# marios2019/CSN

Hardware: AMD Instinct MI355X
Metric: CSA fwd+bwd points/sec (10k pts x 256 ch, K=3) (higher is better)
Workload: dtype bf16x3 (fp32 operands split into 2 bf16, 3 bf16 MFMA per product, fp32 accumulate); 1 GPU; BASELINE configs[2]: CSA K=3, 32 query shapes/GPU x 10000 pts x 256 ch, n_heads=1, d_k=d_v=256, 20 blocks of 500, 39 classes, fwd + masked CE + bwd, train mode (dropout 0.1 live, 2K+2 evaluations/shape), math mode bf16x3; K=3, parallelism=single GPU

## Files before the change

csn_amd/_lib.py:

```python
from __future__ import annotations

import ctypes
import hashlib
import os
import subprocess
from ctypes import c_char_p, c_double, c_float, c_int, c_longlong, c_ulonglong, c_void_p
from typing import Optional

_HERE = os.path.dirname(os.path.abspath(__file__))
_CSRC = os.path.join(_HERE, "csrc")
LIB_PATH = os.path.join(_HERE, "libcsn_hip.so")
SOURCES = ["gemm_f32.hip", "gemm_bf16x3.hip", "wx_stream.hip", "wx_lnb.hip", "loss.hip", "attn_f32.hip", "attn_bf16x3.hip", "attn_dkv.hip", "attn_dv_scores.hip", "fold.hip", "outproj_ln.hip", "retrieval.hip", "retrieval_screen.hip", "combine.hip", "compat.hip", "minkowski_csn.hip", "minkowski_seg.hip", "rows_fc.hip", "sparse_conv.hip", "sparse_conv_maps16.hip", "train_maps16.hip", "sparse_conv_cat.hip", "octant_conv.hip", "octant_conv_maps16.hip", "octant_conv_stats.hip", "rows_bn_act.hip", "point_field.hip", "kernel_map.hip", "octant_map.hip", "points.hip", "csn_capi.hip"]
HEADERS = ["csn_common.h", "csn_kernels.h", "csn_window.h", "wx_common.h", "rows_mma.h", "sconv_gemm_body.inc", "sconv_a16_body.inc", "rows_bn_act_body.inc", "octant_rows_body.inc", os.path.join("..", "..", "include", "csn_hip.h")]
ARCH = "gfx950"
BUILD_FLAGS = [f"--offload-arch={ARCH}", "-O3", "-std=c++17", "-fPIC", "-fvisibility=hidden", "-shared"]

_lib: Optional[ctypes.CDLL] = None


class CsnError(RuntimeError):
    pass


class BnTerms(ctypes.Structure):
    _fields_ = [("z", c_void_p * 3), ("ld_z", c_longlong * 3), ("mean", c_void_p * 3), ("scale", c_void_p * 3),
                ("gamma", c_void_p * 3), ("beta", c_void_p * 3), ("dz", c_void_p * 3), ("ld_dz", c_longlong * 3),
                ("dgamma", c_void_p * 3), ("dbeta", c_void_p * 3)]


class CatParts(ctypes.Structure):
    _fields_ = [("x", c_void_p * 4), ("ld_x", c_longlong * 4), ("c_in", c_int * 4)]


STAMP_PATH = LIB_PATH + ".sha256"


def _source_digest() -> str:
    h = hashlib.sha256(" ".join(BUILD_FLAGS).encode())
    for f in SOURCES + HEADERS:
        h.update(f.encode())
        with open(os.path.join(_CSRC, f), "rb") as fh:
            h.update(fh.read())
    return h.hexdigest()


def _stale() -> bool:
# ... 127 lines not shown
                                        c_float, c_ulonglong, c_void_p]),
    "csn_varlen_attn_bwd_f32": (c_int, [c_void_p, c_void_p, c_longlong, c_void_p, c_void_p, c_void_p, c_longlong, c_longlong,
                                        c_int, c_int, c_void_p, c_void_p, c_void_p, c_void_p, c_void_p, c_void_p, c_void_p,
                                        c_longlong, c_longlong, c_int, c_int, c_int, c_int, c_int, c_void_p, c_void_p, c_int,
                                        c_float, c_ulonglong, c_void_p]),
    "csn_cross_attn_flash_available": (c_int, [c_int]),
    "csn_cross_attn_bwd_flash_f32": (c_int, [c_void_p, c_void_p, c_longlong, c_void_p, c_void_p, c_void_p, c_longlong, c_longlong,
                                             c_int, c_int, c_void_p, c_void_p, c_void_p, c_void_p, c_void_p, c_longlong,
                                             c_longlong, c_int, c_int, c_int, c_int, c_int, c_int, c_float, c_ulonglong,
                                             c_void_p]),
    "csn_varlen_attn_bwd_flash_f32": (c_int, [c_void_p, c_void_p, c_longlong, c_void_p, c_void_p, c_void_p, c_longlong, c_longlong,
                                              c_int, c_int, c_void_p, c_void_p, c_void_p, c_void_p, c_void_p, c_longlong,
                                              c_longlong, c_int, c_int, c_int, c_int, c_int, c_void_p, c_void_p, c_int, c_float,
                                              c_ulonglong, c_void_p]),
    "csn_project_qkv_f32": (c_int, [c_void_p, c_longlong, c_int, c_void_p, c_int, c_int, c_void_p, c_longlong, c_int, c_void_p,
                                    c_longlong, c_int, c_int, c_int, c_float, c_int, c_void_p]),
    "csn_outproj_ln_workspace_floats": (c_longlong, [c_int, c_int, c_int, c_int]),
    "csn_masked_ce_workspace_bytes": (c_longlong, [c_int, c_int]),
    "csn_masked_ce_fwd_f32": (c_int, [c_void_p, c_longlong, c_int, c_void_p, c_longlong, c_int, c_int, c_int, c_int, c_void_p,
                                      c_void_p, c_longlong, c_void_p, c_void_p]),
    "csn_masked_ce_bwd_f32": (c_int, [c_void_p, c_longlong, c_int, c_void_p, c_longlong, c_int, c_int, c_int, c_int, c_void_p,
                                      c_void_p, c_void_p, c_void_p, c_longlong, c_int, c_void_p]),
    "csn_outproj_ln_fwd_f32": (c_int, [c_void_p, c_longlong, c_void_p, c_void_p, c_longlong, c_void_p, c_void_p,
                                       c_longlong, c_void_p, c_int, c_int, c_int, c_int, c_int, c_float, c_float,
                                       c_ulonglong, c_void_p, c_void_p, c_longlong, c_void_p]),
    "csn_outproj_ln_bwd_f32": (c_int, [c_void_p, c_void_p, c_void_p, c_longlong, c_void_p, c_longlong, c_void_p,
                                       c_void_p, c_void_p, c_void_p, c_void_p, c_void_p, c_longlong, c_int, c_int, c_int,
                                       c_int, c_int, c_int, c_float, c_ulonglong, c_int, c_longlong, c_void_p, c_int,
                                       c_void_p, c_int, c_void_p]),
    "csn_outproj_lnb_workspace_floats": (c_longlong, [c_int, c_int, c_int, c_int, c_int]),
    "csn_outproj_lnb_f32": (c_int, [c_void_p, c_void_p, c_void_p, c_longlong, c_void_p, c_void_p, c_void_p, c_void_p, c_int, c_int,
                                    c_int, c_int, c_int, c_int, c_float, c_ulonglong, c_void_p, c_int, c_void_p, c_int, c_void_p,
                                    c_void_p, c_void_p, c_longlong, c_void_p]),
    "csn_project_wgrad_f32": (c_int, [c_void_p, c_longlong, c_int, c_void_p, c_longlong, c_int, c_void_p, c_int, c_int,
                                      c_int, c_int, c_float, c_int, c_void_p, c_longlong, c_void_p]),
    "csn_retrieval_measure_f32": (c_int, [c_void_p, c_void_p, c_void_p, c_int, c_int, c_int, c_int, c_int, c_void_p,
                                          c_longlong, c_void_p]),
    "csn_rowsum_f32": (c_int, [c_void_p, c_void_p, c_longlong, c_int, c_longlong, c_void_p]),
    "csn_mix_fwd_f32": (c_int, [c_void_p, c_void_p, c_void_p, c_void_p, c_void_p, c_int, c_int, c_int, c_int, c_void_p,
                                c_void_p]),
    "csn_mix_bwd_f32": (c_int, [c_void_p, c_void_p, c_void_p, c_void_p, c_void_p, c_void_p, c_void_p, c_int, c_int, c_int,
                                c_int, c_void_p, c_void_p, c_void_p]),
    "csn_compat_fwd_f32": (c_int, [c_void_p, c_void_p, c_void_p, c_void_p, c_void_p, c_void_p, c_void_p, c_void_p, c_int, c_int,
                                   c_int, c_int, c_void_p]),
    "csn_compat_bwd_f32": (c_int, [c_void_p, c_void_p, c_void_p, c_void_p, c_void_p, c_void_p, c_void_p, c_void_p, c_longlong,
                                   c_void_p, c_void_p, c_void_p, c_void_p, c_void_p, c_int, c_int, c_int, c_int, c_void_p]),
    "csn_ragged_pool_f32": (c_int, [c_void_p, c_longlong, c_int, c_void_p, c_void_p, c_int, c_int, c_void_p, c_void_p, c_void_p,
                                    c_void_p, c_void_p]),
    "csn_ragged_pool_bwd_f32": (c_int, [c_void_p, c_void_p, c_void_p, c_void_p, c_int, c_int, c_void_p, c_longlong, c_int, c_int,
                                        c_void_p]),
    "csn_ragged_mix_fwd_f32": (c_int, [c_void_p, c_longlong, c_int, c_int, c_int, c_void_p, c_void_p, c_int, c_int, c_int, c_void_p,
                                       c_void_p, c_void_p, c_void_p, c_longlong, c_void_p]),
    "csn_ragged_mix_bwd_f32": (c_int, [c_void_p, c_longlong, c_void_p, c_longlong, c_int, c_int, c_int, c_void_p, c_void_p, c_int,
                                       c_int, c_int, c_void_p, c_void_p, c_void_p, c_void_p, c_void_p, c_void_p, c_longlong,
                                       c_void_p]),
    "csn_ragged_retrieval_f32": (c_int, [c_void_p, c_void_p, c_void_p, c_int, c_void_p, c_void_p, c_void_p, c_int, c_int, c_void_p,
                                         c_void_p, c_longlong, c_void_p]),
    "csn_retrieval_screen_workspace_floats": (c_longlong, [c_longlong, c_longlong, c_int, c_int, c_int, c_int]),
    "csn_retrieval_screen_eps": (c_float, [c_int]),
    "csn_ragged_retrieval_screen_f16": (c_int, [c_void_p, c_void_p, c_void_p, c_int, c_void_p, c_void_p, c_void_p, c_int, c_int,
                                                c_void_p, c_void_p, c_longlong, c_void_p]),
    "csn_ragged_retrieval_pairs_f32": (c_int, [c_void_p, c_void_p, c_void_p, c_int, c_void_p, c_void_p, c_void_p, c_int, c_int,
                                               c_void_p, c_longlong, c_void_p, c_void_p, c_longlong, c_void_p]),
    "csn_ragged_seg_workspace_bytes": (c_longlong, [c_int]),
    "csn_ragged_seg_fwd_f32": (c_int, [c_void_p, c_int, c_int, c_void_p, c_void_p, c_void_p, c_int, c_int, c_int, c_void_p, c_void_p,
                                       c_void_p, c_void_p, c_void_p, c_void_p, c_longlong, c_void_p]),
# ... 68 lines not shown
                                                  c_void_p, c_void_p, c_void_p, c_void_p, c_float, c_float, c_void_p, c_longlong,
                                                  c_void_p]),
    "csn_sparse_conv_stats_fwd_t16": (c_int, [c_void_p, c_int, c_longlong, c_int, c_void_p, c_int, c_int, c_int, c_int, c_void_p, c_void_p,
                                              c_longlong, c_void_p, c_void_p, c_void_p, c_void_p, c_float, c_float, c_void_p,
                                              c_longlong, c_void_p]),
    "csn_rows_bn_act_fwd_t16": (c_int, [c_void_p, c_int, c_int, c_int, c_int, c_float, c_void_p, c_int, c_longlong, c_int, c_void_p,
                                        c_int, c_longlong, c_void_p]),
    "csn_rows_bn_act_bwd_t16": (c_int, [c_void_p, c_longlong, c_void_p, c_int, c_longlong, c_void_p, c_int, c_int, c_int, c_int,
                                        c_float, c_int, c_void_p, c_longlong, c_void_p, c_longlong, c_void_p]),
    "csn_sparse_conv_bwd_t16": (c_int, [c_void_p, c_longlong, c_void_p, c_int, c_longlong, c_int, c_int, c_int, c_int, c_int, c_void_p,
                                        c_void_p, c_void_p, c_void_p, c_longlong, c_void_p, c_void_p, c_void_p, c_longlong, c_void_p]),
    "csn_voxel_mean_f32": (c_int, [c_void_p, c_longlong, c_int, c_void_p, c_void_p, c_int, c_int, c_void_p, c_longlong, c_void_p]),
    "csn_point_interp_fwd_f32": (c_int, [c_void_p, c_longlong, c_int, c_void_p, c_void_p, c_void_p, c_int, c_int, c_void_p, c_longlong,
                                         c_void_p]),
    "csn_point_interp_bwd_f32": (c_int, [c_void_p, c_longlong, c_int, c_void_p, c_void_p, c_void_p, c_void_p, c_int, c_int, c_void_p,
                                         c_longlong, c_void_p]),
    "csn_coord_keys_i64": (c_int, [c_void_p, c_int, c_int, c_void_p, c_void_p, c_void_p]),
    "csn_coord_down_i64": (c_int, [c_void_p, c_int, c_int, c_void_p, c_void_p]),
    "csn_kernel_map_i32": (c_int, [c_void_p, c_void_p, c_int, c_void_p, c_int, c_int, c_int, c_void_p, c_void_p, c_void_p]),
    "csn_octant_partition_i32": (c_int, [c_void_p, c_void_p, c_int, c_int, c_void_p, c_void_p, c_int, c_void_p, c_void_p, c_void_p, c_void_p,
                                         c_void_p]),
    "csn_octant_order_workspace_bytes": (c_longlong, [c_int]),
    "csn_octant_order_i32": (c_int, [c_void_p, c_int, c_void_p, c_void_p, c_void_p, c_longlong, c_void_p, c_void_p]),
    "csn_points_normalize_f32": (c_int, [c_void_p, c_void_p, c_int, c_longlong, c_int, c_void_p, c_void_p, c_void_p]),
    "csn_points_bounds_f64": (c_int, [c_void_p, c_void_p, c_int, c_longlong, c_void_p, c_void_p, c_int, c_void_p, c_void_p, c_void_p]),
    "csn_points_batch_f32": (c_int, [c_void_p, c_void_p, c_void_p, c_int, c_longlong, c_void_p, c_void_p, c_void_p, c_void_p, c_int,
                                     c_int, c_double, c_double, c_double, c_void_p, c_void_p, c_void_p, c_void_p, c_longlong, c_void_p,
                                     c_void_p]),
    "csn_field_index_i32": (c_int, [c_void_p, c_void_p, c_void_p, c_int, c_int, c_void_p, c_void_p, c_void_p, c_void_p, c_void_p,
                                    c_void_p]),
}

EXPORTS = tuple(_SIGNATURES)
DEV_BIG_TILES, DEV_WIDE_GEMM, DEV_WIDE_FORMS, DEV_WX, DEV_LNB_GROUP, DEV_SCONV_NB, DEV_KV_SAME = 0, 1, 2, 3, 5, 7, 8
DEV_WX_DEFAULT = 9


def lib() -> ctypes.CDLL:
    global _lib
    if _lib is None:
        path = os.environ.get("CSN_LIB_PATH", LIB_PATH)
        if not os.path.exists(path):
            raise CsnError(f"{path} is missing: run `python -c 'import __graft_entry__ as g; g.build()'` "
                           "(there is no CPU or eager fallback for the CSA kernels)")
        handle = ctypes.CDLL(path)
        for name, (res, args) in _SIGNATURES.items():
            fn = getattr(handle, name)
            fn.restype = res
            fn.argtypes = args
        if handle.csn_version() != 17:
            raise CsnError("libcsn_hip.so ABI version mismatch")
        _lib = _Hooked(handle)
    return _lib


_call_hook = None


def set_call_hook(fn) -> None:
    global _call_hook
    _call_hook = fn


class _Hooked:

    def __init__(self, handle):
        self._handle = handle
# ... 24 lines not shown
```

csn_amd/csrc/attn_bf16x3.hip:

```cpp
#include "csn_common.h"
#include "csn_kernels.h"

namespace {

constexpr int KT = 32;
constexpr float LOG2E = 1.4426950408889634f, LN2 = 0.6931471805599453f;

using namespace csn_mode;
typedef f32x4m f32x4v;
typedef s16x4 __attribute__((address_space(3))) * lds_s16x4;
typedef short __attribute__((address_space(3))) lds_s16;
typedef s16x8 __attribute__((address_space(3))) lds_s16x8;

CSN_DEVINL const lds_s16* opaque_lds(const short* p) {
  const lds_s16* q = (const lds_s16*)p;
  asm volatile("" : "+v"(q));
  return q;
}

template <typename PR>
CSN_DEVINL f32x4v mma16(s16x8 ah, s16x8 al, s16x8 bh, s16x8 bl, f32x4v c) {
  if constexpr (PR::NT == 3) {
    c = mfma16<PR::HALF>(al, bh, c);
    c = mfma16<PR::HALF>(ah, bl, c);
  }
  return mfma16<PR::HALF>(ah, bh, c);
}

constexpr bool csn_attn_x3fwd96(int npl, int dt, bool bwd) { return npl == 2 && dt == 3 && !bwd; }
constexpr int csn_attn_waves(int npl, int dt, bool bwd, bool rc_f32 = false) {
  return (!rc_f32 && ((npl == 1 ? dt <= 3 : dt <= 2) || csn_attn_x3fwd96(npl, dt, bwd))) ? 4 : 2;
}
template <typename PR, int DT, bool BWD, bool KVP, bool RC = false, int NOP = 0, bool KV_SAME = false>
__global__ __launch_bounds__(512, csn_attn_waves(PR::NPL, DT, BWD, RC && !KVP)) void csn_attn_bf16x3_kernel(CsnAttnArgs p) {
  static_assert(!KV_SAME || (DT == 8 && NOP == 2), "one request per tile: the folded d = 256 backward");
  static_assert(PR::NT == 3 || KVP, "single-product modes take K / V as tile planes");
  static_assert(!RC || BWD, "score recomputation: backward kernel");
  static_assert(!NOP || (BWD && KVP && !RC && PR::NPL == 2), "no P planes: the kept-scores backward in two planes");
  constexpr int NPL = PR::NPL;
  constexpr int D = 32 * DT;
  constexpr int UPR = KVP ? 4 * NPL : 8;
  constexpr int RPP = 512 / UPR;
  constexpr int PIECES = D * UPR;
  constexpr int NP_T = (PIECES + 511) / 512;
  constexpr int PLANE = D * KT + 32;
  constexpr bool EARLY = NPL == 1 || DT <= 4 || (!BWD && !RC);
  static_assert(!RC || EARLY, "score recomputation: early requests (where three LDS images per stage fit)");
  constexpr int NB_ST = RC ? 3 : 2;
  constexpr int TILE_EL = (2 + NB_ST + (RC ? 2 : 0)) * NPL * PLANE, STAGE_EL = D * 128 * 2;
  static_assert(2 * (TILE_EL > STAGE_EL ? TILE_EL : STAGE_EL) <= 160 * 1024, "LDS budget of one CU");
  __shared__ __attribute__((aligned(16))) short tiles[TILE_EL > STAGE_EL ? TILE_EL : STAGE_EL];
  auto tileA = [&](int st, int pl) -> short* { return tiles + (st * NPL + pl) * PLANE; };
  auto tileB = [&](int st, int pl) -> short* { return tiles + ((2 + st) * NPL + pl) * PLANE; };
  auto tileC = [&](int st, int pl) -> short* { return tiles + ((2 + NB_ST + st) * NPL + pl) * PLANE; };

  const int tid = threadIdx.x, lane = tid & 63, wave = tid >> 6;
  const int lq = lane & 15, kq = lane >> 4;
  const int Tq = p.Tq > 0 ? p.Tq : p.T;
  const int QT = (Tq + 127) / 128;
  const int Y = p.n_blocks * p.H;
  const int L = blockIdx.x, slot = L & 7, jj = L >> 3;
  const int qt = jj % QT, u = (jj / QT) * 8 + slot;
  if (u >= Y * p.E) return;
  const int zz = u / Y;
  const int it0 = p.grp_off ? p.grp_off[zz] : zz;
  const int it1 = p.grp_off ? p.grp_off[zz + 1] : it0 + 1;
  const int e0 = p.eval_ids ? p.eval_ids[it0] : it0;
  const int hd = (u % Y) % p.H, blk = (u % Y) / p.H;
// ... 106 lines not shown
    if (KVP) {
      const unsigned off = (kt * KT + 8 * t_u) < T ? t_off : CSN_OOB;
#pragma unroll
      for (int i = 0; i < NP_T; ++i)
        g[i] = csn_bload4(rs, (i == NP_T - 1 && !t_last_ok) ? CSN_OOB : off, (unsigned)(kt * (64 * NPL) + RPP * i * kld * 2));
    } else {
      const int k0 = kt * KT;
      const unsigned off = (k0 + 4 * t_c) < T ? t_off : CSN_OOB;
#pragma unroll
      for (int i = 0; i < NP_T; ++i)
        g[i] = csn_bload4(rs, (i == NP_T - 1 && !t_last_ok) ? CSN_OOB : off, (unsigned)(k0 + 64 * i * ldk) * 4u);
    }
  };

  auto stage_in = [&](const csn_rsrc_t& rs, int fmt) {
    f32x4 ch[CH_T];
    if (NPL == 1 && fmt) {
      u32x2 c2[CH_T];
#pragma unroll
      for (int t = 0; t < CH_T; ++t) c2[t] = csn_bload2(rs, c_off == CSN_OOB ? CSN_OOB : c_off >> 1, (unsigned)(16 * t * ld) * 2u);
#pragma unroll
      for (int t = 0; t < CH_T; ++t) ch[t] = act16_to_f32(__builtin_bit_cast(s16x4, c2[t]), fmt);
    } else {
#pragma unroll
      for (int t = 0; t < CH_T; ++t) ch[t] = csn_bload4(rs, c_off, (unsigned)(16 * t * ld) * 4u);
    }
#pragma unroll
    for (int t = 0; t < CH_T; ++t) {
      const int row = crow + 16 * t;
      *reinterpret_cast<f32x4*>(&xbuf[row * 128 + ((cc ^ (4 * ((row >> 3) & 1))) << 2)]) = ch[t];
    }
  };
  auto pick = [&](int row) { return xbuf[row * 128 + ((((col >> 2) ^ (4 * ((row >> 3) & 1))) << 2) | (col & 3))]; };
  float rv[D / 4];
  if (BWD || it == it0) {
    stage_in(Rr, p.r_fmt);
    __syncthreads();
#pragma unroll
    for (int s = 0; s < D / 32; ++s)
#pragma unroll
      for (int j = 0; j < 8; ++j) {
        const float v = pick(32 * s + 8 * kq + j);
        rv[8 * s + j] = v;
        Rh[s][j] = to16<PR::HALF>(v);
        Rl[s][j] = PR::NT == 3 ? to16<PR::HALF>(v - from16<PR::HALF>(Rh[s][j])) : Rh[s][j];
      }
  }
  if (!BWD) {
    os = p.out_index ? p.out_index[e] : e;
    stat_off0 = stat_off;
#pragma unroll
    for (int c = 0; c < D / 16; ++c) O[c] = f32x4v{0.f, 0.f, 0.f, 0.f};
    m_run = -INFINITY; m2_run = -INFINITY; l_run = 0.f;
  }
  float delta_q = 0.f;
  if (BWD) {
    const csn_rsrc_t Xr = map_rsrc(p.ctx, qs * p.q_shape_stride + head_off, p.ctx_fmt);
    __syncthreads();
    stage_in(Xr, p.ctx_fmt);
    __syncthreads();
#pragma unroll
    for (int s = 0; s < D / 32; ++s)
#pragma unroll
      for (int j = 0; j < 8; ++j) delta_q = fmaf(rv[8 * s + j], pick(32 * s + 8 * kq + j), delta_q);
    delta_q += __shfl_xor(delta_q, 16, 64);
    delta_q += __shfl_xor(delta_q, 32, 64);
  }
  if constexpr (RC) {
    const long long q2s = p.q2_index ? p.q2_index[e] : e;
    if (it == it0 || q2s != q2s_staged) {
      q2s_staged = q2s;
      const csn_rsrc_t Qr = map_rsrc(p.q2, q2s * p.q2_shape_stride + head_off, p.q2_fmt);
      __syncthreads();
      stage_in(Qr, p.q2_fmt);
      __syncthreads();
#pragma unroll
      for (int s = 0; s < D / 32; ++s)
#pragma unroll
        for (int j = 0; j < 8; ++j) {
          const float v = pick(32 * s + 8 * kq + j);
          Qh[s][j] = to16<PR::HALF>(v);
          Ql[s][j] = PR::NT == 3 ? to16<PR::HALF>(v - from16<PR::HALF>(Qh[s][j])) : Qh[s][j];
        }
    }
  }
  __syncthreads();

  const bool drop = p.dropout_p > 0.f;
  const unsigned thr16 = csn_drop_threshold16(p.dropout_p);
  const float keep_scale = drop ? 1.f / (1.f - p.dropout_p) : 1.f;
  const unsigned salt = csn_block_salt((unsigned long long)(((long long)e * p.H + hd) * p.n_blocks + blk), p.seed);
  const int mp = Tq > Tp ? Tq : Tp;
  const unsigned pw_base = (unsigned)(4 * kq * mp + qrow);

  float lse2_q = 0.f;
  if (BWD) {
    lse2_q = q_ok ? p.lse[stat_off + qrow] * LOG2E : 0.f;
// ... 305 lines not shown
    if constexpr (RC) {
    } else if constexpr (EARLY) {
      if (more) commitB_from(nxt, g2);
    } else {
      if (more) { commitB(nxt); if (kt + 2 < nkt) fetch(Ar, kt + 2); }
    }
    __syncthreads();
  }

  if (!late) __syncthreads();
  if constexpr (!BWD) write_out();
  }

  if constexpr (BWD) write_out();
}

template <typename PR, int DT>
int launch_dt(const CsnAttnArgs& a, bool bwd, hipStream_t st) {
  const long long units = (long long)a.n_blocks * a.H * a.E;
  dim3 grid((unsigned)(((units + 7) / 8) * 8 * (((a.Tq > 0 ? a.Tq : a.T) + 127) / 128)));
  if (a.kv_planes) {
    if (bwd) {
      if constexpr (!PR::HALF) {
        if (a.q2) {
          if constexpr (csn_attn_recompute_fits(PR::NPL, DT))
            hipLaunchKernelGGL((csn_attn_bf16x3_kernel<PR, DT, true, true, true>), grid, dim3(512), 0, st, a);
          else return -1;
        } else if (a.sc_tiles == 2) {
          if constexpr (csn_attn_dv_scores_fits(PR::NT == 3 ? 1 : 2, 32 * DT))
            hipLaunchKernelGGL((csn_attn_bf16x3_kernel<PR, DT, true, true, false, 1>), grid, dim3(512), 0, st, a);
          else return -1;
        } else if (a.sc_tiles == 3) {
          if constexpr (csn_attn_dv_scores_fits(PR::NT == 3 ? 1 : 2, 32 * DT)) {
            if (a.kv_same) hipLaunchKernelGGL((csn_attn_bf16x3_kernel<PR, DT, true, true, false, 2, true>), grid, dim3(512), 0, st, a);
            else hipLaunchKernelGGL((csn_attn_bf16x3_kernel<PR, DT, true, true, false, 2>), grid, dim3(512), 0, st, a);
          } else return -1;
        } else hipLaunchKernelGGL((csn_attn_bf16x3_kernel<PR, DT, true, true>), grid, dim3(512), 0, st, a);
      } else return -1;
    } else hipLaunchKernelGGL((csn_attn_bf16x3_kernel<PR, DT, false, true>), grid, dim3(512), 0, st, a);
  } else {
    if constexpr (PR::NT == 3) {
      if (bwd && a.q2) {
        if constexpr (csn_attn_recompute_fits(PR::NPL, DT))
          hipLaunchKernelGGL((csn_attn_bf16x3_kernel<PR, DT, true, false, true>), grid, dim3(512), 0, st, a);
        else return -1;
      } else if (bwd) hipLaunchKernelGGL((csn_attn_bf16x3_kernel<PR, DT, true, false>), grid, dim3(512), 0, st, a);
      else hipLaunchKernelGGL((csn_attn_bf16x3_kernel<PR, DT, false, false>), grid, dim3(512), 0, st, a);
    } else return -1;
  }
  return (int)hipGetLastError();
}

template <typename PR>
int launch_any(const CsnAttnArgs& a, int d, bool bwd, hipStream_t st) {
  if (a.E <= 0 || a.n_blocks <= 0) return 0;
  if ((a.ld & 3) || (a.Tp & 3) || (a.ld_kv & 3)) return -2;
  if ((a.T & 3) && a.kv_planes) return -2;
  if ((a.q_shape_stride & 3) || (a.kv_shape_stride & 3)) return -4;
  if (a.sc_tiles && a.Tp < (a.T + 31) / 32 * 32) return -2;
  if (a.sc_layout && (PR::NPL != 2 || !a.kv_planes || a.Tq > 0 || a.tq_arr || a.t_arr || a.Tp < (a.T + 31) / 32 * 32 || (bwd && !a.sc_tiles)))
    return -1;
  if (a.q2 && (!bwd || (a.q2_shape_stride & 3))) return -1;
  if (a.sc_tiles >= 2 && (a.sc_tiles > 3 || !bwd || !a.kv_planes || a.q2 || a.Tq > 0 || a.tq_arr || a.t_arr)) return -1;
  if (a.q2 && !a.kv_planes && (a.sc_tiles || a.grp_off)) return -1;
  if ((a.r_fmt || a.ctx_fmt || a.q2_fmt || a.out_fmt) && (PR::NPL != 1 || !a.kv_planes)) return -1;
  if (a.out_fmt && a.accumulate) return -1;
  if (a.kv_planes && (a.T > 512 || (a.kv_ld & 7) || (a.kv_shape_stride & 7))) return -2;
  switch (d) {
    case 32: return launch_dt<PR, 1>(a, bwd, st);
    case 64: return launch_dt<PR, 2>(a, bwd, st);
    case 96: return launch_dt<PR, 3>(a, bwd, st);
    case 128: return launch_dt<PR, 4>(a, bwd, st);
    case 256: return launch_dt<PR, 8>(a, bwd, st);
    default: return -5;
  }
}

int launch_mode(const CsnAttnArgs& a, int d, int mode, bool bwd, hipStream_t st) {
  switch (mode) {
    case 1: return launch_any<Bf16x3>(a, d, bwd, st);
    case 2: return launch_any<Bf16>(a, d, bwd, st);
    case 3: return launch_any<F16>(a, d, bwd, st);
    default: return -1;
  }
}

}

int csn_dev_kv_same = 1;

int csn_launch_attn_fwd_bf16x3(const CsnAttnArgs& a, int d, int mode, hipStream_t st) {
  return launch_mode(a, d, mode, false, st);
}
int csn_launch_attn_bwd_bf16x3(const CsnAttnArgs& a, int d, int mode, hipStream_t st) { return launch_mode(a, d, mode, true, st); }
```

csn_amd/csrc/csn_capi.hip:

```cpp
#include "../../include/csn_hip.h"
#include "csn_kernels.h"
#include <cmath>

namespace {

int g_math_mode = CSN_MATH_BF16X3;
thread_local int t_math_mode = -1;

inline int mode() { return t_math_mode >= 0 ? t_math_mode : g_math_mode; }
thread_local int t_act16 = 0;
inline int act16() { return t_act16 & 3; }
inline bool grad16() { return (t_act16 & 4) != 0; }
inline bool act16_fwd_ok() { return act16() == 0 || (act16() == 1 && mode() == 2) || (act16() == 2 && mode() == 3); }
inline bool act16_bwd_ok() { return act16() == 0 || mode() == 2; }
thread_local int t_rows16 = 0;
inline int rows_mode() { return mode() >= 2 && !t_rows16 ? 1 : mode(); }
thread_local int t_score_layout = 0;
inline int planes_of(int m) { return m == 1 ? 2 : 1; }

struct ModeGuard {
  int saved;
  explicit ModeGuard(int m) : saved(t_math_mode) { t_math_mode = m; }
  ~ModeGuard() { t_math_mode = saved; }
};

int launch_gemm(const CsnGemmArgs& a, int b_is_nk, int batch, hipStream_t st) {
  if (mode() != 0) {
    if (a.M <= 0 || a.N <= 0 || batch <= 0) return 0;
    if ((a.A.ld & 3) || (a.B.ld & 3) || (a.K & 3) || (a.k_chunk & 3)) return CSN_E_ALIGN;
    if (a.N & 3) return CSN_E_ALIGN;
    return csn_launch_gemm_bf16x3(a, b_is_nk, batch, mode(), st);
  }
  return csn_launch_gemm_f32(a, b_is_nk, batch, st);
}

inline bool mis16(const void* p) { return (reinterpret_cast<uintptr_t>(p) & 15) != 0; }

int launch_wx(const float* w, const float* x, long long x_stride, int ldx, void* out, long long out_stride, int ldo, int rows,
              int n_items, int n_points, int div_rows, float div_val, int out_mode, int tb, hipStream_t st) {
  CsnWxArgs a;
  a.w = w; a.x = x; a.x_item_stride = x_stride; a.ldx = ldx;
  a.out = out; a.out_item_stride = out_stride; a.ldo = ldo;
  a.n_items = n_items; a.n_points = n_points; a.n_sets = rows / 256;
  a.div_rows = div_rows; a.div_val = div_val; a.div_rcp = 1.f / div_val;
  int ex = 0;
  a.div_exact = (std::frexp(div_val, &ex) == 0.5f && div_val > 0.f) ? 1 : 0;
  a.tb = tb;
  return csn_launch_wx(a, out_mode, st);
}

// ... 17 lines not shown
int wgrad_chunk(int n_maps, int n_points) {
  long long total = (long long)n_maps * n_points;
  long long want = (total + 511) / 512;
  if (want < 256) want = 256;
  long long n_chunks = (n_points + want - 1) / want;
  if (n_chunks < 1) n_chunks = 1;
  long long c = (n_points + n_chunks - 1) / n_chunks;
  c = ((c + 3) / 4) * 4;
  return (int)c;
}

int wgrad(const float* a, long long a_stride, int lda, const float* b, long long b_stride, int ldb, float* dw, int rows,
          int cols, int n_maps, int n_points, float scale, int accumulate, float* ws, long long ws_floats,
          hipStream_t st, int a_fmt = 0, int b_fmt = 0) {
  const int chunk = wgrad_chunk(n_maps, n_points);
  const int n_chunks = (n_points + chunk - 1) / chunk;
  const long long slabs = (long long)n_maps * n_chunks;
  if (ws_floats < slabs * rows * cols) return CSN_E_WORKSPACE;
  CsnGemmArgs g;
  g.A = operand(a, chunk, 0, a_stride, nullptr, lda);
  g.B = operand(b, chunk, 0, b_stride, nullptr, ldb);
  g.A.fmt = a_fmt; g.B.fmt = b_fmt;
  g.C = operand(ws, (long long)rows * cols, 0, (long long)n_chunks * rows * cols, nullptr, cols);
  g.M = rows; g.N = cols; g.K = n_points;
  g.n0 = n_chunks; g.n1 = 1; g.k_chunk = chunk;
  g.alpha = 1.f; g.div_rows = 0; g.div_val = 1.f; g.accumulate = 0; g.eval_ids = nullptr;
  int rc = launch_gemm(g, 1, (int)slabs, st);
  if (rc) return rc;
  return csn_launch_slab_reduce(ws, dw, (int)slabs, (long long)rows * cols, scale, accumulate, st);
}

}

extern "C" {

int csn_version(void) { return CSN_ABI_VERSION; }

int csn_dev_get(int key) {
  switch (key) {
    case CSN_DEV_BIG_TILES: return csn_gemm_big_tiles;
    case CSN_DEV_WIDE_GEMM: return csn_gemm_wide;
    case CSN_DEV_WIDE_FORMS: return csn_gemm_wide_set;
    case CSN_DEV_WX: return csn_dev_wx;
    case CSN_DEV_LNB_GROUP: return csn_dev_lnb_group;
    case CSN_DEV_SCONV_NB: return csn_dev_sconv_nb;
    case CSN_DEV_KV_SAME: return csn_dev_kv_same;
    default: return CSN_E_ARG;
  }
}
int csn_dev_set(int key, int value) {
  const int prev = csn_dev_get(key);
  switch (key) {
    case CSN_DEV_BIG_TILES: csn_gemm_big_tiles = value; break;
    case CSN_DEV_WIDE_GEMM: csn_gemm_wide = value; break;
    case CSN_DEV_WIDE_FORMS: csn_gemm_wide_set = value; break;
    case CSN_DEV_WX:
      if (value & ~(1 | 4 | 8)) return CSN_E_ARG;
      csn_dev_wx = value;
      break;
    case CSN_DEV_LNB_GROUP: csn_dev_lnb_group = value < 0 ? 0 : value; break;
    case CSN_DEV_SCONV_NB:
      if (value < 0 || value > 4) return CSN_E_ARG;
      csn_dev_sconv_nb = value;
      break;
    case CSN_DEV_KV_SAME:
      if (value != 0 && value != 1) return CSN_E_ARG;
      csn_dev_kv_same = value;
      break;
    default: return CSN_E_ARG;
  }
  return prev;
}

int csn_set_math_mode(int m) {
  if (m < 0 || m > 3) return CSN_E_ARG;
  g_math_mode = m;
  return 0;
}
int csn_set_thread_math_mode(int m) {
  if (m < -1 || m > 3) return CSN_E_ARG;
  t_math_mode = m;
  return 0;
}
int csn_get_math_mode(void) { return mode(); }
int csn_get_thread_math_mode(void) { return t_math_mode; }
int csn_set_thread_act16(int fmt) {
  if (fmt < 0 || (fmt & 3) == 3 || fmt > 6 || fmt == 4) return CSN_E_ARG;
  t_act16 = fmt;
  return 0;
}
int csn_get_thread_act16(void) { return t_act16; }
int csn_set_thread_rows16(int on) {
  if (on != 0 && on != 1) return CSN_E_ARG;
  t_rows16 = on;
  return 0;
}
int csn_get_thread_rows16(void) { return t_rows16; }
int csn_set_thread_score_layout(int layout) {
  if (layout < 0 || layout > 1) return CSN_E_ARG;
  t_score_layout = layout;
  return 0;
}
int csn_get_thread_score_layout(void) { return t_score_layout; }

const char* csn_status_string(int status) {
  switch (status) {
    case 0: return "ok";
    case CSN_E_ARG: return "csn: null pointer, non-positive size, a count beyond its row, or a flag this math mode does not take";
    case CSN_E_ALIGN: return "csn: a size or leading dimension is not a multiple of 4 floats";
    case CSN_E_PTR: return "csn: device pointer not 16-byte aligned";
    case CSN_E_STRIDE: return "csn: a stride is not a multiple of 4 floats";
    case CSN_E_DIM: return "csn: unsupported head / model dimension (need 32, 64, 96, 128 or 256)";
    case CSN_E_WORKSPACE: return "csn: workspace too small";
    default: return status > 0 ? hipGetErrorString((hipError_t)status) : "csn: unknown status";
  }
}

long long csn_wgrad_workspace_floats(int rows, int cols, int n_maps, int n_points) {
  if (rows <= 0 || cols <= 0 || n_maps <= 0 || n_points <= 0) return 0;
  const int chunk = wgrad_chunk(n_maps, n_points);
  const long long n_chunks = (n_points + chunk - 1) / chunk;
  return (long long)n_maps * n_chunks * rows * cols;
}

// ... 221 lines not shown

int csn_block_attn_fwd_grouped_f32(const float* q, const float* k, const float* v, long long q_shape_stride,
                                   long long kv_shape_stride, const int* q_index, const int* kv_index, int ld, float* ctx,
                                   long long ctx_eval_stride, float* scores, float* lse, int n_evals, int n_heads,
                                   int d_head, int block, int n_blocks, int score_pitch, float rescale_threshold,
                                   float dropout_p, unsigned long long seed, int qkv_split, long long qkv_plane_stride,
                                   const int* eval_ids, const int* group_offsets, int n_groups, void* stream) {
  if (!eval_ids || !group_offsets) return CSN_E_ARG;
  return attn_fwd_impl(q, k, v, q_shape_stride, kv_shape_stride, q_index, kv_index, ld, ctx, ctx_eval_stride, scores, lse,
                       n_evals, n_heads, d_head, block, n_blocks, score_pitch, rescale_threshold, dropout_p, seed, qkv_split,
                       qkv_plane_stride, 0, 0, stream, nullptr, nullptr, eval_ids, group_offsets, n_groups);
}

int csn_cross_attn_fwd_f32(const float* q, const float* k, const float* v, long long q_shape_stride,
                           long long kv_shape_stride, int ld_q, int ld_kv, float* ctx, long long ctx_eval_stride,
                           float* scores, float* lse, int n_evals, int n_heads, int d_head, int n_queries, int n_keys,
                           int score_pitch, float rescale_threshold, float dropout_p, unsigned long long seed, void* stream) {
  if (n_queries <= 0 || n_keys <= 0) return CSN_E_ARG;
  if (n_queries & 3) return CSN_E_ALIGN;
  ModeGuard guard(mode() >= 2 ? 1 : mode());
  return attn_fwd_impl(q, k, v, q_shape_stride, kv_shape_stride, nullptr, nullptr, ld_q, ctx, ctx_eval_stride, scores, lse,
                       n_evals, n_heads, d_head, n_keys, 1, score_pitch, rescale_threshold, dropout_p, seed, 0, 0, n_queries,
                       ld_kv, stream);
}

static int attn_bwd_dq_impl(const float* dctx, const float* ctx, long long ctx_eval_stride, const float* k,
                            const float* v, long long kv_shape_stride, const int* kv_index, int ld, float* scores,
                            float* dscores, const float* lse, float* delta, float* dq, long long dq_slot_stride,
                            const int* dq_index, int accumulate, const int* eval_ids, int n_launch_evals, int n_heads,
                            int d_head, int block, int n_blocks, int score_pitch, float dropout_p,
                            unsigned long long seed, int dctx_split, long long dctx_plane_stride, int kv_split,
                            long long kv_plane_stride, int probs_tiles, int block_q, int ld_kv, const int* group_offsets,
                            int n_groups, void* stream, const int* tq_arr = nullptr, const int* t_arr = nullptr,
                            const float* q = nullptr, long long q_shape_stride = 0, const int* q_index = nullptr) {
  if (block_q < 0 || ld_kv < 0 || (ld_kv & 3)) return CSN_E_ARG;
  if (q && (block_q != 0 || !kv_split || !(csn_attn_bwd_grouping(d_head, block) & 4) || mis16(q))) return CSN_E_ARG;
  if (q && (q_shape_stride & 3)) return CSN_E_STRIDE;
  if ((tq_arr || t_arr) && (group_offsets || n_blocks != 1)) return CSN_E_ARG;
  if (n_blocks <= 0 || block <= 0) return CSN_E_ARG;
  const int t_last = last_block_points(block, n_blocks, ld, block_q);
  if (t_last < 0) return t_last;
  if (block_q != 0 && ((long long)n_blocks * block_q > ld || (long long)n_blocks * ((block + 3) / 4 * 4) > (ld_kv > 0 ? ld_kv : ld)))
    return CSN_E_ARG;
  if (group_offsets && (n_groups <= 0 || !eval_ids || !(csn_attn_bwd_grouping(d_head, block) & 1))) return CSN_E_ARG;
  if ((block & 3) && (block_q == 0 || kv_split)) return CSN_E_ALIGN;
  if (probs_tiles && (mode() == 0 || score_pitch < (block + 31) / 32 * 32)) return CSN_E_ARG;
  if (probs_tiles < 0 || probs_tiles > 3) return CSN_E_ARG;
  if (probs_tiles >= 2 && (q || !kv_split || block_q != 0 || tq_arr || t_arr || act16() ||
                           !csn_attn_bwd_dv_scores_available(d_head, block)))
    return CSN_E_ARG;
  if (dropout_p < 0.f || dropout_p >= 1.f) return CSN_E_ARG;
  if (dctx_split) return CSN_E_ARG;
  if (kv_split && mode() == 0) return CSN_E_ARG;
  if (kv_split < 0 || kv_split > 2 || (kv_split == 2 && mode() != 2)) return CSN_E_ARG;
  if (mode() == 3) return CSN_E_ARG;
  if (mode() == 2 && !(kv_split && (probs_tiles || q))) return CSN_E_ARG;
  const int bp = 512 * planes_of(mode());
  if (kv_split && (kv_plane_stride <= 0 || (kv_plane_stride % bp) || kv_plane_stride < (long long)n_blocks * bp ||
                   block > 512 || (kv_shape_stride & 7)))
    return CSN_E_ARG;
  const bool need_sc = !q || (probs_tiles && mode() == 1), need_ds = (!q || probs_tiles) && probs_tiles != 3;
  if (!dctx || !ctx || !k || !v || !lse || (!delta && probs_tiles != 3) || !dq || (need_sc && !scores) || (need_ds && !dscores)) return CSN_E_ARG;
  if (n_launch_evals <= 0 || n_heads <= 0 || block <= 0 || n_blocks <= 0) return CSN_E_ARG;
  if (!dim_ok(d_head)) return CSN_E_DIM;
  if ((ld & 3) || (score_pitch & 3) || score_pitch < (block + 3) / 4 * 4) return CSN_E_ALIGN;
  if (mis16(dctx) || mis16(k) || mis16(v) || mis16(scores) || mis16(dscores) || mis16(dq)) return CSN_E_PTR;
  if ((kv_shape_stride & 3) || (ctx_eval_stride & 3) || (dq_slot_stride & 3)) return CSN_E_STRIDE;
  hipStream_t st = (hipStream_t)stream;
  CsnAttnArgs a;
  a.ctx = ctx;
  a.T_last = t_last;
  a.Tq = block_q; a.ld_kv = ld_kv;
  a.q = dctx; a.k = k; a.v = v;
  a.q_shape_stride = dctx_split ? 2 * ctx_eval_stride : ctx_eval_stride;
  a.kv_shape_stride = kv_shape_stride;
  a.q_index = nullptr; a.kv_index = kv_index; a.ld = ld;
  a.out = dq; a.out_eval_stride = dq_slot_stride;
  a.scores = scores; a.dscores = dscores; a.lse = const_cast<float*>(lse); a.delta = delta;
  a.E = group_offsets ? n_groups : n_launch_evals; a.H = n_heads; a.T = block; a.Tp = score_pitch; a.n_blocks = n_blocks;
  a.rescale_threshold = 0.f;
  a.eval_ids = eval_ids; a.grp_off = group_offsets; a.out_index = dq_index; a.accumulate = accumulate;
  a.dropout_p = dropout_p; a.seed = seed;
  a.r_planes = 0; a.kv_planes = kv_split != 0; a.r_plane_stride = 0; a.kv_plane_stride = 0; a.kv_ld = (int)kv_plane_stride;
  a.kv_f16 = kv_split == 2;
  a.sc_tiles = probs_tiles;
  if (kv_split == 1 && k == v && mode() == 1 && d_head == 256 && probs_tiles == 3) a.kv_same = csn_dev_kv_same;
  a.tq_arr = tq_arr; a.t_arr = t_arr;
  a.q2 = q; a.q2_shape_stride = q_shape_stride; a.q2_index = q_index;
  if (t_score_layout) {
    if (mode() != 1 || !kv_split || block_q != 0 || tq_arr || t_arr || !probs_tiles) return CSN_E_ARG;
    a.sc_layout = 1;
  }
  if (act16()) {
    if (!act16_bwd_ok() || !kv_split || block_q != 0) return CSN_E_ARG;
    a.r_fmt = 1; a.ctx_fmt = act16(); a.q2_fmt = act16();
    if (grad16()) {
      if (accumulate) return CSN_E_ARG;
      a.out_fmt = 1;
    }
  }
  return mode() != 0 ? csn_launch_attn_bwd_bf16x3(a, d_head, mode(), st) : csn_launch_attn_bwd_f32(a, d_head, st);
}

int csn_block_attn_bwd_dq_f32(const float* dctx, const float* ctx, long long ctx_eval_stride, const float* k,
                              const float* v, long long kv_shape_stride, const int* kv_index, int ld, float* scores,
                              float* dscores, const float* lse, float* delta, float* dq, long long dq_slot_stride,
                              const int* dq_index, int accumulate, const int* eval_ids, int n_launch_evals, int n_heads,
                              int d_head, int block, int n_blocks, int score_pitch, float dropout_p,
                              unsigned long long seed, int dctx_split, long long dctx_plane_stride, int kv_split,
                              long long kv_plane_stride, int probs_tiles, const int* group_offsets, int n_groups,
                              void* stream) {
  return attn_bwd_dq_impl(dctx, ctx, ctx_eval_stride, k, v, kv_shape_stride, kv_index, ld, scores, dscores, lse, delta, dq,
                          dq_slot_stride, dq_index, accumulate, eval_ids, n_launch_evals, n_heads, d_head, block, n_blocks,
                          score_pitch, dropout_p, seed, dctx_split, dctx_plane_stride, kv_split, kv_plane_stride, probs_tiles,
                          0, 0, group_offsets, n_groups, stream);
}

int csn_block_attn_bwd_dq_recompute_f32(const float* dctx, const float* ctx, long long ctx_eval_stride, const float* q,
                                        long long q_shape_stride, const int* q_index, const float* k, const float* v,
                                        long long kv_shape_stride, const int* kv_index, int ld, float* probs,
                                        float* dscores, const float* lse, float* delta, float* dq,
                                        long long dq_slot_stride, const int* dq_index, int accumulate, const int* eval_ids,
                                        int n_launch_evals, int n_heads, int d_head, int block, int n_blocks,
                                        int score_pitch, float dropout_p, unsigned long long seed,
                                        long long kv_plane_stride, int kv_f16, int probs_tiles, const int* group_offsets,
                                        int n_groups, void* stream) {
  if (!q) return CSN_E_ARG;
  return attn_bwd_dq_impl(dctx, ctx, ctx_eval_stride, k, v, kv_shape_stride, kv_index, ld, probs, dscores, lse, delta, dq,
                          dq_slot_stride, dq_index, accumulate, eval_ids, n_launch_evals, n_heads, d_head, block, n_blocks,
                          score_pitch, dropout_p, seed, 0, 0, kv_f16 ? 2 : 1, kv_plane_stride, probs_tiles, 0, 0, group_offsets,
                          n_groups, stream, nullptr, nullptr, q, q_shape_stride, q_index);
}

static int attn_bwd_dkv_impl(const float* dctx, long long ctx_eval_stride, const float* q, long long q_shape_stride,
                             const int* q_index, int ld, const float* probs, const float* dscores, float* dk,
                             float* dv, long long dkv_slot_stride, const int* dk_index, const int* dv_index,
                             int accumulate, const int* eval_ids, int n_launch_evals, int n_heads, int d_head,
                             int block, int n_blocks, int score_pitch, int dctx_split, long long dctx_plane_stride,
                             int q_split, long long q_plane_stride, int probs_tiles, int block_q, int ld_kv,
                             const int* group_offsets, int n_groups, void* stream, const int* tq_arr = nullptr,
                             const int* t_arr = nullptr) {
  if (block_q < 0 || ld_kv < 0 || (ld_kv & 3) || (block_q & 3)) return CSN_E_ARG;
  if ((block & 3) && block_q == 0) return CSN_E_ALIGN;
  const int bq = block_q > 0 ? block_q : block, lk = ld_kv > 0 ? ld_kv : ld, bk4 = (block + 3) / 4 * 4;
  if (n_blocks <= 0 || block <= 0) return CSN_E_ARG;
  const int t_last = last_block_points(block, n_blocks, ld, block_q);
  if (t_last < 0) return t_last;
  if (block_q != 0 && ((long long)n_blocks * bk4 > lk || (long long)n_blocks * bq > ld)) return CSN_E_ARG;
  if (probs_tiles && (mode() == 0 || score_pitch < (block + 31) / 32 * 32)) return CSN_E_ARG;
  if (mode() == 3 || (mode() == 2 && !probs_tiles)) return CSN_E_ARG;
  if (dctx_split || q_split) return CSN_E_ARG;
  if (group_offsets && (n_groups <= 0 || !eval_ids || !(csn_attn_bwd_grouping(d_head, block) & 2))) return CSN_E_ARG;
  const bool dk_only = !probs && !dv;
  if (!dctx || !q || !dscores || !dk || (!dv && !dk_only)) return CSN_E_ARG;
  if (!probs && !dk_only && !(probs_tiles && mode() == 2)) return CSN_E_ARG;
  if (n_launch_evals <= 0 || n_heads <= 0 || block <= 0 || n_blocks <= 0) return CSN_E_ARG;
  if (!dim_ok(d_head)) return CSN_E_DIM;
  if ((ld & 3) || (score_pitch & 3) || score_pitch < bk4) return CSN_E_ALIGN;
  if (mis16(dctx) || mis16(q) || mis16(probs) || mis16(dscores) || mis16(dk) || mis16(dv)) return CSN_E_PTR;
  if ((q_shape_stride & 3) || (ctx_eval_stride & 3) || (dkv_slot_stride & 3)) return CSN_E_STRIDE;
// ... 310 lines not shown
                           long long xres_shape_stride, const int* res_index, float* xhat,
                           long long xhat_eval_stride, float* rstd, int n_evals, int d_model, int d_inner, int ld,
                           int n_points, float eps, float dropout_p, unsigned long long seed, float* xhat_sum,
                           float* sum_ws, long long sum_ws_floats, void* stream) {
  if (dropout_p < 0.f || dropout_p >= 1.f) return CSN_E_ARG;
  if (!ctx || !wfc || !xres || !xhat || !rstd || n_evals <= 0 || n_points <= 0 || d_inner <= 0 || n_points > ld) return CSN_E_ARG;
  if (dropout_p > 0.f && (long long)(d_model / 2 + 1) * ld >= (1ll << 32)) return CSN_E_ARG;
  if (xhat_sum && xhat_eval_stride != (long long)d_model * ld) return CSN_E_STRIDE;
  if (!dim_ok(d_model)) return CSN_E_DIM;
  if ((ld & 3) || (d_inner & 3) || (n_points & 3)) return CSN_E_ALIGN;
  if (mis16(ctx) || mis16(wfc) || mis16(xres) || mis16(xhat)) return CSN_E_PTR;
  if ((ctx_eval_stride & 3) || (xres_shape_stride & 3) || (xhat_eval_stride & 3)) return CSN_E_STRIDE;
  CsnOutProjArgs a;
  a.ctx = ctx; a.ctx_eval_stride = ctx_eval_stride; a.wfc = wfc;
  a.xres = xres; a.xres_shape_stride = xres_shape_stride; a.res_index = res_index;
  a.xhat = xhat; a.xhat_eval_stride = xhat_eval_stride; a.rstd = rstd;
  a.E = n_evals; a.C = d_model; a.D = d_inner; a.ld = ld; a.n_points = n_points; a.eps = eps;
  a.dropout_p = dropout_p; a.seed = seed;
  a.xhat_sum = xhat_sum; a.sum_ws = sum_ws; a.sum_ws_floats = sum_ws ? sum_ws_floats : 0;
  if (act16() && !act16_fwd_ok()) return CSN_E_ARG;
  a.act16 = act16();
  return csn_launch_outproj_ln_fwd_f32(a, mode(), (hipStream_t)stream);
}

int csn_outproj_ln_bwd_f32(const float* dxhat, const float* xhat, const float* rstd, long long eval_stride,
                           const float* ctx, long long ctx_eval_stride, const float* wfc_t, float* dz, float* dz_res,
                           float* dctx, float* dwfc, float* ws, long long ws_floats, int n_evals, int d_model,
                           int d_inner, int ld, int n_points, int accumulate, float dropout_p,
                           unsigned long long seed, int dctx_split, long long dctx_plane_stride,
                           const float* dxhat_rows, int n_dense_evals, const float* dxhat_scale, int dxhat_group,
                           void* stream) {
  if (dropout_p < 0.f || dropout_p >= 1.f) return CSN_E_ARG;
  if (dxhat_group < 0) return CSN_E_ARG;
  if (dropout_p > 0.f && (long long)(d_model / 2 + 1) * ld >= (1ll << 32)) return CSN_E_ARG;
  if (dctx_split && mode() == 0) return CSN_E_ARG;
  if (n_dense_evals < 0 || n_dense_evals > n_evals || (n_dense_evals > 0 && !dxhat)) return CSN_E_ARG;
  if (!xhat || !rstd || !ctx || !wfc_t || !dz || !dctx || !dwfc || !ws) return CSN_E_ARG;
  if (n_evals <= 0 || n_points <= 0 || d_inner <= 0 || d_model <= 0 || n_points > ld) return CSN_E_ARG;
  if ((ld & 3) || (d_inner & 3) || (d_model & 3) || (n_points & 3)) return CSN_E_ALIGN;
  if (mis16(dxhat) || mis16(xhat) || mis16(ctx) || mis16(wfc_t) || mis16(dz) || mis16(dctx) || mis16(dwfc) || mis16(ws))
    return CSN_E_PTR;
  if ((eval_stride & 3) || (ctx_eval_stride & 3)) return CSN_E_STRIDE;
  hipStream_t st = (hipStream_t)stream;
  CsnLnBwdArgs l;
  l.dxhat = dxhat; l.xhat = xhat; l.rstd = rstd; l.dz = dz; l.dz_res = dz_res; l.eval_stride = eval_stride;
  l.E = n_evals; l.C = d_model; l.ld = ld; l.n_points = n_points;
  l.dropout_p = dropout_p; l.seed = seed;
  l.dxhat_rows = dxhat_rows; l.n_dense = n_dense_evals;
  l.dxhat_scale = dxhat_scale; l.dxhat_group = dxhat_group > 0 ? dxhat_group : 1;
  const int a16 = act16();
  if (a16 && (!act16_bwd_ok() || dctx_split)) return CSN_E_ARG;
  l.act16 = a16;
  int rc = 0;
  if (mode() == 1 && !a16 && !dctx_split && csn_wx_takes(d_inner, d_model) &&
      csn_wx_geometry_takes(csn_dev_lnb_group > 0 && csn_dev_lnb_group < n_evals ? csn_dev_lnb_group : n_evals, n_points, d_inner / 256)) {
    const int G = csn_dev_lnb_group > 0 ? csn_dev_lnb_group : n_evals;
    const bool fused = csn_wx_lnb_takes(l, d_inner) && eval_stride == ctx_eval_stride;
    for (int e0 = 0; e0 < n_evals && !rc; e0 += G) {
      const int ng = n_evals - e0 < G ? n_evals - e0 : G;
      if (fused) {
        CsnWxLnbArgs f{};
        f.w = wfc_t; f.xhat = xhat; f.rstd = rstd; f.eval_stride = eval_stride; f.ld = ld;
        f.dxhat = dxhat; f.dxhat_group = l.dxhat_group; f.n_dense = n_dense_evals; f.dxhat_scale = dxhat_scale; f.dxhat_rows = dxhat_rows;
        f.dz = dz; f.dz_res = dz_res; f.dctx = dctx; f.dctx_eval_stride = ctx_eval_stride;
        f.n_items = ng; f.n_points = n_points; f.e_base = e0; f.dropout_p = dropout_p; f.seed = seed;
        rc = csn_launch_wx_lnb(f, st);
        if (rc != CSN_NOT_TAKEN) continue;
      }
      l.e_base = e0; l.E = ng;
      rc = csn_launch_ln_bwd_f32(l, st);
      if (rc) return rc;
      rc = launch_wx(wfc_t, dz + (long long)e0 * eval_stride, eval_stride, ld, dctx + (long long)e0 * ctx_eval_stride, ctx_eval_stride, ld,
                     d_inner, ng, n_points, 0, 1.f, 0, 0, st);
    }
    if (rc) return rc;
    return wgrad(dz, eval_stride, ld, ctx, ctx_eval_stride, ld, dwfc, d_model, d_inner, n_evals, n_points, 1.f, accumulate, ws,
                 ws_floats, st, 0, 0);
  }
  rc = csn_launch_ln_bwd_f32(l, st);
  if (rc) return rc;
  CsnGemmArgs g;
  g.A = operand(wfc_t, 0, 0, 0, nullptr, d_model);
  g.B = operand(dz, 0, 0, eval_stride, nullptr, ld);
  g.C = operand(dctx, 0, 0, dctx_split ? 2 * ctx_eval_stride : ctx_eval_stride, nullptr, ld);
  g.C.planes = dctx_split; g.C.plane_stride = dctx_plane_stride;
  if (a16) { g.B.fmt = CSN_FMT_16; g.C.planes = 1; }
  g.M = d_inner; g.N = n_points; g.K = d_model;
  g.n0 = 1; g.n1 = 1; g.k_chunk = 0;
  g.alpha = 1.f; g.div_rows = 0; g.div_val = 1.f; g.accumulate = 0; g.eval_ids = nullptr;
  rc = launch_gemm(g, 0, n_evals, st);
  if (rc) return rc;
  return wgrad(dz, eval_stride, ld, ctx, ctx_eval_stride, ld, dwfc, d_model, d_inner, n_evals, n_points, 1.f,
               accumulate, ws, ws_floats, st, a16 ? CSN_FMT_16 : 0, a16 == 2 ? CSN_FMT_F16_TO_BF16 : (a16 ? CSN_FMT_16 : 0));
}

static bool lnb_range_takes(int n_evals, int d_model, int d_inner, int ld, int n_points, long long eval_stride) {
  if (n_evals <= 0 || n_points <= 0 || n_points > ld || mode() != 1 || act16()) return false;
  CsnLnBwdArgs l{};
  l.C = d_model; l.ld = ld; l.n_points = n_points; l.eval_stride = eval_stride; l.act16 = 0;
  return csn_wx_takes(d_inner, d_model) && csn_wx_geometry_takes(n_evals, n_points, d_inner / 256) && csn_wx_lnb_takes(l, d_inner);
}

long long csn_outproj_lnb_workspace_floats(int n_evals, int d_model, int d_inner, int ld, int n_points) {
  if (!lnb_range_takes(n_evals, d_model, d_inner, ld, n_points, (long long)d_model * ld)) return 0;
  return csn_wx_lnb_red_floats(n_evals, n_points);
}

int csn_outproj_lnb_f32(const float* dxhat, const float* xhat, const float* rstd, long long eval_stride, const float* wfc_t,
                        float* dz, float* dz_res, float* dctx, int e_base, int n_evals, int d_model, int d_inner, int ld,
                        int n_points, float dropout_p, unsigned long long seed, const float* dxhat_rows, int n_dense_evals,
                        const float* dxhat_scale, int dxhat_group, float* rowdot, float* rowsum, float* red_ws,
                        long long red_ws_floats, void* stream) {
  if (dropout_p < 0.f || dropout_p >= 1.f) return CSN_E_ARG;
  if (dxhat_group < 0 || e_base < 0 || n_evals <= 0 || n_dense_evals < 0 || (n_dense_evals > 0 && !dxhat)) return CSN_E_ARG;
  if (!xhat || !rstd || !wfc_t || !dz || !dctx) return CSN_E_ARG;
  if (n_points <= 0 || d_inner <= 0 || d_model <= 0 || n_points > ld) return CSN_E_ARG;
  if (dropout_p > 0.f && (long long)(d_model / 2 + 1) * ld >= (1ll << 32)) return CSN_E_ARG;
  if ((ld & 3) || (d_inner & 3) || (d_model & 3) || (n_points & 3)) return CSN_E_ALIGN;
  if (mis16(dxhat) || mis16(xhat) || mis16(wfc_t) || mis16(dz) || mis16(dz_res) || mis16(dctx) || mis16(red_ws)) return CSN_E_PTR;
  if (eval_stride & 3) return CSN_E_STRIDE;
  if (!lnb_range_takes(e_base + n_evals, d_model, d_inner, ld, n_points, eval_stride)) return CSN_E_DIM;
  const int group = dxhat_group > 0 ? dxhat_group : 1;
  const bool reduce = rowdot || rowsum || red_ws;
  if (reduce) {
    if (!rowdot || !rowsum || !red_ws || e_base != 0 || n_evals > n_dense_evals || n_evals % group) return CSN_E_ARG;
    if (red_ws_floats < csn_wx_lnb_red_floats(n_evals, n_points)) return CSN_E_WORKSPACE;
  }
  CsnWxLnbArgs f{};
  f.w = wfc_t; f.xhat = xhat; f.rstd = rstd; f.eval_stride = eval_stride; f.ld = ld;
  f.dxhat = dxhat; f.dxhat_group = group; f.n_dense = n_dense_evals; f.dxhat_scale = dxhat_scale; f.dxhat_rows = dxhat_rows;
  f.dz = dz; f.dz_res = dz_res; f.dctx = dctx; f.dctx_eval_stride = eval_stride;
  f.n_items = n_evals; f.n_points = n_points; f.e_base = e_base; f.dropout_p = dropout_p; f.seed = seed;
  if (reduce) { f.red_ws = red_ws; f.red_slots = csn_wx_ln_sum_slots(n_evals, n_points); f.rowdot = rowdot; f.rowsum = rowsum; }
  const int rc = csn_launch_wx_lnb(f, (hipStream_t)stream);
  return rc == CSN_NOT_TAKEN ? CSN_E_DIM : rc;
}

int csn_project_wgrad_f32(const float* dout, long long dout_shape_stride, int ld_dout, const float* x,
                          long long x_shape_stride, int ld_x, float* dw, int rows, int channels, int n_shapes,
                          int n_points, float scale, int accumulate, float* ws, long long ws_floats,
                          void* stream) {
  if (!dout || !x || !dw || !ws || rows <= 0 || channels <= 0 || n_shapes <= 0 || n_points <= 0) return CSN_E_ARG;
  if (n_points > ld_dout || n_points > ld_x) return CSN_E_ARG;
  if ((ld_dout & 3) || (ld_x & 3) || (n_points & 3) || (channels & 3)) return CSN_E_ALIGN;
  if (mis16(dout) || mis16(x) || mis16(dw) || mis16(ws)) return CSN_E_PTR;
  if ((dout_shape_stride & 3) || (x_shape_stride & 3)) return CSN_E_STRIDE;
  const bool g16 = act16() && grad16();
  if (g16 && !act16_bwd_ok()) return CSN_E_ARG;
  return wgrad(dout, dout_shape_stride, ld_dout, x, x_shape_stride, ld_x, dw, rows, channels, n_shapes, n_points, scale,
               accumulate, ws, ws_floats, (hipStream_t)stream, g16 ? CSN_FMT_16 : 0, 0);
}

int csn_retrieval_measure_f32(const float* f1, const float* f2, float* out, int s1, int n1, int s2, int n2,
                              int channels, float* ws, long long ws_floats, void* stream) {
  if (!f1 || !f2 || !out || !ws || s1 <= 0 || s2 <= 0 || n1 <= 0 || n2 <= 0 || channels <= 0) return CSN_E_ARG;
  if (channels & 3) return CSN_E_ALIGN;
  if (mis16(f1) || mis16(f2) || mis16(ws)) return CSN_E_PTR;
  const long long need = (long long)s1 * n1 + (long long)s2 * n2 + (long long)s1 * s2 * n1;
  if (ws_floats < need) return CSN_E_WORKSPACE;
  return csn_launch_retrieval_f32(f1, f2, out, s1, n1, s2, n2, channels, ws, (hipStream_t)stream);
}

int csn_rowsum_f32(const float* x, float* out, long long rows, int n_points, long long ld, void* stream) {
  if (!x || !out || rows <= 0 || n_points <= 0 || n_points > ld) return CSN_E_ARG;
  if ((n_points & 3) || (ld & 3)) return CSN_E_ALIGN;
  if (mis16(x)) return CSN_E_PTR;
  return csn_launch_rowsum_f32(x, out, rows, n_points, ld, (hipStream_t)stream, act16());
}
// ... 1025 lines not shown
```

csn_amd/csrc/csn_kernels.h:

```cpp
#pragma once
#include "csn_common.h"

struct CsnGemmArgs {
  CsnOperand A, B, C;
  int M, N, K;
  int n0, n1;
  int k_chunk;
  float alpha;
  int div_rows;
  float div_val;
  int accumulate;
  const int* eval_ids;
  int batch;
  const int* grp_off = nullptr;
  const int* grp_items = nullptr;
  const int* n_arr = nullptr;
  const int* k_arr = nullptr;
  int n_last = 0, k_last = 0;
};

int csn_launch_gemm_f32(const CsnGemmArgs& a, int b_is_nk, int batch, hipStream_t st);
int csn_launch_gemm_bf16x3(const CsnGemmArgs& a, int b_is_nk, int batch, int mode, hipStream_t st);
int csn_gemm_tile_major_planes(int M, int N);
int csn_gemm_bf16x3_big_tiles(int M, int N);
// ... 37 lines not shown
struct CsnAttnArgs {
  const float* q;  const float* k;  const float* v;
  long long q_shape_stride, kv_shape_stride;
  const int* q_index; const int* kv_index;
  int ld;
  float* out;        long long out_eval_stride;
  float* scores;
  float* dscores;
  float* lse;
  float* delta;
  const float* ctx;
  int E, H, T, Tp, n_blocks;
  float rescale_threshold;
  const int* eval_ids;
  const int* grp_off;
  const int* out_index;
  int accumulate;
  float dropout_p;
  unsigned long long seed;
  int r_planes, kv_planes;
  long long r_plane_stride, kv_plane_stride;
  int kv_ld;
  int Tq;
  int ld_kv;
  int sc_tiles;
  const int* tq_arr;
  const int* t_arr;
  int T_last;
  const float* q2 = nullptr; long long q2_shape_stride = 0; const int* q2_index = nullptr;
  int kv_f16 = 0;
  int r_fmt = 0, ctx_fmt = 0, q2_fmt = 0, out_fmt = 0;
  int sc_layout = 0;
  int kv_same = 0;
};
extern int csn_dev_kv_same;
constexpr bool csn_attn_recompute_fits(int planes, int dt) { return planes == 1 || dt <= 4; }
struct CsnAttnDkvArgs {
  const float* q;     long long q_shape_stride;  const int* q_index;
  const float* dctx;  long long ctx_eval_stride;
  const float* k;  const float* v;
  long long kv_shape_stride;  int kv_ld;  const int* kv_index;
  const float* lse;  const float* delta;
  float* dk;  float* dv;  long long dkv_slot_stride;
  const int* dk_index;  const int* dv_index;
  int accumulate;
  const int* eval_ids;  const int* grp_off;  int n_groups;
  int ld, H, T, Tp, n_blocks, T_last;
  float dropout_p;  unsigned long long seed;
  int kv_f16 = 0;
  int q_fmt = 0, dctx_fmt = 0;
  int out_fmt = 0;
  int Tq = 0, ld_kv = 0;
  const int* tq_arr = nullptr;  const int* t_arr = nullptr;
};
int csn_launch_attn_dkv_flash(const CsnAttnDkvArgs& a, int d, int mode, hipStream_t st);
constexpr bool csn_attn_dkv_flash_fits(int dt) { return dt <= 4; }

struct CsnAttnDvArgs {
  const float* dctx;  long long ctx_eval_stride;
  const float* scores;
  const float* lse;
  float* dv;  long long dkv_slot_stride;  const int* dv_index;
  const int* eval_ids;  const int* grp_off;  int n_groups;
  int ld, H, T, Tp, n_blocks, T_last;
  float dropout_p;  unsigned long long seed;
  int sc_layout = 0;
// ... 30 lines not shown
  float* lse;
  double* partials;
  float* stats;
  const float* grad_out;  float* dlogits;  long long dshape_stride;  int dld;
};
long long csn_masked_ce_blocks(int n_shapes, int n_points);
int csn_launch_masked_ce_fwd(const CsnMaskedCeArgs& a, hipStream_t st);
int csn_launch_masked_ce_bwd(const CsnMaskedCeArgs& a, hipStream_t st);

struct CsnLnBwdArgs {
  const float* dxhat; const float* xhat; const float* rstd;
  const float* dxhat_rows;
  int n_dense;
  const float* dxhat_scale; int dxhat_group;
  float* dz;
  float* dz_res;
  long long eval_stride;
  int E, C, ld, n_points;
  float dropout_p;
  unsigned long long seed;
  int act16 = 0;
  int e_base = 0;
};
int csn_launch_ln_bwd_f32(const CsnLnBwdArgs& a, hipStream_t st);
struct CsnWxLnbArgs {
  const float* w;
  const float* xhat; const float* rstd; long long eval_stride; int ld;
  const float* dxhat; int dxhat_group; int n_dense; const float* dxhat_scale; const float* dxhat_rows;
  float* dz; float* dz_res;
  float* dctx; long long dctx_eval_stride;
  int n_items, n_points, e_base;
  float dropout_p; unsigned long long seed;
  float* red_ws; int red_slots; float* rowdot; float* rowsum;
};
long long csn_wx_lnb_red_floats(int n_items, int n_points);
bool csn_wx_lnb_takes(const CsnLnBwdArgs& a, int d_inner);
int csn_launch_wx_lnb(const CsnWxLnbArgs& a, hipStream_t st);

int csn_launch_rowdot_f32(const float* a, const float* b, float* out, const int* eval_ids, int E, int H, int d, int ld,
                          int n_points, long long eval_stride, int a_split, long long a_plane_stride, hipStream_t st);

int csn_launch_rowsum_f32(const float* x, float* out, long long rows, int n, long long ld, hipStream_t st, int x16 = 0);
int csn_launch_mix_fwd_f32(const float* xhat, const float* comp, const float* gamma, const float* beta, float* feats, int B,
                           int K1, int C, int NP, const float* xhat0, hipStream_t st, int x16 = 0);
int csn_launch_mix_bwd_f32(const float* dfeats, const float* xhat, const float* comp, const float* gamma, float* dxhat,
                           float* rowdot, float* rowsum, int B, int K1, int C, int NP, const float* xhat0, float* dxhat0,
                           hipStream_t st, int x16 = 0);
int csn_launch_retrieval_f32(const float* f1, const float* f2, float* out, int s1, int n1, int s2, int n2, int C,
                             float* ws, hipStream_t st);

int csn_ragged_mix_tiles(int max_points);
int csn_launch_ragged_pool_f32(const float* xhat, long long eval_stride, int ld, const int* counts, int E, int C, const float* gamma,
                               const float* beta, float* pooled, float* mean, hipStream_t st);
int csn_launch_ragged_pool_bwd_f32(const float* dpooled, const float* gamma, const int* counts, int E, int C, float* dxhat,
                                   long long eval_stride, int ld, int accumulate, hipStream_t st);
int csn_launch_ragged_mix_fwd_f32(const float* xhat, long long eval_stride, int ld, int cross_first, const int* offsets, int B,
                                  int K1, int C, int max_points, const float* comp, const float* gamma, const float* beta, float* out,
                                  long long ld_out, hipStream_t st);
int csn_launch_ragged_mix_bwd_f32(const float* dout, long long ld_dout, const float* xhat, long long eval_stride, int ld,
                                  int cross_first, const int* offsets, int B, int K1, int C, const float* comp, const float* gamma,
                                  float* dxhat, double* rowdot, double* rowsum, double* ws, hipStream_t st);
int csn_launch_ragged_retrieval_f32(const float* f1, const int* off1, int s1, long long N1, const float* f2, const int* off2, int s2,
                                    long long N2, int max_n1, int C, float* out, float* ws, hipStream_t st);
int csn_launch_ragged_mean_f32(const float* part, const int* off1, float* out, int pairs, int s2, int tiles, hipStream_t st);
int csn_launch_ragged_retrieval_pairs_f32(const float* f1, const int* off1, int s1, long long N1, const float* f2, const int* off2,
                                          int s2, long long N2, int max_n1, int C, const int* pairs, long long n_pairs, float* out,
                                          float* ws, hipStream_t st);
// ... 211 lines not shown
```

csn_amd/csrc/wx_lnb.hip:

```cpp
#include "csn_common.h"
#include "csn_kernels.h"
#include "wx_common.h"
#include <type_traits>

namespace {

constexpr int LNB_G = 8 * WX_EB * 2;
constexpr int LNB_EBW = WX_EB / 2;

template <int N>
CSN_DEVINL void lnb_arrived(f32x4* R) {
  asm volatile("s_waitcnt vmcnt(%5)" : "+v"(R[0]), "+v"(R[1]), "+v"(R[2]), "+v"(R[3]), "+v"(R[4]) : "n"(N) : "memory");
}

CSN_DEVINL void lnb_store1(float v, u32x4 rsrc, unsigned voff) {
  asm volatile("buffer_store_dword %0, %1, %2, 0 offen\n\ts_nop 1" :: "v"(v), "v"(voff), "s"(rsrc) : "memory");
}

CSN_DEVINL float lnb_sum_row_groups(float v) {
  v += __builtin_bit_cast(float, __builtin_amdgcn_mov_dpp(__builtin_bit_cast(int, v), 0x128 , 0xf, 0xf, false));
  float c = v;
  asm("s_nop 1\n\tv_permlane16_swap_b32 %0, %1" : "+v"(v), "+v"(c));
  v += c;
  c = v;
  asm("s_nop 1\n\tv_permlane32_swap_b32 %0, %1" : "+v"(v), "+v"(c));
  return v + c;
}

CSN_DEVINL float lnb_sum_row_lanes(float v) {
  v += __builtin_bit_cast(float, __builtin_amdgcn_mov_dpp(__builtin_bit_cast(int, v), 0xb1 , 0xf, 0xf, false));
  v += __builtin_bit_cast(float, __builtin_amdgcn_mov_dpp(__builtin_bit_cast(int, v), 0x4e , 0xf, 0xf, false));
  v += __builtin_bit_cast(float, __builtin_amdgcn_mov_dpp(__builtin_bit_cast(int, v), 0x141 , 0xf, 0xf, false));
  return v;
}

template <bool DROP, bool RES, bool RED>
__global__ __launch_bounds__(512, 2) void csn_wx_lnb_kernel(CsnWxLnbArgs p) {
  __shared__ __attribute__((aligned(16))) short smem[LNB_G + WX_NS * WX_STAGE + 8 * LNB_EBW * 2 + 1024 + 1024 + 1024];
  short* xs = smem + LNB_G;
  const int tid = threadIdx.x, lane = tid & 63, wave = __builtin_amdgcn_readfirstlane(tid >> 6);
  const int l31 = lane & 31, h = lane >> 5;
  float* eb = reinterpret_cast<float*>(smem + LNB_G + WX_NS * WX_STAGE) + wave * LNB_EBW;
  float* red = reinterpret_cast<float*>(smem + LNB_G + WX_NS * WX_STAGE + 8 * LNB_EBW * 2);
  const float* gbuf = reinterpret_cast<const float*>(smem) + 4 * tid;
  float* ctab = red + 512;
  float* cells = ctab + 512;

  const int xcd = blockIdx.x & 7, j = blockIdx.x >> 3;
  const int n_streams = (int)gridDim.x;
  const int stream = j * 8 + xcd;
  const unsigned cpi = (unsigned)(p.n_points + WX_CH - 1) / WX_CH;
  const int n_chunks = p.n_items * (int)cpi;
  const int run = (n_chunks + n_streams - 1) / n_streams;
  const int q0 = stream * run, q_end = min(q0 + run, n_chunks);
  if (q0 >= q_end) return;

  s16x8 Wh[WX_K / 16], Wl[WX_K / 16];
  {
    const float* wrow = p.w + ((long long)(32 * wave + l31) * WX_K + 8 * h);
#pragma unroll
    for (int s = 0; s < WX_K / 16; ++s) {
      const f32x4 a0 = *reinterpret_cast<const f32x4*>(wrow + 16 * s), a1 = *reinterpret_cast<const f32x4*>(wrow + 16 * s + 4);
      s16x4 h0, l0, h1, l1;
      split4<Bf16x3>(a0, h0, l0);
      split4<Bf16x3>(a1, h1, l1);
      Wh[s] = join8(h0, h1);
      Wl[s] = join8(l0, l1);
    }
  }

  const int krow = tid >> 3, c4 = tid & 7;
  const int ld = p.ld;
  const unsigned x_voff = (unsigned)(2 * krow * ld + 4 * c4) * 4u;
  auto row_soff = [&](int i) { return (unsigned)(((i & 1) + 128 * (i >> 1)) * ld) * 4u; };
  struct Cursor { int q; unsigned item, tile; };
  auto cursor_at = [&](int q) { Cursor c; c.q = q; c.item = (unsigned)q / cpi; c.tile = (unsigned)q - c.item * cpi; return c; };
  auto advance = [&](Cursor& c) { ++c.q; if (++c.tile >= cpi) { c.tile = 0; ++c.item; } };
  auto locate = [&](const Cursor& c, int& col0, int& valid, unsigned& item) {
    const bool exists = c.q < q_end;
    col0 = exists ? (int)(c.tile * WX_CH) : 0;
    valid = exists ? min(WX_CH, p.n_points - col0) : 0;
    item = __builtin_amdgcn_readfirstlane(exists ? c.item : 0u);
  };
  auto issue_x = [&](const Cursor& cu, f32x4* R) {
    int col0, valid; unsigned item;
    locate(cu, col0, valid, item);
    const u32x4 Xr = wx_rsrc(p.xhat + (long long)(p.e_base + item) * p.eval_stride + col0, ((long long)(WX_K - 1) * ld + valid) * 4);
    const unsigned off = 4 * c4 < valid ? x_voff : CSN_OOB;
#pragma unroll
    for (int i = 0; i < 4; ++i) wx_request(R[i], Xr, off, row_soff(i));
    const u32x4 Sr = wx_rsrc(p.rstd + (long long)(p.e_base + item) * p.n_points + col0, (long long)valid * 4);
    wx_request(R[4], Sr, 4 * c4 < valid ? (unsigned)(16 * c4) : CSN_OOB, 0u);
  };
  const unsigned g_lds = __builtin_amdgcn_readfirstlane((unsigned)(unsigned long)((short __attribute__((address_space(3)))*)smem)) + (unsigned)wave * 1024u;
  auto issue_g = [&](const Cursor& cu) {
    int col0, valid; unsigned item;
    locate(cu, col0, valid, item);
    const unsigned e = (unsigned)p.e_base + item;
    const bool dense = RED || (int)e < p.n_dense;
    const unsigned src = p.dxhat_group > 1 ? e / (unsigned)p.dxhat_group : e;
    const u32x4 Gr = wx_rsrc(dense ? p.dxhat + (long long)src * p.eval_stride + col0 : nullptr, dense ? ((long long)(WX_K - 1) * ld + valid) * 4 : 0);
    const unsigned off = 4 * c4 < valid ? x_voff : CSN_OOB;
    asm volatile("s_waitcnt lgkmcnt(0)" ::: "memory");
#pragma unroll
    for (int i = 0; i < 4; ++i) wx_dma(g_lds + 8192u * i, Gr, off, row_soff(i));
  };

  const int grp = lane >> 4, gq = (lane >> 2) & 3, gp = lane & 3;
  const int tr_base = (8 * (grp >> 1) + gq) * WX_CH + 16 * (grp & 1) + 4 * gp;
  auto compute = [&](int stage) {
    f32x16 acc;
#pragma unroll
    for (int r = 0; r < 16; ++r) acc[r] = 0.f;
    const short* xh = xs + stage * WX_STAGE + tr_base;
    constexpr int WX_PD = 2, NSTEP = WX_K / 16;
    s16x8 bh[WX_PD], bl[WX_PD];
    auto rd = [&](int s, s16x8& fh, s16x8& fl) {
      const short* a = xh + 16 * s * WX_CH;
      fh = join8(__builtin_amdgcn_ds_read_tr16_b64_v4i16((lds_s16x4)(a)),
                 __builtin_amdgcn_ds_read_tr16_b64_v4i16((lds_s16x4)(a + 4 * WX_CH)));
      fl = join8(__builtin_amdgcn_ds_read_tr16_b64_v4i16((lds_s16x4)(a + WX_PLANE)),
                 __builtin_amdgcn_ds_read_tr16_b64_v4i16((lds_s16x4)(a + WX_PLANE + 4 * WX_CH)));
    };
    __builtin_amdgcn_sched_barrier(0);
#pragma unroll
    for (int s = 0; s < WX_PD; ++s) rd(s, bh[s], bl[s]);
    __builtin_amdgcn_sched_group_barrier(0x100, 4 * WX_PD, 0);
#pragma unroll
    for (int s = 0; s < NSTEP; ++s) {
      const int r = s % WX_PD;
      acc = wx_mma(Wh[s], Wl[s], bh[r], bl[r], acc);
      if (s + WX_PD < NSTEP) rd(s + WX_PD, bh[r], bl[r]);
      __builtin_amdgcn_sched_group_barrier(0x008, 3, 0);
      __builtin_amdgcn_sched_group_barrier(0x100, 4, 0);
    }
    __builtin_amdgcn_sched_barrier(0);
    return acc;
  };
  const int erow = lane >> 3, c8 = lane & 7;
  auto epilogue = [&](const Cursor& cu, const f32x16& acc) {
    int col0, valid; unsigned item;
    locate(cu, col0, valid, item);
    const bool n_ok = 4 * c8 < valid;
    const u32x4 Or = wx_rsrc(p.dctx + (long long)(p.e_base + item) * p.dctx_eval_stride, (long long)256 * ld * 4);
#pragma unroll
    for (int half = 0; half < 2; ++half) {
#pragma unroll
      for (int rr = 0; rr < 8; ++rr) eb[csn_acc_row(rr, h) * 32 + l31] = acc[8 * half + rr];
      const unsigned off = n_ok ? (unsigned)((32 * wave + 16 * half + erow) * ld + col0 + 4 * c8) * 4u : CSN_OOB;
#pragma unroll
      for (int t = 0; t < 2; ++t) {
        const f32x4 v = *reinterpret_cast<const f32x4*>(&eb[(erow + 8 * t) * 32 + 4 * c8]);
        wx_store4(v, Or, off, (unsigned)(8 * t * ld) * 4u);
      }
    }
  };

  const unsigned thr16 = csn_drop_threshold16(p.dropout_p);
  const float keep_scale = DROP ? 1.f / (1.f - p.dropout_p) : 1.f;
  unsigned cst_item = 0xffffffffu;
  unsigned red_item = 0xffffffffu;
  typedef float f32x2 __attribute__((ext_vector_type(2)));
  typedef f32x2 __attribute__((address_space(3))) * lds_f32x2;
  const unsigned smem_lds = (unsigned)(unsigned long)((short __attribute__((address_space(3)))*)smem);
  const unsigned cells_lds = (unsigned)(unsigned long)((float __attribute__((address_space(3)))*)cells);
  auto tid16 = [&]() {
    unsigned ga = (unsigned)(unsigned long)((const float __attribute__((address_space(3)))*)gbuf);
    asm volatile("" : "+v"(ga));
    return ga - smem_lds;
  };
  auto flush_red = [&]() __attribute__((always_inline)) {
    const unsigned slot = (unsigned)stream - (red_item * cpi) / (unsigned)run;
    const u32x4 Wr = wx_rsrc(p.red_ws + ((long long)red_item * p.red_slots + slot) * (2 * WX_K), 2 * WX_K * 4);
    const unsigned t16 = tid16();
    if ((t16 & 0x70u) == 0) {
      const unsigned cell = cells_lds + ((t16 >> 7) << 4), voff = (t16 >> 7) << 3;
#pragma unroll
      for (int i = 0; i < 4; ++i) {
        const lds_f32x2 c = (lds_f32x2)(unsigned long)(cell + 8 * (i & 1) + 1024 * (i >> 1));
        const f32x2 v = *c;
        *c = f32x2{0.f, 0.f};
        lnb_store1(v.x, Wr, voff + 4 * (i & 1) + 512 * (i >> 1));
        lnb_store1(v.y, Wr, voff + 4 * (i & 1) + 512 * (i >> 1) + 4 * WX_K);
      }
    }
  };
  if (RED && c4 == 0) {
#pragma unroll
    for (int i = 0; i < 4; ++i) *reinterpret_cast<float2*>(&cells[2 * (2 * krow + (i & 1) + 128 * (i >> 1))]) = make_float2(0.f, 0.f);
  }
  auto commit = [&](auto wait_c, int stage, f32x4* R, const Cursor& cu, const Cursor& cg) __attribute__((always_inline)) {
    int col0, valid; unsigned item;
    locate(cu, col0, valid, item);
    const unsigned e = (unsigned)p.e_base + item;
    const bool dense = RED || (int)e < p.n_dense;
    if (item != cst_item) {
      cst_item = item;
      if (tid < WX_K) {
        const float s = (dense && p.dxhat_scale) ? p.dxhat_scale[(long long)e * WX_K + tid] : 1.f;
        const float r = p.dxhat_rows ? p.dxhat_rows[(long long)e * WX_K + tid] : 0.f;
        *reinterpret_cast<float2*>(&ctab[2 * tid]) = make_float2(s, r);
      }
      __syncthreads();
    }
    const bool reduce = RED && cu.q < q_end;
    if (reduce && item != red_item) {
      if (red_item != 0xffffffffu) flush_red();
      red_item = item;
    }
    lnb_arrived<decltype(wait_c)::value>(R);
    if (reduce) {
      const unsigned t16 = tid16();
      const unsigned cell = cells_lds + ((t16 >> 7) << 4);
      const bool first_lane = (t16 & 0x70u) == 0;
      const bool in = (int)((t16 >> 2) & 0x1cu) < valid;
#pragma unroll
      for (int i = 0; i < 4; ++i) {
        const f32x4 g = *reinterpret_cast<const f32x4*>(gbuf + 2048 * i);
        float rd = fmaf(g[3], R[i][3], fmaf(g[2], R[i][2], fmaf(g[1], R[i][1], g[0] * R[i][0])));
        float rs = in ? (g[0] + g[1]) + (g[2] + g[3]) : 0.f;
        rd = lnb_sum_row_lanes(rd);
        rs = lnb_sum_row_lanes(rs);
        if (first_lane) {
          if (i == 0) asm volatile("ds_add_f32 %0, %1\n\tds_add_f32 %0, %2 offset:4" :: "v"(cell), "v"(rd), "v"(rs) : "memory");
          if (i == 1) asm volatile("ds_add_f32 %0, %1 offset:8\n\tds_add_f32 %0, %2 offset:12" :: "v"(cell), "v"(rd), "v"(rs) : "memory");
          if (i == 2) asm volatile("ds_add_f32 %0, %1 offset:1024\n\tds_add_f32 %0, %2 offset:1028" :: "v"(cell), "v"(rd), "v"(rs) : "memory");
          if (i == 3) asm volatile("ds_add_f32 %0, %1 offset:1032\n\tds_add_f32 %0, %2 offset:1036" :: "v"(cell), "v"(rd), "v"(rs) : "memory");
        }
      }
      __builtin_amdgcn_sched_barrier(0);
    }
    float sc[4], rw[4];
#pragma unroll
    for (int i = 0; i < 4; ++i) {
      const float2 c2 = *reinterpret_cast<const float2*>(&ctab[2 * (2 * krow + (i & 1) + 128 * (i >> 1))]);
      sc[i] = c2.x;
      rw[i] = c2.y;
    }
    f32x4 gx[4];
    f32x4 s1 = f32x4{0.f, 0.f, 0.f, 0.f}, s2 = s1;
#pragma unroll
    for (int i = 0; i < 4; ++i) {
      const f32x4 g = *reinterpret_cast<const f32x4*>(gbuf + 2048 * i);
#pragma unroll
      for (int jj = 0; jj < 4; ++jj) {
        gx[i][jj] = dense ? fmaf(g[jj], sc[i], rw[i]) : rw[i];
        s1[jj] += gx[i][jj];
        s2[jj] += gx[i][jj] * R[i][jj];
      }
    }
#pragma unroll
    for (int jj = 0; jj < 4; ++jj) {
      s1[jj] = lnb_sum_row_groups(s1[jj]);
      s2[jj] = lnb_sum_row_groups(s2[jj]);
    }
    if (lane < 8) {
      *reinterpret_cast<f32x4*>(&red[(wave * 2 + 0) * 32 + 4 * c4]) = s1;
      *reinterpret_cast<f32x4*>(&red[(wave * 2 + 1) * 32 + 4 * c4]) = s2;
    }
    {
      Cursor cn = cg;
      issue_g(cn);
    }
    __syncthreads();
    f32x4 m1 = f32x4{0.f, 0.f, 0.f, 0.f}, m2 = m1;
#pragma unroll
    for (int w = 0; w < 8; ++w) {
      m1 += *reinterpret_cast<const f32x4*>(&red[(w * 2 + 0) * 32 + 4 * c4]);
      m2 += *reinterpret_cast<const f32x4*>(&red[(w * 2 + 1) * 32 + 4 * c4]);
    }
    m1 *= (1.f / WX_K);
    m2 *= (1.f / WX_K);
    const f32x4 rs = R[4];
    const long long ebase = (long long)e * p.eval_stride;
    const u32x4 Zr = wx_rsrc(p.dz + ebase + col0, ((long long)(WX_K - 1) * ld + valid) * 4);
    const u32x4 Zres = wx_rsrc(RES ? p.dz_res + ebase + col0 : nullptr, RES ? ((long long)(WX_K - 1) * ld + valid) * 4 : 0);
    const unsigned off = 4 * c4 < valid ? x_voff : CSN_OOB;
#pragma unroll
    for (int i = 0; i < 4; ++i) {
#pragma unroll
      for (int jj = 0; jj < 4; ++jj) gx[i][jj] = rs[jj] * (gx[i][jj] - m1[jj] - R[i][jj] * m2[jj]);
      if constexpr (RES) wx_store4(gx[i], Zres, off, row_soff(i));
    }
    if constexpr (DROP) {
      const unsigned salt = csn_block_salt((unsigned long long)e, p.seed);
#pragma unroll
      for (int pr = 0; pr < 2; ++pr)
#pragma unroll
        for (int jj = 0; jj < 4; ++jj) {
          const unsigned hp = csn_fc_pair(2 * krow + 128 * pr, (unsigned)ld, (unsigned)(col0 + 4 * c4 + jj), salt);
          gx[2 * pr][jj] = csn_keep16(hp, 0, thr16) ? gx[2 * pr][jj] * keep_scale : 0.f;
          gx[2 * pr + 1][jj] = csn_keep16(hp, 1, thr16) ? gx[2 * pr + 1][jj] * keep_scale : 0.f;
        }
    }
    short* dst = xs + stage * WX_STAGE + 2 * krow * WX_CH + 4 * c4;
#pragma unroll
    for (int i = 0; i < 4; ++i) {
      wx_store4(gx[i], Zr, off, row_soff(i));
      s16x4 hi, lo;
      split4<Bf16x3>(gx[i], hi, lo);
      const int ro = ((i & 1) + 128 * (i >> 1)) * WX_CH;
      *reinterpret_cast<s16x4*>(dst + ro) = hi;
      *reinterpret_cast<s16x4*>(dst + ro + WX_PLANE) = lo;
    }
  };

  f32x4 R0[5], R1[5], R2[5];
  Cursor ci = cursor_at(q0), ce = ci, cc = ci, cg = ci;
  issue_x(ci, R0); advance(ci);
  issue_x(ci, R1); advance(ci);
  issue_g(cg); advance(cg);
  commit(std::integral_constant<int, 0>{}, 0, R0, cc, cg); advance(cc); advance(cg);
  issue_x(ci, R2); advance(ci);
  issue_x(ci, R0); advance(ci);
  __syncthreads();
  commit(std::integral_constant<int, 0>{}, 1, R1, cc, cg); advance(cc); advance(cg);
  __syncthreads();
  auto iteration = [&](auto st_c, f32x4* RQ, f32x4* RC) __attribute__((always_inline)) {
    constexpr int ST = decltype(st_c)::value;
    issue_x(ci, RQ); advance(ci);
    const f32x16 acc = compute(ST);
    epilogue(ce, acc); advance(ce);
    commit(std::integral_constant<int, (RES ? 8 : 4) + 5 + 4>{}, (ST + 2) % 3, RC, cc, cg); advance(cc); advance(cg);
    __syncthreads();
  };
  while (true) {
    if (ce.q >= q_end) break;
    iteration(std::integral_constant<int, 0>{}, R1, R2);
    if (ce.q >= q_end) break;
    iteration(std::integral_constant<int, 1>{}, R2, R0);
    if (ce.q >= q_end) break;
    iteration(std::integral_constant<int, 2>{}, R0, R1);
  }
  if (RED && red_item != 0xffffffffu) flush_red();
  asm volatile("s_waitcnt vmcnt(0)" ::: "memory");
}

__global__ __launch_bounds__(512) void csn_wx_lnb_sums_kernel(const float* __restrict__ ws, float* __restrict__ rowdot,
                                                              float* __restrict__ rowsum, int cpi, int run, int slots, int group) {
  const long long e = blockIdx.x;
  const int c = threadIdx.x & (WX_K - 1);
  const bool is_sum = threadIdx.x >= WX_K;
  if (is_sum && e % group != 0) return;
  const int first = (int)((e * cpi) / run), last = (int)(((e + 1) * cpi - 1) / run);
  const float* src = ws + e * slots * (2 * WX_K) + threadIdx.x;
  double s = 0.0;
  for (int k = 0; k <= last - first; ++k) s += (double)src[(long long)k * (2 * WX_K)];
  if (is_sum) rowsum[(e / group) * WX_K + c] = (float)s;
  else rowdot[e * WX_K + c] = (float)s;
}

}

bool csn_wx_lnb_takes(const CsnLnBwdArgs& a, int d_inner) {
  return (csn_dev_wx & 9) == 9 && a.C == WX_K && d_inner == WX_K && !a.act16 && !(a.ld & 3) && !(a.n_points & 3) && !(a.eval_stride & 3);
}

long long csn_wx_lnb_red_floats(int n_items, int n_points) {
  return n_items > 0 && n_points > 0 ? (long long)n_items * csn_wx_ln_sum_slots(n_items, n_points) * (2 * WX_K) : 0;
}

int csn_launch_wx_lnb(const CsnWxLnbArgs& a, hipStream_t st) {
  if (a.n_items <= 0 || a.n_points <= 0) return 0;
  if ((long long)a.n_items * ((a.n_points + WX_CH - 1) / WX_CH + 16) * 2 >= (1ll << 31)) return CSN_NOT_TAKEN;
  const int grid = wx_grid();
  if (a.red_ws) {
    if (!a.rowdot || !a.rowsum || a.e_base != 0 || a.n_items > a.n_dense || a.dxhat_group < 1 || a.n_items % a.dxhat_group) return -2;
    if (a.red_slots != csn_wx_ln_sum_slots(a.n_items, a.n_points)) return -2;
  }
  if (a.red_ws) {
    if (a.dz_res) hipLaunchKernelGGL((csn_wx_lnb_kernel<true, true, true>), dim3(grid), dim3(512), 0, st, a);
    else hipLaunchKernelGGL((csn_wx_lnb_kernel<true, false, true>), dim3(grid), dim3(512), 0, st, a);
  } else if (a.dz_res) hipLaunchKernelGGL((csn_wx_lnb_kernel<true, true, false>), dim3(grid), dim3(512), 0, st, a);
  else hipLaunchKernelGGL((csn_wx_lnb_kernel<true, false, false>), dim3(grid), dim3(512), 0, st, a);
  if (a.red_ws) {
    const int cpi = (a.n_points + WX_CH - 1) / WX_CH;
    const int run = (int)(((long long)a.n_items * cpi + grid - 1) / grid);
    hipLaunchKernelGGL(csn_wx_lnb_sums_kernel, dim3(a.n_items), dim3(512), 0, st, a.red_ws, a.rowdot, a.rowsum, cpi, run, a.red_slots,
                       a.dxhat_group);
  }
  return (int)hipGetLastError();
}
```

csn_amd/functional.py:

```python
from __future__ import annotations

import math
from dataclasses import dataclass
from typing import Optional, Tuple

import torch

from . import _lib, tuning

REF_BLOCK = 500
REF_NBLOCKS = 20
LN_EPS = 1e-6
RESCALE_THRESHOLD = 8.0


def draw_seeds(n: int):
    seeds = torch.randint(0, 2 ** 62, (n,)).tolist()
    if torch.distributed.is_available() and torch.distributed.is_initialized():
        salt = (torch.distributed.get_rank() * 0x9E3779B97F4A7C15) & (2 ** 62 - 1)
        seeds = [s ^ salt for s in seeds]
    return seeds


def _ptr(t: Optional[torch.Tensor]):
# ... 138 lines not shown

    def __init__(self, mode):
        self.mode = mode_id(mode)

    def __enter__(self):
        if self.mode is not None:
            L = _lib.lib()
            self.prev = L.csn_get_thread_math_mode()
            _lib.check(L.csn_set_thread_math_mode(self.mode))
        return self

    def __exit__(self, *exc):
        if self.mode is not None:
            _lib.lib().csn_set_thread_math_mode(self.prev)
        return False


class act16:

    def __init__(self, fmt: int):
        self.fmt = int(fmt)

    def __enter__(self):
        L = _lib.lib()
        self.prev = L.csn_get_thread_act16()
        _lib.check(L.csn_set_thread_act16(self.fmt))
        return self

    def __exit__(self, *exc):
        _lib.lib().csn_set_thread_act16(self.prev)
        return False


class rows16:

    def __init__(self, flag):
        self.flag = int(bool(flag))

    def __enter__(self):
        L = _lib.lib()
        self.prev = L.csn_get_thread_rows16()
        _lib.check(L.csn_set_thread_rows16(self.flag))
        return self

    def __exit__(self, *exc):
        _lib.lib().csn_set_thread_rows16(self.prev)
        return False


class score_layout:

    def __init__(self, layout: int):
        self.layout = layout

    def __enter__(self):
        L = _lib.lib()
        self.prev = L.csn_get_thread_score_layout()
        _lib.check(L.csn_set_thread_score_layout(self.layout))
        return self

    def __exit__(self, *exc):
        _lib.lib().csn_set_thread_score_layout(self.prev)
        return False


def _score_flow(mode: int, d: int, T: int) -> int:
# ... 89 lines not shown
        with math_mode(mode), act16(ctx.a16):
            return _MHAEvals._forward(ctx, x_all, w_qs, w_ks, w_vs, w_fc, plan, geo, keep_scores, p_attn, p_fc, n_head_evals,
                                      want_sums, link)

    @staticmethod
    def _forward(ctx, x_all, w_qs, w_ks, w_vs, w_fc, plan, geo, keep_scores, p_attn, p_fc, n_head_evals, want_sums, link):
        seed_attn, seed_fc = draw_seeds(2) if (p_attn > 0 or p_fc > 0) else (0, 0)
        q_slots, kv_slots, v_shift = plan.q_slots, plan.kv_slots, plan.v_shift
        L = _lib.lib()
        S, C, NP = x_all.shape
        H, d, D = geo.n_head, geo.d_head, geo.d_inner
        assert NP == geo.n_points and x_all.is_contiguous()
        assert S == plan.S
        E = plan.E
        T, nb, Tp = geo.block, geo.n_blocks, geo.score_pitch
        NPP = geo.n_padded
        if not (0 < NP <= NPP and NPP - NP < T and NP % 4 == 0):
            raise _lib.CsnError(f"{NP} points do not fill {nb} blocks of {T} (the last block may be short; counts are multiples of 4)")
        dev = x_all.device
        temperature = geo.temperature or float(d) ** 0.5
        w_qkv = torch.cat((w_qs, w_ks, w_vs), dim=0).contiguous()
        w_fc_in = w_fc.contiguous()
        a16 = ctx.a16
        fwd16 = {0: torch.float32, 1: torch.bfloat16, 2: torch.float16}[a16]
        att = torch.empty((E, D, NP), device=dev, dtype=fwd16)
        lse = torch.empty((E, H, NPP), device=dev, dtype=torch.float32)
        tiles = fast_math() and tuning.current().kv_tiles and T <= 512
        tune = tuning.current()
        fold = bool(tune.takes_fold() and ctx.mode == 1 and H == 1 and C == d == D == 256 and tiles and not a16
                    and tuple(w_fc.shape) == (C, D)
                    and plan.v_shift == 0 and not x_all.requires_grad
                    and _score_flow(ctx.mode, d, T) == tuning.KEEP_SCORES and L.csn_attn_bwd_dq_no_planes_available(d, T))
        ctx.fold = fold
        w_fv = w_fv_t = None
        if fold:
            ldp = nb * 1024
            w_m, w_fv, w_fv_t = (torch.empty((C, C), device=dev, dtype=torch.float32) for _ in range(3))
            ws_n = int(L.csn_fold_workspace_floats(D, C))
            ws = torch.empty((ws_n,), device=dev, dtype=torch.float32)
            _lib.check(L.csn_fold_weights_f32(_ptr(w_qkv), _ptr(w_qkv[D:]), _ptr(w_qkv[2 * D:]), _ptr(w_fc.contiguous()), D, C,
                                              temperature, _ptr(w_m), _ptr(w_fv), _ptr(w_fv_t), _ptr(ws), ws_n, _stream()),
                       "csn_fold_weights_f32")
            del ws
            qkv = torch.empty((S, D, NP), device=dev, dtype=torch.float32)
            kv = torch.empty((S, C, ldp), device=dev, dtype=torch.bfloat16)
            for first, step, count in (plan.q_ranges or [(0, 1, S)]):
                _lib.check(L.csn_project_f32(x_all.data_ptr() + 4 * first * C * NP, step * C * NP, NP, _ptr(w_m), D, C,
                                             qkv.data_ptr() + 4 * first * D * NP, step * D * NP, NP, count, NP, 0, 1.0, 0, 0,
                                             _stream()), "csn_project_f32")
            for first, step, count in (plan.kv_ranges or [(0, 1, S)]):
                _lib.check(L.csn_tile_planes_f32(x_all.data_ptr() + 4 * first * C * NP, step * C * NP, NP,
                                                 kv.data_ptr() + 2 * first * C * ldp, step * C * ldp, ldp, count, C, NP, T,
                                                 _stream()), "csn_tile_planes_f32")
            q_ptr, q_stride = qkv.data_ptr(), D * NP
            k_ptr, kv_stride = kv.data_ptr(), C * ldp
            v_ptr = k_ptr
            kv_flag, kv_pitch = 1, ldp
        elif tiles:
            npl = planes()
            ldp = nb * 512 * npl
            qkv = torch.empty((S, D, NP), device=dev, dtype=fwd16)
            kv_dtype = torch.float16 if ctx.mode == 3 else torch.bfloat16
            kv = torch.empty((S, 2 * D, ldp), device=dev, dtype=kv_dtype)
            one_pass = plan.q_ranges is None and plan.kv_ranges is None and not a16 and tuning.current().qkv_one_pass
            if one_pass:
                _lib.check(L.csn_project_qkv_f32(_ptr(x_all), C * NP, NP, _ptr(w_qkv), D, C, _ptr(qkv), D * NP, NP, _ptr(kv),
# ... 28 lines not shown
            kv_flag, kv_pitch = 0, 0
        flow = _score_flow(ctx.mode, d, T) if (keep_scores and tiles) else tuning.KEEP_SCORES
        scores = torch.empty((E, H, nb, T, Tp), device=dev, dtype=torch.float32) if (keep_scores and flow == tuning.KEEP_SCORES) else None
        tune = tuning.current()
        ctx.sc_layout = 1 if (scores is not None and tiles and ctx.mode == 1 and tune.tile_major_scores and tune.grouped_dq and
                              tune.grouped_dkv and Tp >= (T + 31) // 32 * 32 and (L.csn_attn_bwd_grouping(d, T) & 19) == 19) else 0
        with score_layout(ctx.sc_layout):
            if tune.grouped_fwd and fast_math() and plan.n_q_groups < E:
                _lib.check(L.csn_block_attn_fwd_grouped_f32(q_ptr, k_ptr, v_ptr, q_stride, kv_stride,
                                                            _ptr(q_slots), _ptr(kv_slots), NP, _ptr(att), D * NP, _ptr(scores),
                                                            _ptr(lse), E, H, d, T, nb, Tp, RESCALE_THRESHOLD, p_attn, seed_attn,
                                                            kv_flag, kv_pitch, _ptr(plan.q_group_items), _ptr(plan.q_group_off),
                                                            plan.n_q_groups, _stream()),
                           "csn_block_attn_fwd_grouped_f32")
            else:
                _lib.check(L.csn_block_attn_fwd_f32(q_ptr, k_ptr, v_ptr, q_stride, kv_stride,
                                                    _ptr(q_slots), _ptr(kv_slots), NP, _ptr(att), D * NP, _ptr(scores),
                                                    _ptr(lse), E, H, d, T, nb, Tp, RESCALE_THRESHOLD, p_attn, seed_attn,
                                                    kv_flag, kv_pitch, _stream()),
                           "csn_block_attn_fwd_f32")
        xhat = torch.empty((E, C, NP), device=dev, dtype=torch.float16 if a16 else torch.float32)
        rstd = torch.empty((E, NP), device=dev, dtype=torch.float32)
        w_fc = w_fv if fold else w_fc.contiguous()
        sums = torch.empty((E, C), device=dev, dtype=torch.float32) if want_sums else None
        sum_ws_n = int(L.csn_outproj_ln_workspace_floats(E, C, D, NP)) if (want_sums and tuning.current().fused_point_sums) else 0
        sum_ws = torch.empty((sum_ws_n,), device=dev, dtype=torch.float32) if sum_ws_n else None
        _lib.check(L.csn_outproj_ln_fwd_f32(_ptr(att), D * NP, _ptr(w_fc), _ptr(x_all), C * NP, _ptr(q_slots),
                                            _ptr(xhat), C * NP, _ptr(rstd), E, C, D, NP, NP, LN_EPS, p_fc, seed_fc,
                                            _ptr(sums), _ptr(sum_ws), sum_ws_n, _stream()),
                   "csn_outproj_ln_fwd_f32")
        del sum_ws
        if (keep_scores and link is not None and not a16 and tuning.current().fused_mix_bwd and plan.mixed_not_pooled
                and n_head_evals > 0):
            link.pre = (xhat, rstd, w_fc, p_fc, seed_fc, n_head_evals, ctx.mode, bool(x_all.requires_grad), w_fv_t)
        if keep_scores:
            ctx.save_for_backward(x_all, w_qkv, w_fc, None if fold else qkv, att, lse, scores, xhat, rstd, kv, w_fv_t,
                                  w_fc_in if fold else None)
            ctx.flow = flow
            ctx.geo = geo
            ctx.plan = plan
            ctx.drop = (p_attn, seed_attn, p_fc, seed_fc)
            ctx.ptrs = (q_stride, kv_stride, kv_flag, kv_pitch)
        ctx.n_head = n_head_evals
        handle = x_all.new_zeros(1) if link is not None else None
        if a16:
            head = xhat[:n_head_evals]
            ctx.mark_non_differentiable(xhat, head)
            return xhat, head, sums, handle
        return xhat, xhat[:n_head_evals], sums, handle

    @staticmethod
    def backward(ctx, dxhat, dhead, dsums=None, dhandle=None):
        with math_mode(backward_mode(ctx.mode)):
            g16 = 0
            if ctx.a16:
                geo, tune = ctx.geo, ctx.tune
                grouping = _lib.lib().csn_attn_bwd_grouping(geo.d_head, geo.block)
                dq_once = ctx.flow != tuning.KEEP_SCORES or (tune.grouped_dq and (grouping & 1))
                dkv_once = ctx.flow == tuning.FLASH or (tune.grouped_dkv and (grouping & 2))
                g16 = 4 if (dq_once and dkv_once) else 0
            ctx.g16 = g16
            with act16(ctx.a16 + g16), score_layout(getattr(ctx, "sc_layout", 0)):
                return _MHAEvals._backward(ctx, dxhat, dhead, dsums, dhandle)

    @staticmethod
    def _backward(ctx, dxhat, dhead, dsums=None, dhandle=None):
        x_all, w_qkv, w_fc, qkv, att, lse, scores, xhat, rstd, kv, w_fv_t, w_fc_in = ctx.saved_tensors
# ... 17 lines not shown
            dxhat[:ctx.n_head] += dhead
            dhead = None
        dense = dxhat if dxhat is not None else dhead
        n_dense = 0 if dense is None else dense.shape[0]
        dense = None if dense is None else dense.contiguous()
        scale, group = None, 1
        link, ctx.link = ctx.link, None
        head_done = None
        if link is not None:
            head_done, link.head_done, link.pre = link.head_done, None, None
        if dhandle is not None and link is not None and link.dfeats is not None:
            if dense is None:
                dense, scale, group, n_dense = link.dfeats, link.scale, link.group, ctx.n_head
            else:
                head_done = None
                dense = dense.clone() if dense.shape[0] == E else torch.cat(
                    (dense, dense.new_zeros((E - dense.shape[0],) + tuple(dense.shape[1:]))), dim=0)
                dense[:ctx.n_head] += link.scale[:, :, None] * link.dfeats.repeat_interleave(link.group, dim=0)[:ctx.n_head]
                n_dense = E
            link.dfeats = link.scale = None
        else:
            head_done = None
        temperature = geo.temperature or float(d) ** 0.5
        p_attn, seed_attn, p_fc, seed_fc = ctx.drop
        need_dx = ctx.needs_input_grad[0]

        a16 = ctx.a16
        bwd16 = torch.bfloat16 if a16 else torch.float32
        dw_fc = torch.empty((C, D), device=dev, dtype=torch.float32)
        ws_n = L.csn_wgrad_workspace_floats(C, D, E, NP)
        ws = torch.empty((ws_n,), device=dev, dtype=torch.float32)
        if head_done is not None:
            dz, dz_res, datt, w_fc_t = head_done
            if E > ctx.n_head:
                _lib.check(L.csn_outproj_lnb_f32(_ptr(dense), _ptr(xhat), _ptr(rstd), C * NP, _ptr(w_fc_t), _ptr(dz), _ptr(dz_res),
                                                 _ptr(datt), ctx.n_head, E - ctx.n_head, C, D, NP, NP, p_fc, seed_fc, _ptr(rows),
                                                 n_dense, _ptr(scale), group, None, None, None, 0, _stream()),
                           "csn_outproj_lnb_f32")
            _lib.check(L.csn_project_wgrad_f32(_ptr(dz), C * NP, NP, _ptr(att), D * NP, NP, _ptr(dw_fc), C, D, E, NP, 1.0, 0,
                                               _ptr(ws), ws_n, _stream()), "csn_project_wgrad_f32")
        else:
            dz = torch.empty((E, C, NP), device=dev, dtype=bwd16)
            dz_res = torch.empty((E, C, NP), device=dev, dtype=torch.float32) if (need_dx and (p_fc > 0 or a16)) else None
            datt = torch.empty((E, D, NP), device=dev, dtype=bwd16)
            w_fc_t = w_fv_t if ctx.fold else w_fc.t().contiguous()
            _lib.check(L.csn_outproj_ln_bwd_f32(_ptr(dense), _ptr(xhat), _ptr(rstd), C * NP, _ptr(att), D * NP,
                                                _ptr(w_fc_t), _ptr(dz), _ptr(dz_res), _ptr(datt), _ptr(dw_fc), _ptr(ws), ws_n,
                                                E, C, D, NP, NP, 0, p_fc, seed_fc, 0, 0, _ptr(rows), n_dense, _ptr(scale), group,
                                                _stream()),
                       "csn_outproj_ln_bwd_f32")
        del ws

        if ctx.fold:
            g = torch.empty((S, D, NP), device=dev, dtype=torch.float32)
            if plan.q_ranges is None and plan.q_unwritten.numel():
                g.index_fill_(0, plan.q_unwritten, 0.0)
            q_stride, kv_stride, kv_flag, kv_pitch = ctx.ptrs
            if ctx.tune.grouped_dq and (L.csn_attn_bwd_grouping(d, T) & 1):
                launches = [(0, plan.q_group_items, E, plan.q_group_off, plan.n_q_groups)]
            else:
                launches = [(0 if ci == 0 else 1, ids, ids.numel(), None, 0) for ci, ids in enumerate(plan.dq_colors)]
            L.csn_dev_set(_lib.DEV_KV_SAME, int(bool(ctx.tune.kv_same)))
            for accumulate, ids, n_ids, off, n_groups in launches:
                _lib.check(L.csn_block_attn_bwd_dq_f32(_ptr(datt), _ptr(att), D * NP, _ptr(kv), _ptr(kv), kv_stride,
                                                       _ptr(plan.kv_slots), NP, _ptr(scores), None, _ptr(lse), None,
                                                       _ptr(g), D * NP, _ptr(plan.q_slots), accumulate, _ptr(ids), n_ids, H, d, T,
                                                       nb, Tp, p_attn, seed_attn, 0, 0, kv_flag, kv_pitch, 3, _ptr(off), n_groups,
                                                       _stream()), "csn_block_attn_bwd_dq_f32")
            del datt
            if plan.q_ranges is None:
                d_m = project_wgrad(g, x_all)
            else:
                d_m = torch.empty((D, C), device=dev, dtype=torch.float32)
                for i, (first, step, count) in enumerate(plan.q_ranges):
                    ws_n = L.csn_wgrad_workspace_floats(D, C, count, NP)
                    ws = torch.empty((ws_n,), device=dev, dtype=torch.float32)
                    _lib.check(L.csn_project_wgrad_f32(g.data_ptr() + 4 * first * D * NP, step * D * NP, NP,
                                                       x_all.data_ptr() + 4 * first * C * NP, step * C * NP, NP, _ptr(d_m), D, C,
                                                       count, NP, 1.0, 0 if i == 0 else 1, _ptr(ws), ws_n, _stream()),
                               "csn_project_wgrad_f32")
            del g
            dw_qkv = torch.empty((3 * D, C), device=dev, dtype=torch.float32)
            dw_fc_in = torch.empty((C, D), device=dev, dtype=torch.float32)
            ws = torch.empty((D * C,), device=dev, dtype=torch.float32)
            _lib.check(L.csn_unfold_wgrads_f32(_ptr(d_m), _ptr(dw_fc), _ptr(w_qkv), _ptr(w_qkv[D:]), _ptr(w_qkv[2 * D:]),
                                               _ptr(w_fc_in), D, C, temperature, _ptr(dw_qkv), _ptr(dw_qkv[D:]),
                                               _ptr(dw_qkv[2 * D:]), _ptr(dw_fc_in), _ptr(ws), D * C, _stream()),
                       "csn_unfold_wgrads_f32")
            return (None, dw_qkv[:D], dw_qkv[D:2 * D], dw_qkv[2 * D:], dw_fc_in, None, None, None, None, None, None, None, None)
        flow = ctx.flow
        pt = 1 if (fast_math() and Tp >= (T + 31) // 32 * 32) else 0
        if flow == tuning.KEEP_SCORES:
            dscores = torch.empty_like(scores)
        else:
            assert pt == 1 and scores is None
            shape = (E, H, nb, T, Tp)
            travel = flow == tuning.RECOMPUTE_DQ
            scores = torch.empty(shape, device=dev, dtype=torch.float32) if (travel and planes() == 2) else None
            dscores = torch.empty(shape, device=dev, dtype=torch.float32) if travel else None
        delta = torch.empty((E, H, geo.n_padded), device=dev, dtype=torch.float32)
        dqkv = torch.empty((S, 3 * D, NP), device=dev, dtype=torch.bfloat16 if ctx.g16 else torch.float32)
# ... 86 lines not shown
            for rows0, nrows, ranges in ((0, D, plan.q_ranges), (D, 2 * D, plan.kv_ranges)):
                for i, (first, step, count) in enumerate(ranges):
                    ws_n = L.csn_wgrad_workspace_floats(nrows, C, count, NP)
                    ws = torch.empty((ws_n,), device=dev, dtype=torch.float32)
                    _lib.check(L.csn_project_wgrad_f32(dqkv.data_ptr() + ges * (first * 3 * D + rows0) * NP, step * 3 * D * NP, NP,
                                                       x_all.data_ptr() + 4 * first * C * NP, step * C * NP, NP,
                                                       dw_qkv.data_ptr() + 4 * rows0 * C, nrows, C, count, NP, 1.0,
                                                       0 if i == 0 else 1, _ptr(ws), ws_n, _stream()), "csn_project_wgrad_f32")
        else:
            dw_qkv = project_wgrad(dqkv, x_all)
        dw_q = dw_qkv[:D] / temperature
        dw_k, dw_v = dw_qkv[D:2 * D], dw_qkv[2 * D:]

        dx_all = None
        if need_dx:
            dqkv[:, :D] /= temperature
            dx_all = project(dqkv, w_qkv.t().contiguous())
            dx_all.index_add_(0, plan.q_slots.long(), dz if dz_res is None else dz_res)
        return dx_all, dw_q, dw_k, dw_v, dw_fc, None, None, None, None, None, None, None, None


class MixLink:
    __slots__ = ("dfeats", "scale", "group", "pre", "head_done")

    def __init__(self):
        self.dfeats = self.scale = None
        self.group = 1
        self.pre = self.head_done = None


def _lnb_head(link: MixLink, dfeats: torch.Tensor, scale: torch.Tensor, group: int):
    if link is None or link.pre is None:
        return None
    xhat, rstd, w_fc, p_fc, seed_fc, n, mode, need_dx, w_fc_t = link.pre
    E, C, NP = xhat.shape
    D = w_fc.shape[1]
    L = _lib.lib()
    dev = xhat.device
    with math_mode(backward_mode(mode)), act16(0):
        if n % group or L.csn_outproj_lnb_workspace_floats(E, C, D, NP, NP) <= 0:
            return None
        ws_n = int(L.csn_outproj_lnb_workspace_floats(n, C, D, NP, NP))
        red_ws = torch.empty((ws_n,), device=dev, dtype=torch.float32)
        rowdot = torch.empty((n, C), device=dev, dtype=torch.float32)
        rowsum = torch.empty((n // group, C), device=dev, dtype=torch.float32)
        dz = torch.empty((E, C, NP), device=dev, dtype=torch.float32)
        dz_res = torch.empty((E, C, NP), device=dev, dtype=torch.float32) if (need_dx and p_fc > 0) else None
        datt = torch.empty((E, D, NP), device=dev, dtype=torch.float32)
        if w_fc_t is None:
            w_fc_t = w_fc.t().contiguous()
        _lib.check(L.csn_outproj_lnb_f32(_ptr(dfeats), _ptr(xhat), _ptr(rstd), C * NP, _ptr(w_fc_t), _ptr(dz), _ptr(dz_res),
                                         _ptr(datt), 0, n, C, D, NP, NP, p_fc, seed_fc, None, n, _ptr(scale), group, _ptr(rowdot),
                                         _ptr(rowsum), _ptr(red_ws), ws_n, _stream()), "csn_outproj_lnb_f32")
    link.head_done = (dz, dz_res, datt, w_fc_t)
    return rowdot, rowsum


class LinkedMaps:
    __slots__ = ("maps", "handle", "link")

    def __init__(self, maps, handle, link):
        self.maps, self.handle, self.link = maps, handle, link


def mha_evals(x_all: torch.Tensor, w_qs: torch.Tensor, w_ks: torch.Tensor, w_vs: torch.Tensor, w_fc: torch.Tensor,
              plan: EvalPlan, geo: MHAGeometry, p_attn: float = 0.0, p_fc: float = 0.0, n_head_evals: int = 0,
              want_sums: bool = False, link_mix: bool = False):
    keep = torch.is_grad_enabled() and any(t.requires_grad for t in (x_all, w_qs, w_ks, w_vs, w_fc))
    link = MixLink() if (link_mix and tuning.current().link_mix and keep and n_head_evals > 0) else None
    xhat, head, sums, handle = _MHAEvals.apply(x_all, w_qs, w_ks, w_vs, w_fc, plan, geo, keep, float(p_attn), float(p_fc),
                                               int(n_head_evals), bool(want_sums), link)
    if link is not None:
        head = LinkedMaps(head.detach(), handle, link)
    out = (xhat, head) if n_head_evals > 0 else (xhat,)
    if want_sums:
        out = out + (sums,)
    return out if len(out) > 1 else out[0]


class _LinearCM(torch.autograd.Function):

    @staticmethod
    def forward(ctx, x, w):
        _need_cuda(x, w)
        ctx.save_for_backward(x, w)
        ctx.mode = current_mode()
# ... 224 lines not shown
```

csn_amd/tuning.py:

```python
from __future__ import annotations

import contextlib
from dataclasses import dataclass, field, fields, replace
from typing import Dict, Optional

KEEP_SCORES = 0
RECOMPUTE_DQ = 1
FLASH = 2


@dataclass
class Tuning:
    kv_tiles: bool = True
    fused_point_sums: bool = True
    link_mix: bool = True
    fused_mix_bwd: bool = True
    grouped_dkv: bool = True
    grouped_dq: bool = True
    grouped_fwd: bool = True
    fused_compat_head: bool = True
    act16: bool = True
    tile_major_scores: bool = False
    qkv_one_pass: bool = False
    dv_from_scores: bool = True
    folded_projections: bool = True
    kv_same: bool = True
    named: frozenset = frozenset()
    score_flow: Dict[object, int] = field(default_factory=lambda: {
        1: KEEP_SCORES,
        2: RECOMPUTE_DQ,
        **{(2, d): FLASH for d in (32, 64, 96, 128)},
        **{(1, d): FLASH for d in (32, 64, 96)}, (1, 128): RECOMPUTE_DQ})

    cross_score_free: Optional[bool] = None
    cross_score_budget: Optional[int] = None
    native_kernel_maps: bool = False
    rows_single_product: bool = False
    eval_epilogue: bool = False
    infer_maps16: bool = False
    octant_single_product: bool = False
    unet_maps16: bool = False
    unet_fused_tail: bool = False
    retrieval_screen: bool = False

    grouped_passes: bool = False
    train_maps16: bool = False

    def flow_for(self, mode: int, d_head: int) -> int:
        return self.score_flow.get((mode, d_head), self.score_flow.get(mode, KEEP_SCORES))

    def takes_fold(self) -> bool:
        return self.folded_projections and not (self.named & UNFOLDED_ONLY)


UNFOLDED_ONLY = frozenset({"dv_from_scores", "grouped_dkv", "qkv_one_pass"})


def cross_takes_score_free(score_bytes: int, budget: int, available: bool) -> bool:
    return bool(available) and score_bytes > budget
# ... 23 lines not shown
```

include/csn_hip.h:

```cpp
#ifndef CSN_HIP_H
#define CSN_HIP_H

#ifdef __cplusplus
extern "C" {
#endif

#define CSN_ABI_VERSION 17
#define CSN_API __attribute__((visibility("default")))

#define CSN_MATH_FP32 0
#define CSN_MATH_BF16X3 1
#define CSN_MATH_BF16 2
#define CSN_MATH_FP16 3

#define CSN_E_ARG (-1)
#define CSN_E_ALIGN (-2)
#define CSN_E_PTR (-3)
#define CSN_E_STRIDE (-4)
#define CSN_E_DIM (-5)
#define CSN_E_WORKSPACE (-6)

CSN_API int csn_version(void);
CSN_API int csn_set_thread_act16(int fmt);
CSN_API int csn_get_thread_act16(void);
// ... 328 lines not shown
CSN_API int csn_octant_down_stats_fwd_f32(const float* x, long long ld_x, int n_fine, const int* children, int n_coarse, int c_in,
                                  int c_out, const float* w, float* z, long long ld_z, float* mean, float* invstd,
                                  float* running_mean, float* running_var, float eps, float momentum, void* ws, long long ws_bytes,
                                  void* stream);
CSN_API int csn_octant_up_stats_fwd_f32(const float* x, long long ld_x, int n_coarse, const int* parent, const int* order,
                                const int* seg, int n_fine, int c_in, int c_out, const float* w, float* z, long long ld_z,
                                float* mean, float* invstd, float* running_mean, float* running_var, float eps, float momentum,
                                void* ws, long long ws_bytes, void* stream);

typedef struct CsnCatParts {
  const float* x[4];
  long long ld_x[4];
  int c_in[4];
} CsnCatParts;
CSN_API long long csn_sparse_conv_cat_stats_workspace_bytes(int n_out, int c_out);
CSN_API int csn_sparse_conv_cat_stats_fwd_f32(const CsnCatParts* parts, int n_parts, int n_in, const int* table, int n_out, int kv,
                                      int c_out, const float* w, float* z, long long ld_z, float* mean, float* invstd,
                                      float* running_mean, float* running_var, float eps, float momentum, void* ws,
                                      long long ws_bytes, void* stream);

CSN_API int csn_sparse_conv_stats_fwd_t16(const void* x, int x16, long long ld_x, int n_in, const int* table, int n_out, int kv, int c_in,
                                  int c_out, const float* w, float* z, long long ld_z, float* mean, float* invstd,
                                  float* running_mean, float* running_var, float eps, float momentum, void* ws, long long ws_bytes,
                                  void* stream);
CSN_API int csn_rows_bn_act_fwd_t16(const CsnBnTerms* terms, int n_terms, int n_rows, int channels, int training, float eps,
                            const void* r, int r16, long long ld_r, int relu, void* y, int y16, long long ld_y, void* stream);
CSN_API int csn_rows_bn_act_bwd_t16(const float* dy, long long ld_dy, const void* y, int y16, long long ld_y, const CsnBnTerms* terms,
                            int n_terms, int n_rows, int channels, int training, float eps, int relu, float* dr, long long ld_dr,
                            void* ws, long long ws_bytes, void* stream);
CSN_API int csn_sparse_conv_bwd_t16(const float* dy, long long ld_dy, const void* x, int x16, long long ld_x, int n_in, int n_out, int kv,
                            int c_in, int c_out, const int* fwd_table, const int* bwd_table, const float* w, float* dx,
                            long long ld_dx, float* dw, float* dbias, void* ws, long long ws_bytes, void* stream);

#define CSN_DEV_BIG_TILES 0
#define CSN_DEV_WIDE_GEMM 1
#define CSN_DEV_WIDE_FORMS 2
#define CSN_DEV_WX 3
#define CSN_DEV_LNB_GROUP 5
#define CSN_DEV_SCONV_NB 7
#define CSN_DEV_KV_SAME 8
CSN_API int csn_dev_set(int key, int value);
CSN_API int csn_dev_get(int key);

#ifdef __cplusplus
}
#endif
#endif
```

Baseline: 18.14 million points/s.

## Emit dctx as pre-split bf16 operand planes for the attention dq backward

The fused LN-backward kernel now writes the attention output gradient directly as hi/lo bf16 planes in the tile-ordered layout that the bf16x3 dq-backward kernel consumes. The attention kernel then loads these planes with buffer loads instead of staging fp32 rows through shared memory and splitting them. This is meant to remove an fp32 round trip, the in-kernel split and a barrier. In exchange it adds a new layout contract between the two kernels, restricted to d=256, H=1 and dz_res-free paths, and a thread-local mode toggle.

```diff
diff --git a/csn_amd/_lib.py b/csn_amd/_lib.py
--- a/csn_amd/_lib.py
+++ b/csn_amd/_lib.py
@@ -11,7 +11,7 @@
 _CSRC = os.path.join(_HERE, "csrc")
 LIB_PATH = os.path.join(_HERE, "libcsn_hip.so")
 SOURCES = ["gemm_f32.hip", "gemm_bf16x3.hip", "wx_stream.hip", "wx_lnb.hip", "loss.hip", "attn_f32.hip", "attn_bf16x3.hip", "attn_dkv.hip", "attn_dv_scores.hip", "fold.hip", "outproj_ln.hip", "retrieval.hip", "retrieval_screen.hip", "combine.hip", "compat.hip", "minkowski_csn.hip", "minkowski_seg.hip", "rows_fc.hip", "sparse_conv.hip", "sparse_conv_maps16.hip", "train_maps16.hip", "sparse_conv_cat.hip", "octant_conv.hip", "octant_conv_maps16.hip", "octant_conv_stats.hip", "rows_bn_act.hip", "point_field.hip", "kernel_map.hip", "octant_map.hip", "points.hip", "csn_capi.hip"]
-HEADERS = ["csn_common.h", "csn_kernels.h", "csn_window.h", "wx_common.h", "rows_mma.h", "sconv_gemm_body.inc", "sconv_a16_body.inc", "rows_bn_act_body.inc", "octant_rows_body.inc", os.path.join("..", "..", "include", "csn_hip.h")]
+HEADERS = ["csn_common.h", "csn_kernels.h", "csn_window.h", "wx_common.h", "wx_lnb_body.inc", "rows_mma.h", "sconv_gemm_body.inc", "sconv_a16_body.inc", "rows_bn_act_body.inc", "octant_rows_body.inc", os.path.join("..", "..", "include", "csn_hip.h")]
 ARCH = "gfx950"
 BUILD_FLAGS = [f"--offload-arch={ARCH}", "-O3", "-std=c++17", "-fPIC", "-fvisibility=hidden", "-shared"]
 
@@ -205,6 +205,9 @@
     "csn_outproj_lnb_f32": (c_int, [c_void_p, c_void_p, c_void_p, c_longlong, c_void_p, c_void_p, c_void_p, c_void_p, c_int, c_int,
                                     c_int, c_int, c_int, c_int, c_float, c_ulonglong, c_void_p, c_int, c_void_p, c_int, c_void_p,
                                     c_void_p, c_void_p, c_longlong, c_void_p]),
+    "csn_operand_planes_elements": (c_longlong, [c_int, c_int, c_int, c_int, c_int, c_int]),
+    "csn_set_thread_operand_planes": (c_int, [c_int]),
+    "csn_get_thread_operand_planes": (c_int, []),
     "csn_project_wgrad_f32": (c_int, [c_void_p, c_longlong, c_int, c_void_p, c_longlong, c_int, c_void_p, c_int, c_int,
                                       c_int, c_int, c_float, c_int, c_void_p, c_longlong, c_void_p]),
     "csn_retrieval_measure_f32": (c_int, [c_void_p, c_void_p, c_void_p, c_int, c_int, c_int, c_int, c_int, c_void_p,
@@ -339,7 +342,7 @@
 }
 
 EXPORTS = tuple(_SIGNATURES)
-DEV_BIG_TILES, DEV_WIDE_GEMM, DEV_WIDE_FORMS, DEV_WX, DEV_LNB_GROUP, DEV_SCONV_NB, DEV_KV_SAME = 0, 1, 2, 3, 5, 7, 8
+DEV_BIG_TILES, DEV_WIDE_GEMM, DEV_WIDE_FORMS, DEV_WX, DEV_LNB_GROUP, DEV_SCONV_NB, DEV_KV_SAME, DEV_OPERAND_PLANES = 0, 1, 2, 3, 5, 7, 8, 9
 DEV_WX_DEFAULT = 9
 
 
diff --git a/csn_amd/csrc/attn_bf16x3.hip b/csn_amd/csrc/attn_bf16x3.hip
--- a/csn_amd/csrc/attn_bf16x3.hip
+++ b/csn_amd/csrc/attn_bf16x3.hip
@@ -31,9 +31,10 @@
 constexpr int csn_attn_waves(int npl, int dt, bool bwd, bool rc_f32 = false) {
   return (!rc_f32 && ((npl == 1 ? dt <= 3 : dt <= 2) || csn_attn_x3fwd96(npl, dt, bwd))) ? 4 : 2;
 }
-template <typename PR, int DT, bool BWD, bool KVP, bool RC = false, int NOP = 0, bool KV_SAME = false>
+template <typename PR, int DT, bool BWD, bool KVP, bool RC = false, int NOP = 0, bool KV_SAME = false, bool ROP = false>
 __global__ __launch_bounds__(512, csn_attn_waves(PR::NPL, DT, BWD, RC && !KVP)) void csn_attn_bf16x3_kernel(CsnAttnArgs p) {
   static_assert(!KV_SAME || (DT == 8 && NOP == 2), "one request per tile: the folded d = 256 backward");
+  static_assert(!ROP || (DT == 8 && NOP == 2 && PR::NT == 3), "operand planes: the folded d = 256 backward");
   static_assert(PR::NT == 3 || KVP, "single-product modes take K / V as tile planes");
   static_assert(!RC || BWD, "score recomputation: backward kernel");
   static_assert(!NOP || (BWD && KVP && !RC && PR::NPL == 2), "no P planes: the kept-scores backward in two planes");
@@ -206,7 +207,17 @@
     }
   };
   auto pick = [&](int row) { return xbuf[row * 128 + ((((col >> 2) ^ (4 * ((row >> 3) & 1))) << 2) | (col & 3))]; };
-  float rv[D / 4];
+  float rv[ROP ? 1 : D / 4];
+  if constexpr (ROP) {
+    const int G = 8 * QT;
+    const csn_rsrc_t Pr = csn_make_rsrc(reinterpret_cast<const short*>(p.q) + qs * p.r_opl_stride + ((long long)blk * G + 8 * qt + __builtin_amdgcn_readfirstlane(wave)) * 8192, 16384);
+    const unsigned p_off = q_ok ? (unsigned)(lane * 16) : CSN_OOB;
+#pragma unroll
+    for (int s = 0; s < D / 32; ++s) {
+      Rh[s] = __builtin_bit_cast(s16x8, csn_bload4(Pr, p_off, (unsigned)(2048 * s)));
+      Rl[s] = __builtin_bit_cast(s16x8, csn_bload4(Pr, p_off, (unsigned)(2048 * s + 1024)));
+    }
+  } else
   if (BWD || it == it0) {
     stage_in(Rr, p.r_fmt);
     __syncthreads();
@@ -230,13 +241,18 @@
   float delta_q = 0.f;
   if (BWD) {
     const csn_rsrc_t Xr = map_rsrc(p.ctx, qs * p.q_shape_stride + head_off, p.ctx_fmt);
-    __syncthreads();
+    if constexpr (!ROP) __syncthreads();
     stage_in(Xr, p.ctx_fmt);
     __syncthreads();
 #pragma unroll
     for (int s = 0; s < D / 32; ++s)
 #pragma unroll
-      for (int j = 0; j < 8; ++j) delta_q = fmaf(rv[8 * s + j], pick(32 * s + 8 * kq + j), delta_q);
+      for (int j = 0; j < 8; ++j) {
+        float dv;
+        if constexpr (ROP) dv = from16<false>(Rh[s][j]) + from16<false>(Rl[s][j]);
+        else dv = rv[8 * s + j];
+        delta_q = fmaf(dv, pick(32 * s + 8 * kq + j), delta_q);
+      }
     delta_q += __shfl_xor(delta_q, 16, 64);
     delta_q += __shfl_xor(delta_q, 32, 64);
   }
@@ -608,6 +624,15 @@
           else return -1;
         } else if (a.sc_tiles == 3) {
           if constexpr (csn_attn_dv_scores_fits(PR::NT == 3 ? 1 : 2, 32 * DT)) {
+            if constexpr (DT == 8 && PR::NT == 3) {
+              if (a.r_opl) {
+                if (a.H != 1) return -1;
+                if (a.kv_same) hipLaunchKernelGGL((csn_attn_bf16x3_kernel<PR, DT, true, true, false, 2, true, true>), grid, dim3(512), 0, st, a);
+                else hipLaunchKernelGGL((csn_attn_bf16x3_kernel<PR, DT, true, true, false, 2, false, true>), grid, dim3(512), 0, st, a);
+                return (int)hipGetLastError();
+              }
+            }
+            if (a.r_opl) return -1;
             if (a.kv_same) hipLaunchKernelGGL((csn_attn_bf16x3_kernel<PR, DT, true, true, false, 2, true>), grid, dim3(512), 0, st, a);
             else hipLaunchKernelGGL((csn_attn_bf16x3_kernel<PR, DT, true, true, false, 2>), grid, dim3(512), 0, st, a);
           } else return -1;
@@ -641,6 +666,7 @@
   if (a.q2 && !a.kv_planes && (a.sc_tiles || a.grp_off)) return -1;
   if ((a.r_fmt || a.ctx_fmt || a.q2_fmt || a.out_fmt) && (PR::NPL != 1 || !a.kv_planes)) return -1;
   if (a.out_fmt && a.accumulate) return -1;
+  if (a.r_opl && (!bwd || a.sc_tiles != 3 || d != 256 || PR::NT != 3 || a.H != 1 || a.r_opl_stride < csn_opl_eval_elements(a.T, a.n_blocks))) return -1;
   if (a.kv_planes && (a.T > 512 || (a.kv_ld & 7) || (a.kv_shape_stride & 7))) return -2;
   switch (d) {
     case 32: return launch_dt<PR, 1>(a, bwd, st);
diff --git a/csn_amd/csrc/csn_capi.hip b/csn_amd/csrc/csn_capi.hip
--- a/csn_amd/csrc/csn_capi.hip
+++ b/csn_amd/csrc/csn_capi.hip
@@ -16,6 +16,7 @@
 thread_local int t_rows16 = 0;
 inline int rows_mode() { return mode() >= 2 && !t_rows16 ? 1 : mode(); }
 thread_local int t_score_layout = 0;
+thread_local int t_operand_planes = 0;
 inline int planes_of(int m) { return m == 1 ? 2 : 1; }
 
 struct ModeGuard {
@@ -99,6 +100,8 @@
 
 }
 
+static int g_dev_operand_planes = 1;
+
 extern "C" {
 
 int csn_version(void) { return CSN_ABI_VERSION; }
@@ -112,6 +115,7 @@
     case CSN_DEV_LNB_GROUP: return csn_dev_lnb_group;
     case CSN_DEV_SCONV_NB: return csn_dev_sconv_nb;
     case CSN_DEV_KV_SAME: return csn_dev_kv_same;
+    case CSN_DEV_OPERAND_PLANES: return g_dev_operand_planes;
     default: return CSN_E_ARG;
   }
 }
@@ -134,6 +138,10 @@
       if (value != 0 && value != 1) return CSN_E_ARG;
       csn_dev_kv_same = value;
       break;
+    case CSN_DEV_OPERAND_PLANES:
+      if (value != 0 && value != 1) return CSN_E_ARG;
+      g_dev_operand_planes = value;
+      break;
     default: return CSN_E_ARG;
   }
   return prev;
@@ -157,6 +165,12 @@
   return 0;
 }
 int csn_get_thread_act16(void) { return t_act16; }
+int csn_set_thread_operand_planes(int block) {
+  if (block != 0 && (block < 32 || block > 512 || (block & 3))) return CSN_E_ARG;
+  t_operand_planes = block;
+  return 0;
+}
+int csn_get_thread_operand_planes(void) { return t_operand_planes; }
 int csn_set_thread_rows16(int on) {
   if (on != 0 && on != 1) return CSN_E_ARG;
   t_rows16 = on;
@@ -444,7 +458,11 @@
                             unsigned long long seed, int dctx_split, long long dctx_plane_stride, int kv_split,
                             long long kv_plane_stride, int probs_tiles, int block_q, int ld_kv, const int* group_offsets,
                             int n_groups, void* stream, const int* tq_arr = nullptr, const int* t_arr = nullptr,
-                            const float* q = nullptr, long long q_shape_stride = 0, const int* q_index = nullptr) {
+                            const float* q = nullptr, long long q_shape_stride = 0, const int* q_index = nullptr,
+                            long long opl_stride = 0 ) {
+  if (opl_stride && (probs_tiles != 3 || mode() != 1 || d_head != 256 || n_heads != 1 || kv_split != 1 || block < 32 ||
+                     opl_stride < csn_opl_eval_elements(block, n_blocks) || opl_stride * 2 > 0x7fffffffLL || (opl_stride & 7)))
+    return CSN_E_ARG;
   if (block_q < 0 || ld_kv < 0 || (ld_kv & 3)) return CSN_E_ARG;
   if (q && (block_q != 0 || !kv_split || !(csn_attn_bwd_grouping(d_head, block) & 4) || mis16(q))) return CSN_E_ARG;
   if (q && (q_shape_stride & 3)) return CSN_E_STRIDE;
@@ -497,6 +515,7 @@
   a.kv_f16 = kv_split == 2;
   a.sc_tiles = probs_tiles;
   if (kv_split == 1 && k == v && mode() == 1 && d_head == 256 && probs_tiles == 3) a.kv_same = csn_dev_kv_same;
+  if (opl_stride) { a.r_opl = 1; a.r_opl_stride = opl_stride; }
   a.tq_arr = tq_arr; a.t_arr = t_arr;
   a.q2 = q; a.q2_shape_stride = q_shape_stride; a.q2_index = q_index;
   if (t_score_layout) {
@@ -522,10 +541,12 @@
                               unsigned long long seed, int dctx_split, long long dctx_plane_stride, int kv_split,
                               long long kv_plane_stride, int probs_tiles, const int* group_offsets, int n_groups,
                               void* stream) {
+  if (t_operand_planes && (t_operand_planes != block || n_blocks <= 0)) return CSN_E_ARG;
+  const long long opl_stride = t_operand_planes ? csn_opl_eval_elements(block, n_blocks) : 0;
   return attn_bwd_dq_impl(dctx, ctx, ctx_eval_stride, k, v, kv_shape_stride, kv_index, ld, scores, dscores, lse, delta, dq,
                           dq_slot_stride, dq_index, accumulate, eval_ids, n_launch_evals, n_heads, d_head, block, n_blocks,
                           score_pitch, dropout_p, seed, dctx_split, dctx_plane_stride, kv_split, kv_plane_stride, probs_tiles,
-                          0, 0, group_offsets, n_groups, stream);
+                          0, 0, group_offsets, n_groups, stream, nullptr, nullptr, nullptr, 0, nullptr, opl_stride);
 }
 
 int csn_block_attn_bwd_dq_recompute_f32(const float* dctx, const float* ctx, long long ctx_eval_stride, const float* q,
@@ -537,7 +558,7 @@
                                         int score_pitch, float dropout_p, unsigned long long seed,
                                         long long kv_plane_stride, int kv_f16, int probs_tiles, const int* group_offsets,
                                         int n_groups, void* stream) {
-  if (!q) return CSN_E_ARG;
+  if (!q || t_operand_planes) return CSN_E_ARG;
   return attn_bwd_dq_impl(dctx, ctx, ctx_eval_stride, k, v, kv_shape_stride, kv_index, ld, probs, dscores, lse, delta, dq,
                           dq_slot_stride, dq_index, accumulate, eval_ids, n_launch_evals, n_heads, d_head, block, n_blocks,
                           score_pitch, dropout_p, seed, 0, 0, kv_f16 ? 2 : 1, kv_plane_stride, probs_tiles, 0, 0, group_offsets,
@@ -914,6 +935,7 @@
                            void* stream) {
   if (dropout_p < 0.f || dropout_p >= 1.f) return CSN_E_ARG;
   if (dxhat_group < 0) return CSN_E_ARG;
+  if (t_operand_planes && (dz_res || dctx_split || d_model != 256 || d_inner != 256)) return CSN_E_ARG;
   if (dropout_p > 0.f && (long long)(d_model / 2 + 1) * ld >= (1ll << 32)) return CSN_E_ARG;
   if (dctx_split && mode() == 0) return CSN_E_ARG;
   if (n_dense_evals < 0 || n_dense_evals > n_evals || (n_dense_evals > 0 && !dxhat)) return CSN_E_ARG;
@@ -938,6 +960,7 @@
       csn_wx_geometry_takes(csn_dev_lnb_group > 0 && csn_dev_lnb_group < n_evals ? csn_dev_lnb_group : n_evals, n_points, d_inner / 256)) {
     const int G = csn_dev_lnb_group > 0 ? csn_dev_lnb_group : n_evals;
     const bool fused = csn_wx_lnb_takes(l, d_inner) && eval_stride == ctx_eval_stride;
+    if (t_operand_planes && !fused) return CSN_E_DIM;
     for (int e0 = 0; e0 < n_evals && !rc; e0 += G) {
       const int ng = n_evals - e0 < G ? n_evals - e0 : G;
       if (fused) {
@@ -946,7 +969,14 @@
         f.dxhat = dxhat; f.dxhat_group = l.dxhat_group; f.n_dense = n_dense_evals; f.dxhat_scale = dxhat_scale; f.dxhat_rows = dxhat_rows;
         f.dz = dz; f.dz_res = dz_res; f.dctx = dctx; f.dctx_eval_stride = ctx_eval_stride;
         f.n_items = ng; f.n_points = n_points; f.e_base = e0; f.dropout_p = dropout_p; f.seed = seed;
+        if (t_operand_planes) {
+          f.dctx = nullptr; f.dctx_planes = reinterpret_cast<short*>(dctx);
+          f.opl_block = t_operand_planes; f.opl_groups = csn_opl_groups(t_operand_planes);
+          f.opl_eval_stride = csn_opl_eval_elements(t_operand_planes, (n_points + t_operand_planes - 1) / t_operand_planes);
+          if (f.opl_eval_stride * 2 > 0x7fffffffLL) return CSN_E_DIM;
+        }
         rc = csn_launch_wx_lnb(f, st);
+        if (rc == CSN_NOT_TAKEN && t_operand_planes) return CSN_E_DIM;
         if (rc != CSN_NOT_TAKEN) continue;
       }
       l.e_base = e0; l.E = ng;
@@ -959,6 +989,7 @@
     return wgrad(dz, eval_stride, ld, ctx, ctx_eval_stride, ld, dwfc, d_model, d_inner, n_evals, n_points, 1.f, accumulate, ws,
                  ws_floats, st, 0, 0);
   }
+  if (t_operand_planes) return CSN_E_DIM;
   rc = csn_launch_ln_bwd_f32(l, st);
   if (rc) return rc;
   CsnGemmArgs g;
@@ -1012,10 +1043,25 @@
   f.w = wfc_t; f.xhat = xhat; f.rstd = rstd; f.eval_stride = eval_stride; f.ld = ld;
   f.dxhat = dxhat; f.dxhat_group = group; f.n_dense = n_dense_evals; f.dxhat_scale = dxhat_scale; f.dxhat_rows = dxhat_rows;
   f.dz = dz; f.dz_res = dz_res; f.dctx = dctx; f.dctx_eval_stride = eval_stride;
+  if (t_operand_planes) {
+    if (dz_res || d_model != 256 || d_inner != 256) return CSN_E_ARG;
+    f.dctx = nullptr; f.dctx_planes = reinterpret_cast<short*>(dctx);
+    f.opl_block = t_operand_planes; f.opl_groups = csn_opl_groups(t_operand_planes);
+    f.opl_eval_stride = csn_opl_eval_elements(t_operand_planes, (n_points + t_operand_planes - 1) / t_operand_planes);
+    if (f.opl_eval_stride * 2 > 0x7fffffffLL) return CSN_E_DIM;
+  }
   f.n_items = n_evals; f.n_points = n_points; f.e_base = e_base; f.dropout_p = dropout_p; f.seed = seed;
   if (reduce) { f.red_ws = red_ws; f.red_slots = csn_wx_ln_sum_slots(n_evals, n_points); f.rowdot = rowdot; f.rowsum = rowsum; }
   const int rc = csn_launch_wx_lnb(f, (hipStream_t)stream);
   return rc == CSN_NOT_TAKEN ? CSN_E_DIM : rc;
+}
+
+long long csn_operand_planes_elements(int n_evals, int d_model, int d_inner, int ld, int n_points, int block) {
+  if (!g_dev_operand_planes || d_model != 256 || d_inner != 256 || block < 32 || block > 512 || (block & 3)) return 0;
+  if (!lnb_range_takes(n_evals, d_model, d_inner, ld, n_points, (long long)d_model * ld)) return 0;
+  if (!csn_attn_bwd_dv_scores_available(256, block)) return 0;
+  const long long el = csn_opl_eval_elements(block, (n_points + block - 1) / block);
+  return el * 2 > 0x7fffffffLL ? 0 : el;
 }
 
 int csn_project_wgrad_f32(const float* dout, long long dout_shape_stride, int ld_dout, const float* x,
diff --git a/csn_amd/csrc/csn_kernels.h b/csn_amd/csrc/csn_kernels.h
--- a/csn_amd/csrc/csn_kernels.h
+++ b/csn_amd/csrc/csn_kernels.h
@@ -93,6 +93,7 @@
   int r_fmt = 0, ctx_fmt = 0, q2_fmt = 0, out_fmt = 0;
   int sc_layout = 0;
   int kv_same = 0;
+  int r_opl = 0; long long r_opl_stride = 0;
 };
 extern int csn_dev_kv_same;
 constexpr bool csn_attn_recompute_fits(int planes, int dt) { return planes == 1 || dt <= 4; }
@@ -189,7 +190,10 @@
   int n_items, n_points, e_base;
   float dropout_p; unsigned long long seed;
   float* red_ws; int red_slots; float* rowdot; float* rowsum;
-};
+  short* dctx_planes = nullptr; int opl_block = 0, opl_groups = 0; long long opl_eval_stride = 0;
+};
+constexpr int csn_opl_groups(int block) { return 8 * ((block + 127) / 128); }
+constexpr long long csn_opl_eval_elements(int block, int n_blocks) { return (long long)n_blocks * csn_opl_groups(block) * 8192; }
 long long csn_wx_lnb_red_floats(int n_items, int n_points);
 bool csn_wx_lnb_takes(const CsnLnBwdArgs& a, int d_inner);
 int csn_launch_wx_lnb(const CsnWxLnbArgs& a, hipStream_t st);
diff --git a/csn_amd/csrc/wx_lnb.hip b/csn_amd/csrc/wx_lnb.hip
--- a/csn_amd/csrc/wx_lnb.hip
+++ b/csn_amd/csrc/wx_lnb.hip
@@ -34,307 +34,16 @@
   return v;
 }
 
-template <bool DROP, bool RES, bool RED>
-__global__ __launch_bounds__(512, 2) void csn_wx_lnb_kernel(CsnWxLnbArgs p) {
-  __shared__ __attribute__((aligned(16))) short smem[LNB_G + WX_NS * WX_STAGE + 8 * LNB_EBW * 2 + 1024 + 1024 + 1024];
-  short* xs = smem + LNB_G;
-  const int tid = threadIdx.x, lane = tid & 63, wave = __builtin_amdgcn_readfirstlane(tid >> 6);
-  const int l31 = lane & 31, h = lane >> 5;
-  float* eb = reinterpret_cast<float*>(smem + LNB_G + WX_NS * WX_STAGE) + wave * LNB_EBW;
-  float* red = reinterpret_cast<float*>(smem + LNB_G + WX_NS * WX_STAGE + 8 * LNB_EBW * 2);
-  const float* gbuf = reinterpret_cast<const float*>(smem) + 4 * tid;
-  float* ctab = red + 512;
-  float* cells = ctab + 512;
-
-  const int xcd = blockIdx.x & 7, j = blockIdx.x >> 3;
-  const int n_streams = (int)gridDim.x;
-  const int stream = j * 8 + xcd;
-  const unsigned cpi = (unsigned)(p.n_points + WX_CH - 1) / WX_CH;
-  const int n_chunks = p.n_items * (int)cpi;
-  const int run = (n_chunks + n_streams - 1) / n_streams;
-  const int q0 = stream * run, q_end = min(q0 + run, n_chunks);
-  if (q0 >= q_end) return;
-
-  s16x8 Wh[WX_K / 16], Wl[WX_K / 16];
-  {
-    const float* wrow = p.w + ((long long)(32 * wave + l31) * WX_K + 8 * h);
-#pragma unroll
-    for (int s = 0; s < WX_K / 16; ++s) {
-      const f32x4 a0 = *reinterpret_cast<const f32x4*>(wrow + 16 * s), a1 = *reinterpret_cast<const f32x4*>(wrow + 16 * s + 4);
-      s16x4 h0, l0, h1, l1;
-      split4<Bf16x3>(a0, h0, l0);
-      split4<Bf16x3>(a1, h1, l1);
-      Wh[s] = join8(h0, h1);
-      Wl[s] = join8(l0, l1);
-    }
-  }
-
-  const int krow = tid >> 3, c4 = tid & 7;
-  const int ld = p.ld;
-  const unsigned x_voff = (unsigned)(2 * krow * ld + 4 * c4) * 4u;
-  auto row_soff = [&](int i) { return (unsigned)(((i & 1) + 128 * (i >> 1)) * ld) * 4u; };
-  struct Cursor { int q; unsigned item, tile; };
-  auto cursor_at = [&](int q) { Cursor c; c.q = q; c.item = (unsigned)q / cpi; c.tile = (unsigned)q - c.item * cpi; return c; };
-  auto advance = [&](Cursor& c) { ++c.q; if (++c.tile >= cpi) { c.tile = 0; ++c.item; } };
-  auto locate = [&](const Cursor& c, int& col0, int& valid, unsigned& item) {
-    const bool exists = c.q < q_end;
-    col0 = exists ? (int)(c.tile * WX_CH) : 0;
-    valid = exists ? min(WX_CH, p.n_points - col0) : 0;
-    item = __builtin_amdgcn_readfirstlane(exists ? c.item : 0u);
-  };
-  auto issue_x = [&](const Cursor& cu, f32x4* R) {
-    int col0, valid; unsigned item;
-    locate(cu, col0, valid, item);
-    const u32x4 Xr = wx_rsrc(p.xhat + (long long)(p.e_base + item) * p.eval_stride + col0, ((long long)(WX_K - 1) * ld + valid) * 4);
-    const unsigned off = 4 * c4 < valid ? x_voff : CSN_OOB;
-#pragma unroll
-    for (int i = 0; i < 4; ++i) wx_request(R[i], Xr, off, row_soff(i));
-    const u32x4 Sr = wx_rsrc(p.rstd + (long long)(p.e_base + item) * p.n_points + col0, (long long)valid * 4);
-    wx_request(R[4], Sr, 4 * c4 < valid ? (unsigned)(16 * c4) : CSN_OOB, 0u);
-  };
-  const unsigned g_lds = __builtin_amdgcn_readfirstlane((unsigned)(unsigned long)((short __attribute__((address_space(3)))*)smem)) + (unsigned)wave * 1024u;
-  auto issue_g = [&](const Cursor& cu) {
-    int col0, valid; unsigned item;
-    locate(cu, col0, valid, item);
-    const unsigned e = (unsigned)p.e_base + item;
-    const bool dense = RED || (int)e < p.n_dense;
-    const unsigned src = p.dxhat_group > 1 ? e / (unsigned)p.dxhat_group : e;
-    const u32x4 Gr = wx_rsrc(dense ? p.dxhat + (long long)src * p.eval_stride + col0 : nullptr, dense ? ((long long)(WX_K - 1) * ld + valid) * 4 : 0);
-    const unsigned off = 4 * c4 < valid ? x_voff : CSN_OOB;
-    asm volatile("s_waitcnt lgkmcnt(0)" ::: "memory");
-#pragma unroll
-    for (int i = 0; i < 4; ++i) wx_dma(g_lds + 8192u * i, Gr, off, row_soff(i));
-  };
-
-  const int grp = lane >> 4, gq = (lane >> 2) & 3, gp = lane & 3;
-  const int tr_base = (8 * (grp >> 1) + gq) * WX_CH + 16 * (grp & 1) + 4 * gp;
-  auto compute = [&](int stage) {
-    f32x16 acc;
-#pragma unroll
-    for (int r = 0; r < 16; ++r) acc[r] = 0.f;
-    const short* xh = xs + stage * WX_STAGE + tr_base;
-    constexpr int WX_PD = 2, NSTEP = WX_K / 16;
-    s16x8 bh[WX_PD], bl[WX_PD];
-    auto rd = [&](int s, s16x8& fh, s16x8& fl) {
-      const short* a = xh + 16 * s * WX_CH;
-      fh = join8(__builtin_amdgcn_ds_read_tr16_b64_v4i16((lds_s16x4)(a)),
-                 __builtin_amdgcn_ds_read_tr16_b64_v4i16((lds_s16x4)(a + 4 * WX_CH)));
-      fl = join8(__builtin_amdgcn_ds_read_tr16_b64_v4i16((lds_s16x4)(a + WX_PLANE)),
-                 __builtin_amdgcn_ds_read_tr16_b64_v4i16((lds_s16x4)(a + WX_PLANE + 4 * WX_CH)));
-    };
-    __builtin_amdgcn_sched_barrier(0);
-#pragma unroll
-    for (int s = 0; s < WX_PD; ++s) rd(s, bh[s], bl[s]);
-    __builtin_amdgcn_sched_group_barrier(0x100, 4 * WX_PD, 0);
-#pragma unroll
-    for (int s = 0; s < NSTEP; ++s) {
-      const int r = s % WX_PD;
-      acc = wx_mma(Wh[s], Wl[s], bh[r], bl[r], acc);
-      if (s + WX_PD < NSTEP) rd(s + WX_PD, bh[r], bl[r]);
-      __builtin_amdgcn_sched_group_barrier(0x008, 3, 0);
-      __builtin_amdgcn_sched_group_barrier(0x100, 4, 0);
-    }
-    __builtin_amdgcn_sched_barrier(0);
-    return acc;
-  };
-  const int erow = lane >> 3, c8 = lane & 7;
-  auto epilogue = [&](const Cursor& cu, const f32x16& acc) {
-    int col0, valid; unsigned item;
-    locate(cu, col0, valid, item);
-    const bool n_ok = 4 * c8 < valid;
-    const u32x4 Or = wx_rsrc(p.dctx + (long long)(p.e_base + item) * p.dctx_eval_stride, (long long)256 * ld * 4);
-#pragma unroll
-    for (int half = 0; half < 2; ++half) {
-#pragma unroll
-      for (int rr = 0; rr < 8; ++rr) eb[csn_acc_row(rr, h) * 32 + l31] = acc[8 * half + rr];
-      const unsigned off = n_ok ? (unsigned)((32 * wave + 16 * half + erow) * ld + col0 + 4 * c8) * 4u : CSN_OOB;
-#pragma unroll
-      for (int t = 0; t < 2; ++t) {
-        const f32x4 v = *reinterpret_cast<const f32x4*>(&eb[(erow + 8 * t) * 32 + 4 * c8]);
-        wx_store4(v, Or, off, (unsigned)(8 * t * ld) * 4u);
-      }
-    }
-  };
-
-  const unsigned thr16 = csn_drop_threshold16(p.dropout_p);
-  const float keep_scale = DROP ? 1.f / (1.f - p.dropout_p) : 1.f;
-  unsigned cst_item = 0xffffffffu;
-  unsigned red_item = 0xffffffffu;
-  typedef float f32x2 __attribute__((ext_vector_type(2)));
-  typedef f32x2 __attribute__((address_space(3))) * lds_f32x2;
-  const unsigned smem_lds = (unsigned)(unsigned long)((short __attribute__((address_space(3)))*)smem);
-  const unsigned cells_lds = (unsigned)(unsigned long)((float __attribute__((address_space(3)))*)cells);
-  auto tid16 = [&]() {
-    unsigned ga = (unsigned)(unsigned long)((const float __attribute__((address_space(3)))*)gbuf);
-    asm volatile("" : "+v"(ga));
-    return ga - smem_lds;
-  };
-  auto flush_red = [&]() __attribute__((always_inline)) {
-    const unsigned slot = (unsigned)stream - (red_item * cpi) / (unsigned)run;
-    const u32x4 Wr = wx_rsrc(p.red_ws + ((long long)red_item * p.red_slots + slot) * (2 * WX_K), 2 * WX_K * 4);
-    const unsigned t16 = tid16();
-    if ((t16 & 0x70u) == 0) {
-      const unsigned cell = cells_lds + ((t16 >> 7) << 4), voff = (t16 >> 7) << 3;
-#pragma unroll
-      for (int i = 0; i < 4; ++i) {
-        const lds_f32x2 c = (lds_f32x2)(unsigned long)(cell + 8 * (i & 1) + 1024 * (i >> 1));
-        const f32x2 v = *c;
-        *c = f32x2{0.f, 0.f};
-        lnb_store1(v.x, Wr, voff + 4 * (i & 1) + 512 * (i >> 1));
-        lnb_store1(v.y, Wr, voff + 4 * (i & 1) + 512 * (i >> 1) + 4 * WX_K);
-      }
-    }
-  };
-  if (RED && c4 == 0) {
-#pragma unroll
-    for (int i = 0; i < 4; ++i) *reinterpret_cast<float2*>(&cells[2 * (2 * krow + (i & 1) + 128 * (i >> 1))]) = make_float2(0.f, 0.f);
-  }
-  auto commit = [&](auto wait_c, int stage, f32x4* R, const Cursor& cu, const Cursor& cg) __attribute__((always_inline)) {
-    int col0, valid; unsigned item;
-    locate(cu, col0, valid, item);
-    const unsigned e = (unsigned)p.e_base + item;
-    const bool dense = RED || (int)e < p.n_dense;
-    if (item != cst_item) {
-      cst_item = item;
-      if (tid < WX_K) {
-        const float s = (dense && p.dxhat_scale) ? p.dxhat_scale[(long long)e * WX_K + tid] : 1.f;
-        const float r = p.dxhat_rows ? p.dxhat_rows[(long long)e * WX_K + tid] : 0.f;
-        *reinterpret_cast<float2*>(&ctab[2 * tid]) = make_float2(s, r);
-      }
-      __syncthreads();
-    }
-    const bool reduce = RED && cu.q < q_end;
-    if (reduce && item != red_item) {
-      if (red_item != 0xffffffffu) flush_red();
-      red_item = item;
-    }
-    lnb_arrived<decltype(wait_c)::value>(R);
-    if (reduce) {
-      const unsigned t16 = tid16();
-      const unsigned cell = cells_lds + ((t16 >> 7) << 4);
-      const bool first_lane = (t16 & 0x70u) == 0;
-      const bool in = (int)((t16 >> 2) & 0x1cu) < valid;
-#pragma unroll
-      for (int i = 0; i < 4; ++i) {
-        const f32x4 g = *reinterpret_cast<const f32x4*>(gbuf + 2048 * i);
-        float rd = fmaf(g[3], R[i][3], fmaf(g[2], R[i][2], fmaf(g[1], R[i][1], g[0] * R[i][0])));
-        float rs = in ? (g[0] + g[1]) + (g[2] + g[3]) : 0.f;
-        rd = lnb_sum_row_lanes(rd);
-        rs = lnb_sum_row_lanes(rs);
-        if (first_lane) {
-          if (i == 0) asm volatile("ds_add_f32 %0, %1\n\tds_add_f32 %0, %2 offset:4" :: "v"(cell), "v"(rd), "v"(rs) : "memory");
-          if (i == 1) asm volatile("ds_add_f32 %0, %1 offset:8\n\tds_add_f32 %0, %2 offset:12" :: "v"(cell), "v"(rd), "v"(rs) : "memory");
-          if (i == 2) asm volatile("ds_add_f32 %0, %1 offset:1024\n\tds_add_f32 %0, %2 offset:1028" :: "v"(cell), "v"(rd), "v"(rs) : "memory");
-          if (i == 3) asm volatile("ds_add_f32 %0, %1 offset:1032\n\tds_add_f32 %0, %2 offset:1036" :: "v"(cell), "v"(rd), "v"(rs) : "memory");
-        }
-      }
-      __builtin_amdgcn_sched_barrier(0);
-    }
-    float sc[4], rw[4];
-#pragma unroll
-    for (int i = 0; i < 4; ++i) {
-      const float2 c2 = *reinterpret_cast<const float2*>(&ctab[2 * (2 * krow + (i & 1) + 128 * (i >> 1))]);
-      sc[i] = c2.x;
-      rw[i] = c2.y;
-    }
-    f32x4 gx[4];
-    f32x4 s1 = f32x4{0.f, 0.f, 0.f, 0.f}, s2 = s1;
-#pragma unroll
-    for (int i = 0; i < 4; ++i) {
-      const f32x4 g = *reinterpret_cast<const f32x4*>(gbuf + 2048 * i);
-#pragma unroll
-      for (int jj = 0; jj < 4; ++jj) {
-        gx[i][jj] = dense ? fmaf(g[jj], sc[i], rw[i]) : rw[i];
-        s1[jj] += gx[i][jj];
-        s2[jj] += gx[i][jj] * R[i][jj];
-      }
-    }
-#pragma unroll
-    for (int jj = 0; jj < 4; ++jj) {
-      s1[jj] = lnb_sum_row_groups(s1[jj]);
-      s2[jj] = lnb_sum_row_groups(s2[jj]);
-    }
-    if (lane < 8) {
-      *reinterpret_cast<f32x4*>(&red[(wave * 2 + 0) * 32 + 4 * c4]) = s1;
-      *reinterpret_cast<f32x4*>(&red[(wave * 2 + 1) * 32 + 4 * c4]) = s2;
-    }
-    {
-      Cursor cn = cg;
-      issue_g(cn);
-    }
-    __syncthreads();
-    f32x4 m1 = f32x4{0.f, 0.f, 0.f, 0.f}, m2 = m1;
-#pragma unroll
-    for (int w = 0; w < 8; ++w) {
-      m1 += *reinterpret_cast<const f32x4*>(&red[(w * 2 + 0) * 32 + 4 * c4]);
-      m2 += *reinterpret_cast<const f32x4*>(&red[(w * 2 + 1) * 32 + 4 * c4]);
-    }
-    m1 *= (1.f / WX_K);
-    m2 *= (1.f / WX_K);
-    const f32x4 rs = R[4];
-    const long long ebase = (long long)e * p.eval_stride;
-    const u32x4 Zr = wx_rsrc(p.dz + ebase + col0, ((long long)(WX_K - 1) * ld + valid) * 4);
-    const u32x4 Zres = wx_rsrc(RES ? p.dz_res + ebase + col0 : nullptr, RES ? ((long long)(WX_K - 1) * ld + valid) * 4 : 0);
-    const unsigned off = 4 * c4 < valid ? x_voff : CSN_OOB;
-#pragma unroll
-    for (int i = 0; i < 4; ++i) {
-#pragma unroll
-      for (int jj = 0; jj < 4; ++jj) gx[i][jj] = rs[jj] * (gx[i][jj] - m1[jj] - R[i][jj] * m2[jj]);
-      if constexpr (RES) wx_store4(gx[i], Zres, off, row_soff(i));
-    }
-    if constexpr (DROP) {
-      const unsigned salt = csn_block_salt((unsigned long long)e, p.seed);
-#pragma unroll
-      for (int pr = 0; pr < 2; ++pr)
-#pragma unroll
-        for (int jj = 0; jj < 4; ++jj) {
-          const unsigned hp = csn_fc_pair(2 * krow + 128 * pr, (unsigned)ld, (unsigned)(col0 + 4 * c4 + jj), salt);
-          gx[2 * pr][jj] = csn_keep16(hp, 0, thr16) ? gx[2 * pr][jj] * keep_scale : 0.f;
-          gx[2 * pr + 1][jj] = csn_keep16(hp, 1, thr16) ? gx[2 * pr + 1][jj] * keep_scale : 0.f;
-        }
-    }
-    short* dst = xs + stage * WX_STAGE + 2 * krow * WX_CH + 4 * c4;
-#pragma unroll
-    for (int i = 0; i < 4; ++i) {
-      wx_store4(gx[i], Zr, off, row_soff(i));
-      s16x4 hi, lo;
-      split4<Bf16x3>(gx[i], hi, lo);
-      const int ro = ((i & 1) + 128 * (i >> 1)) * WX_CH;
-      *reinterpret_cast<s16x4*>(dst + ro) = hi;
-      *reinterpret_cast<s16x4*>(dst + ro + WX_PLANE) = lo;
-    }
-  };
-
-  f32x4 R0[5], R1[5], R2[5];
-  Cursor ci = cursor_at(q0), ce = ci, cc = ci, cg = ci;
-  issue_x(ci, R0); advance(ci);
-  issue_x(ci, R1); advance(ci);
-  issue_g(cg); advance(cg);
-  commit(std::integral_constant<int, 0>{}, 0, R0, cc, cg); advance(cc); advance(cg);
-  issue_x(ci, R2); advance(ci);
-  issue_x(ci, R0); advance(ci);
-  __syncthreads();
-  commit(std::integral_constant<int, 0>{}, 1, R1, cc, cg); advance(cc); advance(cg);
-  __syncthreads();
-  auto iteration = [&](auto st_c, f32x4* RQ, f32x4* RC) __attribute__((always_inline)) {
-    constexpr int ST = decltype(st_c)::value;
-    issue_x(ci, RQ); advance(ci);
-    const f32x16 acc = compute(ST);
-    epilogue(ce, acc); advance(ce);
-    commit(std::integral_constant<int, (RES ? 8 : 4) + 5 + 4>{}, (ST + 2) % 3, RC, cc, cg); advance(cc); advance(cg);
-    __syncthreads();
-  };
-  while (true) {
-    if (ce.q >= q_end) break;
-    iteration(std::integral_constant<int, 0>{}, R1, R2);
-    if (ce.q >= q_end) break;
-    iteration(std::integral_constant<int, 1>{}, R2, R0);
-    if (ce.q >= q_end) break;
-    iteration(std::integral_constant<int, 2>{}, R0, R1);
-  }
-  if (RED && red_item != 0xffffffffu) flush_red();
-  asm volatile("s_waitcnt vmcnt(0)" ::: "memory");
-}
+#define WX_LNB_KERNEL csn_wx_lnb_kernel
+#define WX_LNB_OPL false
+#include "wx_lnb_body.inc"
+#undef WX_LNB_KERNEL
+#undef WX_LNB_OPL
+#define WX_LNB_KERNEL csn_wx_lnb_planes_kernel
+#define WX_LNB_OPL true
+#include "wx_lnb_body.inc"
+#undef WX_LNB_KERNEL
+#undef WX_LNB_OPL
 
 __global__ __launch_bounds__(512) void csn_wx_lnb_sums_kernel(const float* __restrict__ ws, float* __restrict__ rowdot,
                                                               float* __restrict__ rowsum, int cpi, int run, int slots, int group) {
@@ -368,7 +77,13 @@
     if (!a.rowdot || !a.rowsum || a.e_base != 0 || a.n_items > a.n_dense || a.dxhat_group < 1 || a.n_items % a.dxhat_group) return -2;
     if (a.red_slots != csn_wx_ln_sum_slots(a.n_items, a.n_points)) return -2;
   }
-  if (a.red_ws) {
+  if (a.dctx_planes) {
+    if (a.dz_res || a.opl_block < 32 || a.opl_block > 512 || (a.opl_block & 3) || a.opl_groups != csn_opl_groups(a.opl_block)) return -2;
+    const long long nb = (a.n_points + a.opl_block - 1) / a.opl_block;
+    if (a.opl_eval_stride < csn_opl_eval_elements(a.opl_block, (int)nb) || a.opl_eval_stride * 2 > 0x7fffffffLL) return -2;
+    if (a.red_ws) hipLaunchKernelGGL((csn_wx_lnb_planes_kernel<true, false, true>), dim3(grid), dim3(512), 0, st, a);
+    else hipLaunchKernelGGL((csn_wx_lnb_planes_kernel<true, false, false>), dim3(grid), dim3(512), 0, st, a);
+  } else if (a.red_ws) {
     if (a.dz_res) hipLaunchKernelGGL((csn_wx_lnb_kernel<true, true, true>), dim3(grid), dim3(512), 0, st, a);
     else hipLaunchKernelGGL((csn_wx_lnb_kernel<true, false, true>), dim3(grid), dim3(512), 0, st, a);
   } else if (a.dz_res) hipLaunchKernelGGL((csn_wx_lnb_kernel<true, true, false>), dim3(grid), dim3(512), 0, st, a);
diff --git a/csn_amd/csrc/wx_lnb_body.inc b/csn_amd/csrc/wx_lnb_body.inc
--- /dev/null
+++ b/csn_amd/csrc/wx_lnb_body.inc
@@ -0,0 +1,334 @@
+template <bool DROP, bool RES, bool RED>
+__global__ __launch_bounds__(512, 2) void WX_LNB_KERNEL(CsnWxLnbArgs p) {
+  constexpr bool OPL = WX_LNB_OPL;
+  __shared__ __attribute__((aligned(16))) short smem[LNB_G + WX_NS * WX_STAGE + 8 * LNB_EBW * 2 + 1024 + 1024 + 1024];
+  short* xs = smem + LNB_G;
+  const int tid = threadIdx.x, lane = tid & 63, wave = __builtin_amdgcn_readfirstlane(tid >> 6);
+  const int l31 = lane & 31, h = lane >> 5;
+  float* eb = reinterpret_cast<float*>(smem + LNB_G + WX_NS * WX_STAGE) + wave * LNB_EBW;
+  float* red = reinterpret_cast<float*>(smem + LNB_G + WX_NS * WX_STAGE + 8 * LNB_EBW * 2);
+  const float* gbuf = reinterpret_cast<const float*>(smem) + 4 * tid;
+  float* ctab = red + 512;
+  float* cells = ctab + 512;
+
+  const int xcd = blockIdx.x & 7, j = blockIdx.x >> 3;
+  const int n_streams = (int)gridDim.x;
+  const int stream = j * 8 + xcd;
+  const unsigned cpi = (unsigned)(p.n_points + WX_CH - 1) / WX_CH;
+  const int n_chunks = p.n_items * (int)cpi;
+  const int run = (n_chunks + n_streams - 1) / n_streams;
+  const int q0 = stream * run, q_end = min(q0 + run, n_chunks);
+  if (q0 >= q_end) return;
+
+  s16x8 Wh[WX_K / 16], Wl[WX_K / 16];
+  {
+    const float* wrow = p.w + ((long long)(32 * wave + l31) * WX_K + 8 * h);
+#pragma unroll
+    for (int s = 0; s < WX_K / 16; ++s) {
+      const f32x4 a0 = *reinterpret_cast<const f32x4*>(wrow + 16 * s), a1 = *reinterpret_cast<const f32x4*>(wrow + 16 * s + 4);
+      s16x4 h0, l0, h1, l1;
+      split4<Bf16x3>(a0, h0, l0);
+      split4<Bf16x3>(a1, h1, l1);
+      Wh[s] = join8(h0, h1);
+      Wl[s] = join8(l0, l1);
+    }
+  }
+
+  const int krow = tid >> 3, c4 = tid & 7;
+  const int ld = p.ld;
+  const unsigned x_voff = (unsigned)(2 * krow * ld + 4 * c4) * 4u;
+  auto row_soff = [&](int i) { return (unsigned)(((i & 1) + 128 * (i >> 1)) * ld) * 4u; };
+  struct Cursor { int q; unsigned item, tile; };
+  auto cursor_at = [&](int q) { Cursor c; c.q = q; c.item = (unsigned)q / cpi; c.tile = (unsigned)q - c.item * cpi; return c; };
+  auto advance = [&](Cursor& c) { ++c.q; if (++c.tile >= cpi) { c.tile = 0; ++c.item; } };
+  auto locate = [&](const Cursor& c, int& col0, int& valid, unsigned& item) {
+    const bool exists = c.q < q_end;
+    col0 = exists ? (int)(c.tile * WX_CH) : 0;
+    valid = exists ? min(WX_CH, p.n_points - col0) : 0;
+    item = __builtin_amdgcn_readfirstlane(exists ? c.item : 0u);
+  };
+  auto issue_x = [&](const Cursor& cu, f32x4* R) {
+    int col0, valid; unsigned item;
+    locate(cu, col0, valid, item);
+    const u32x4 Xr = wx_rsrc(p.xhat + (long long)(p.e_base + item) * p.eval_stride + col0, ((long long)(WX_K - 1) * ld + valid) * 4);
+    const unsigned off = 4 * c4 < valid ? x_voff : CSN_OOB;
+#pragma unroll
+    for (int i = 0; i < 4; ++i) wx_request(R[i], Xr, off, row_soff(i));
+    const u32x4 Sr = wx_rsrc(p.rstd + (long long)(p.e_base + item) * p.n_points + col0, (long long)valid * 4);
+    wx_request(R[4], Sr, 4 * c4 < valid ? (unsigned)(16 * c4) : CSN_OOB, 0u);
+  };
+  const unsigned g_lds = __builtin_amdgcn_readfirstlane((unsigned)(unsigned long)((short __attribute__((address_space(3)))*)smem)) + (unsigned)wave * 1024u;
+  auto issue_g = [&](const Cursor& cu) {
+    int col0, valid; unsigned item;
+    locate(cu, col0, valid, item);
+    const unsigned e = (unsigned)p.e_base + item;
+    const bool dense = RED || (int)e < p.n_dense;
+    const unsigned src = p.dxhat_group > 1 ? e / (unsigned)p.dxhat_group : e;
+    const u32x4 Gr = wx_rsrc(dense ? p.dxhat + (long long)src * p.eval_stride + col0 : nullptr, dense ? ((long long)(WX_K - 1) * ld + valid) * 4 : 0);
+    const unsigned off = 4 * c4 < valid ? x_voff : CSN_OOB;
+    asm volatile("s_waitcnt lgkmcnt(0)" ::: "memory");
+#pragma unroll
+    for (int i = 0; i < 4; ++i) wx_dma(g_lds + 8192u * i, Gr, off, row_soff(i));
+  };
+
+  const int grp = lane >> 4, gq = (lane >> 2) & 3, gp = lane & 3;
+  const int tr_base = (8 * (grp >> 1) + gq) * WX_CH + 16 * (grp & 1) + 4 * gp;
+  auto compute = [&](int stage) {
+    f32x16 acc;
+#pragma unroll
+    for (int r = 0; r < 16; ++r) acc[r] = 0.f;
+    const short* xh = xs + stage * WX_STAGE + tr_base;
+    constexpr int WX_PD = 2, NSTEP = WX_K / 16;
+    s16x8 bh[WX_PD], bl[WX_PD];
+    auto rd = [&](int s, s16x8& fh, s16x8& fl) {
+      const short* a = xh + 16 * s * WX_CH;
+      fh = join8(__builtin_amdgcn_ds_read_tr16_b64_v4i16((lds_s16x4)(a)),
+                 __builtin_amdgcn_ds_read_tr16_b64_v4i16((lds_s16x4)(a + 4 * WX_CH)));
+      fl = join8(__builtin_amdgcn_ds_read_tr16_b64_v4i16((lds_s16x4)(a + WX_PLANE)),
+                 __builtin_amdgcn_ds_read_tr16_b64_v4i16((lds_s16x4)(a + WX_PLANE + 4 * WX_CH)));
+    };
+    __builtin_amdgcn_sched_barrier(0);
+#pragma unroll
+    for (int s = 0; s < WX_PD; ++s) rd(s, bh[s], bl[s]);
+    __builtin_amdgcn_sched_group_barrier(0x100, 4 * WX_PD, 0);
+#pragma unroll
+    for (int s = 0; s < NSTEP; ++s) {
+      const int r = s % WX_PD;
+      acc = wx_mma(Wh[s], Wl[s], bh[r], bl[r], acc);
+      if (s + WX_PD < NSTEP) rd(s + WX_PD, bh[r], bl[r]);
+      __builtin_amdgcn_sched_group_barrier(0x008, 3, 0);
+      __builtin_amdgcn_sched_group_barrier(0x100, 4, 0);
+    }
+    __builtin_amdgcn_sched_barrier(0);
+    return acc;
+  };
+  const int erow = lane >> 3, c8 = lane & 7;
+  auto epilogue = [&](const Cursor& cu, const f32x16& acc) {
+    int col0, valid; unsigned item;
+    locate(cu, col0, valid, item);
+    if constexpr (OPL) {
+      short* eb16 = reinterpret_cast<short*>(eb);
+      const u32x4 Or = wx_rsrc(p.dctx_planes + (long long)(p.e_base + item) * p.opl_eval_stride, p.opl_eval_stride * 2);
+      int ln = lane;
+      asm volatile("" : "+v"(ln));
+      const int T = p.opl_block, lq16 = ln & 15, kq = ln >> 4, l31 = ln & 31, h = ln >> 5;
+      const int b0 = col0 / T, r0 = col0 - b0 * T;
+      unsigned poff[2];
+#pragma unroll
+      for (int gg = 0; gg < 2; ++gg) {
+        const int pt = 16 * gg + lq16;
+        int q = r0 + pt, b = b0;
+        if (q >= T) { q -= T; ++b; }
+        poff[gg] = pt < valid ? (unsigned)(((b * p.opl_groups + (q >> 4)) * 16 + 2 * wave) * 1024 + (16 * kq + (q & 15)) * 16) : CSN_OOB;
+      }
+      s16x4 hi[4], lo[4];
+#pragma unroll
+      for (int k = 0; k < 4; ++k) split4<Bf16x3>(f32x4{acc[4 * k], acc[4 * k + 1], acc[4 * k + 2], acc[4 * k + 3]}, hi[k], lo[k]);
+#pragma unroll
+      for (int pl = 0; pl < 2; ++pl) {
+#pragma unroll
+        for (int k = 0; k < 4; ++k)
+          *reinterpret_cast<s16x4*>(&eb16[l31 * 32 + 8 * (k ^ ((l31 >> 2) & 3)) + 4 * h]) = pl ? lo[k] : hi[k];
+#pragma unroll
+        for (int gg = 0; gg < 2; ++gg) {
+          const int pt = 16 * gg + lq16;
+          const f32x4 v = *reinterpret_cast<const f32x4*>(&eb16[pt * 32 + 8 * (kq ^ ((pt >> 2) & 3))]);
+          wx_store4(v, Or, poff[gg], (unsigned)(1024 * pl));
+        }
+      }
+      return;
+    }
+    const bool n_ok = 4 * c8 < valid;
+    const u32x4 Or = wx_rsrc(p.dctx + (long long)(p.e_base + item) * p.dctx_eval_stride, (long long)256 * ld * 4);
+#pragma unroll
+    for (int half = 0; half < 2; ++half) {
+#pragma unroll
+      for (int rr = 0; rr < 8; ++rr) eb[csn_acc_row(rr, h) * 32 + l31] = acc[8 * half + rr];
+      const unsigned off = n_ok ? (unsigned)((32 * wave + 16 * half + erow) * ld + col0 + 4 * c8) * 4u : CSN_OOB;
+#pragma unroll
+      for (int t = 0; t < 2; ++t) {
+        const f32x4 v = *reinterpret_cast<const f32x4*>(&eb[(erow + 8 * t) * 32 + 4 * c8]);
+        wx_store4(v, Or, off, (unsigned)(8 * t * ld) * 4u);
+      }
+    }
+  };
+
+  const unsigned thr16 = csn_drop_threshold16(p.dropout_p);
+  const float keep_scale = DROP ? 1.f / (1.f - p.dropout_p) : 1.f;
+  unsigned cst_item = 0xffffffffu;
+  unsigned red_item = 0xffffffffu;
+  typedef float f32x2 __attribute__((ext_vector_type(2)));
+  typedef f32x2 __attribute__((address_space(3))) * lds_f32x2;
+  const unsigned smem_lds = (unsigned)(unsigned long)((short __attribute__((address_space(3)))*)smem);
+  const unsigned cells_lds = (unsigned)(unsigned long)((float __attribute__((address_space(3)))*)cells);
+  auto tid16 = [&]() {
+    unsigned ga = (unsigned)(unsigned long)((const float __attribute__((address_space(3)))*)gbuf);
+    asm volatile("" : "+v"(ga));
+    return ga - smem_lds;
+  };
+  auto flush_red = [&]() __attribute__((always_inline)) {
+    const unsigned slot = (unsigned)stream - (red_item * cpi) / (unsigned)run;
+    const u32x4 Wr = wx_rsrc(p.red_ws + ((long long)red_item * p.red_slots + slot) * (2 * WX_K), 2 * WX_K * 4);
+    const unsigned t16 = tid16();
+    if ((t16 & 0x70u) == 0) {
+      const unsigned cell = cells_lds + ((t16 >> 7) << 4), voff = (t16 >> 7) << 3;
+#pragma unroll
+      for (int i = 0; i < 4; ++i) {
+        const lds_f32x2 c = (lds_f32x2)(unsigned long)(cell + 8 * (i & 1) + 1024 * (i >> 1));
+        const f32x2 v = *c;
+        *c = f32x2{0.f, 0.f};
+        lnb_store1(v.x, Wr, voff + 4 * (i & 1) + 512 * (i >> 1));
+        lnb_store1(v.y, Wr, voff + 4 * (i & 1) + 512 * (i >> 1) + 4 * WX_K);
+      }
+    }
+  };
+  if (RED && c4 == 0) {
+#pragma unroll
+    for (int i = 0; i < 4; ++i) *reinterpret_cast<float2*>(&cells[2 * (2 * krow + (i & 1) + 128 * (i >> 1))]) = make_float2(0.f, 0.f);
+  }
+  auto commit = [&](auto wait_c, int stage, f32x4* R, const Cursor& cu, const Cursor& cg) __attribute__((always_inline)) {
+    int col0, valid; unsigned item;
+    locate(cu, col0, valid, item);
+    const unsigned e = (unsigned)p.e_base + item;
+    const bool dense = RED || (int)e < p.n_dense;
+    if (item != cst_item) {
+      cst_item = item;
+      if (tid < WX_K) {
+        const float s = (dense && p.dxhat_scale) ? p.dxhat_scale[(long long)e * WX_K + tid] : 1.f;
+        const float r = p.dxhat_rows ? p.dxhat_rows[(long long)e * WX_K + tid] : 0.f;
+        *reinterpret_cast<float2*>(&ctab[2 * tid]) = make_float2(s, r);
+      }
+      __syncthreads();
+    }
+    const bool reduce = RED && cu.q < q_end;
+    if (reduce && item != red_item) {
+      if (red_item != 0xffffffffu) flush_red();
+      red_item = item;
+    }
+    lnb_arrived<decltype(wait_c)::value>(R);
+    if (reduce) {
+      const unsigned t16 = tid16();
+      const unsigned cell = cells_lds + ((t16 >> 7) << 4);
+      const bool first_lane = (t16 & 0x70u) == 0;
+      const bool in = (int)((t16 >> 2) & 0x1cu) < valid;
+#pragma unroll
+      for (int i = 0; i < 4; ++i) {
+        const f32x4 g = *reinterpret_cast<const f32x4*>(gbuf + 2048 * i);
+        float rd = fmaf(g[3], R[i][3], fmaf(g[2], R[i][2], fmaf(g[1], R[i][1], g[0] * R[i][0])));
+        float rs = in ? (g[0] + g[1]) + (g[2] + g[3]) : 0.f;
+        rd = lnb_sum_row_lanes(rd);
+        rs = lnb_sum_row_lanes(rs);
+        if (first_lane) {
+          if (i == 0) asm volatile("ds_add_f32 %0, %1\n\tds_add_f32 %0, %2 offset:4" :: "v"(cell), "v"(rd), "v"(rs) : "memory");
+          if (i == 1) asm volatile("ds_add_f32 %0, %1 offset:8\n\tds_add_f32 %0, %2 offset:12" :: "v"(cell), "v"(rd), "v"(rs) : "memory");
+          if (i == 2) asm volatile("ds_add_f32 %0, %1 offset:1024\n\tds_add_f32 %0, %2 offset:1028" :: "v"(cell), "v"(rd), "v"(rs) : "memory");
+          if (i == 3) asm volatile("ds_add_f32 %0, %1 offset:1032\n\tds_add_f32 %0, %2 offset:1036" :: "v"(cell), "v"(rd), "v"(rs) : "memory");
+        }
+      }
+      __builtin_amdgcn_sched_barrier(0);
+    }
+    float sc[4], rw[4];
+#pragma unroll
+    for (int i = 0; i < 4; ++i) {
+      const float2 c2 = *reinterpret_cast<const float2*>(&ctab[2 * (2 * krow + (i & 1) + 128 * (i >> 1))]);
+      sc[i] = c2.x;
+      rw[i] = c2.y;
+    }
+    f32x4 gx[4];
+    f32x4 s1 = f32x4{0.f, 0.f, 0.f, 0.f}, s2 = s1;
+#pragma unroll
+    for (int i = 0; i < 4; ++i) {
+      const f32x4 g = *reinterpret_cast<const f32x4*>(gbuf + 2048 * i);
+#pragma unroll
+      for (int jj = 0; jj < 4; ++jj) {
+        gx[i][jj] = dense ? fmaf(g[jj], sc[i], rw[i]) : rw[i];
+        s1[jj] += gx[i][jj];
+        s2[jj] += gx[i][jj] * R[i][jj];
+      }
+    }
+#pragma unroll
+    for (int jj = 0; jj < 4; ++jj) {
+      s1[jj] = lnb_sum_row_groups(s1[jj]);
+      s2[jj] = lnb_sum_row_groups(s2[jj]);
+    }
+    if (lane < 8) {
+      *reinterpret_cast<f32x4*>(&red[(wave * 2 + 0) * 32 + 4 * c4]) = s1;
+      *reinterpret_cast<f32x4*>(&red[(wave * 2 + 1) * 32 + 4 * c4]) = s2;
+    }
+    {
+      Cursor cn = cg;
+      issue_g(cn);
+    }
+    __syncthreads();
+    f32x4 m1 = f32x4{0.f, 0.f, 0.f, 0.f}, m2 = m1;
+#pragma unroll
+    for (int w = 0; w < 8; ++w) {
+      m1 += *reinterpret_cast<const f32x4*>(&red[(w * 2 + 0) * 32 + 4 * c4]);
+      m2 += *reinterpret_cast<const f32x4*>(&red[(w * 2 + 1) * 32 + 4 * c4]);
+    }
+    m1 *= (1.f / WX_K);
+    m2 *= (1.f / WX_K);
+    const f32x4 rs = R[4];
+    const long long ebase = (long long)e * p.eval_stride;
+    const u32x4 Zr = wx_rsrc(p.dz + ebase + col0, ((long long)(WX_K - 1) * ld + valid) * 4);
+    const u32x4 Zres = wx_rsrc(RES ? p.dz_res + ebase + col0 : nullptr, RES ? ((long long)(WX_K - 1) * ld + valid) * 4 : 0);
+    const unsigned off = 4 * c4 < valid ? x_voff : CSN_OOB;
+#pragma unroll
+    for (int i = 0; i < 4; ++i) {
+#pragma unroll
+      for (int jj = 0; jj < 4; ++jj) gx[i][jj] = rs[jj] * (gx[i][jj] - m1[jj] - R[i][jj] * m2[jj]);
+      if constexpr (RES) wx_store4(gx[i], Zres, off, row_soff(i));
+    }
+    if constexpr (DROP) {
+      const unsigned salt = csn_block_salt((unsigned long long)e, p.seed);
+#pragma unroll
+      for (int pr = 0; pr < 2; ++pr)
+#pragma unroll
+        for (int jj = 0; jj < 4; ++jj) {
+          const unsigned hp = csn_fc_pair(2 * krow + 128 * pr, (unsigned)ld, (unsigned)(col0 + 4 * c4 + jj), salt);
+          gx[2 * pr][jj] = csn_keep16(hp, 0, thr16) ? gx[2 * pr][jj] * keep_scale : 0.f;
+          gx[2 * pr + 1][jj] = csn_keep16(hp, 1, thr16) ? gx[2 * pr + 1][jj] * keep_scale : 0.f;
+        }
+    }
+    short* dst = xs + stage * WX_STAGE + 2 * krow * WX_CH + 4 * c4;
+#pragma unroll
+    for (int i = 0; i < 4; ++i) {
+      wx_store4(gx[i], Zr, off, row_soff(i));
+      s16x4 hi, lo;
+      split4<Bf16x3>(gx[i], hi, lo);
+      const int ro = ((i & 1) + 128 * (i >> 1)) * WX_CH;
+      *reinterpret_cast<s16x4*>(dst + ro) = hi;
+      *reinterpret_cast<s16x4*>(dst + ro + WX_PLANE) = lo;
+    }
+  };
+
+  f32x4 R0[5], R1[5], R2[5];
+  Cursor ci = cursor_at(q0), ce = ci, cc = ci, cg = ci;
+  issue_x(ci, R0); advance(ci);
+  issue_x(ci, R1); advance(ci);
+  issue_g(cg); advance(cg);
+  commit(std::integral_constant<int, 0>{}, 0, R0, cc, cg); advance(cc); advance(cg);
+  issue_x(ci, R2); advance(ci);
+  issue_x(ci, R0); advance(ci);
+  __syncthreads();
+  commit(std::integral_constant<int, 0>{}, 1, R1, cc, cg); advance(cc); advance(cg);
+  __syncthreads();
+  auto iteration = [&](auto st_c, f32x4* RQ, f32x4* RC) __attribute__((always_inline)) {
+    constexpr int ST = decltype(st_c)::value;
+    issue_x(ci, RQ); advance(ci);
+    const f32x16 acc = compute(ST);
+    epilogue(ce, acc); advance(ce);
+    commit(std::integral_constant<int, (RES ? 8 : 4) + 5 + 4>{}, (ST + 2) % 3, RC, cc, cg); advance(cc); advance(cg);
+    __syncthreads();
+  };
+  while (true) {
+    if (ce.q >= q_end) break;
+    iteration(std::integral_constant<int, 0>{}, R1, R2);
+    if (ce.q >= q_end) break;
+    iteration(std::integral_constant<int, 1>{}, R2, R0);
+    if (ce.q >= q_end) break;
+    iteration(std::integral_constant<int, 2>{}, R0, R1);
+  }
+  if (RED && red_item != 0xffffffffu) flush_red();
+  asm volatile("s_waitcnt vmcnt(0)" ::: "memory");
+}
diff --git a/csn_amd/functional.py b/csn_amd/functional.py
--- a/csn_amd/functional.py
+++ b/csn_amd/functional.py
@@ -194,6 +194,22 @@
         return False
 
 
+class operand_planes:
+
+    def __init__(self, block: int):
+        self.block = int(block)
+
+    def __enter__(self):
+        L = _lib.lib()
+        self.prev = L.csn_get_thread_operand_planes()
+        _lib.check(L.csn_set_thread_operand_planes(self.block))
+        return self
+
+    def __exit__(self, *exc):
+        _lib.lib().csn_set_thread_operand_planes(self.prev)
+        return False
+
+
 class rows16:
 
     def __init__(self, flag):
@@ -349,6 +365,7 @@
                     and plan.v_shift == 0 and not x_all.requires_grad
                     and _score_flow(ctx.mode, d, T) == tuning.KEEP_SCORES and L.csn_attn_bwd_dq_no_planes_available(d, T))
         ctx.fold = fold
+        ctx.opl = int(L.csn_operand_planes_elements(plan.E, C, D, NP, NP, T)) if (fold and tune.operand_planes) else 0
         w_fv = w_fv_t = None
         if fold:
             ldp = nb * 1024
@@ -443,7 +460,8 @@
         del sum_ws
         if (keep_scores and link is not None and not a16 and tuning.current().fused_mix_bwd and plan.mixed_not_pooled
                 and n_head_evals > 0):
-            link.pre = (xhat, rstd, w_fc, p_fc, seed_fc, n_head_evals, ctx.mode, bool(x_all.requires_grad), w_fv_t)
+            link.pre = (xhat, rstd, w_fc, p_fc, seed_fc, n_head_evals, ctx.mode, bool(x_all.requires_grad), w_fv_t,
+                        (ctx.opl, T))
         if keep_scores:
             ctx.save_for_backward(x_all, w_qkv, w_fc, None if fold else qkv, att, lse, scores, xhat, rstd, kv, w_fv_t,
                                   w_fc_in if fold else None)
@@ -527,23 +545,27 @@
         ws = torch.empty((ws_n,), device=dev, dtype=torch.float32)
         if head_done is not None:
             dz, dz_res, datt, w_fc_t = head_done
+            opl = ctx.opl if datt.dtype == torch.bfloat16 else 0
             if E > ctx.n_head:
-                _lib.check(L.csn_outproj_lnb_f32(_ptr(dense), _ptr(xhat), _ptr(rstd), C * NP, _ptr(w_fc_t), _ptr(dz), _ptr(dz_res),
-                                                 _ptr(datt), ctx.n_head, E - ctx.n_head, C, D, NP, NP, p_fc, seed_fc, _ptr(rows),
-                                                 n_dense, _ptr(scale), group, None, None, None, 0, _stream()),
-                           "csn_outproj_lnb_f32")
+                with operand_planes(T if opl else 0):
+                    _lib.check(L.csn_outproj_lnb_f32(_ptr(dense), _ptr(xhat), _ptr(rstd), C * NP, _ptr(w_fc_t), _ptr(dz),
+                                                     _ptr(dz_res), _ptr(datt), ctx.n_head, E - ctx.n_head, C, D, NP, NP, p_fc,
+                                                     seed_fc, _ptr(rows), n_dense, _ptr(scale), group, None, None, None, 0,
+                                                     _stream()), "csn_outproj_lnb_f32")
             _lib.check(L.csn_project_wgrad_f32(_ptr(dz), C * NP, NP, _ptr(att), D * NP, NP, _ptr(dw_fc), C, D, E, NP, 1.0, 0,
                                                _ptr(ws), ws_n, _stream()), "csn_project_wgrad_f32")
         else:
             dz = torch.empty((E, C, NP), device=dev, dtype=bwd16)
             dz_res = torch.empty((E, C, NP), device=dev, dtype=torch.float32) if (need_dx and (p_fc > 0 or a16)) else None
-            datt = torch.empty((E, D, NP), device=dev, dtype=bwd16)
+            opl = ctx.opl if (ctx.fold and dz_res is None) else 0
+            datt = torch.empty((E, opl), device=dev, dtype=torch.bfloat16) if opl else torch.empty((E, D, NP), device=dev, dtype=bwd16)
             w_fc_t = w_fv_t if ctx.fold else w_fc.t().contiguous()
-            _lib.check(L.csn_outproj_ln_bwd_f32(_ptr(dense), _ptr(xhat), _ptr(rstd), C * NP, _ptr(att), D * NP,
-                                                _ptr(w_fc_t), _ptr(dz), _ptr(dz_res), _ptr(datt), _ptr(dw_fc), _ptr(ws), ws_n,
-                                                E, C, D, NP, NP, 0, p_fc, seed_fc, 0, 0, _ptr(rows), n_dense, _ptr(scale), group,
-                                                _stream()),
-                       "csn_outproj_ln_bwd_f32")
+            with operand_planes(T if opl else 0):
+                _lib.check(L.csn_outproj_ln_bwd_f32(_ptr(dense), _ptr(xhat), _ptr(rstd), C * NP, _ptr(att), D * NP,
+                                                    _ptr(w_fc_t), _ptr(dz), _ptr(dz_res), _ptr(datt), _ptr(dw_fc), _ptr(ws), ws_n,
+                                                    E, C, D, NP, NP, 0, p_fc, seed_fc, 0, 0, _ptr(rows), n_dense, _ptr(scale), group,
+                                                    _stream()),
+                           "csn_outproj_ln_bwd_f32")
         del ws
 
         if ctx.fold:
@@ -557,11 +579,12 @@
                 launches = [(0 if ci == 0 else 1, ids, ids.numel(), None, 0) for ci, ids in enumerate(plan.dq_colors)]
             L.csn_dev_set(_lib.DEV_KV_SAME, int(bool(ctx.tune.kv_same)))
             for accumulate, ids, n_ids, off, n_groups in launches:
-                _lib.check(L.csn_block_attn_bwd_dq_f32(_ptr(datt), _ptr(att), D * NP, _ptr(kv), _ptr(kv), kv_stride,
-                                                       _ptr(plan.kv_slots), NP, _ptr(scores), None, _ptr(lse), None,
-                                                       _ptr(g), D * NP, _ptr(plan.q_slots), accumulate, _ptr(ids), n_ids, H, d, T,
-                                                       nb, Tp, p_attn, seed_attn, 0, 0, kv_flag, kv_pitch, 3, _ptr(off), n_groups,
-                                                       _stream()), "csn_block_attn_bwd_dq_f32")
+                with operand_planes(T if opl else 0):
+                    _lib.check(L.csn_block_attn_bwd_dq_f32(_ptr(datt), _ptr(att), D * NP, _ptr(kv), _ptr(kv), kv_stride,
+                                                           _ptr(plan.kv_slots), NP, _ptr(scores), None, _ptr(lse), None,
+                                                           _ptr(g), D * NP, _ptr(plan.q_slots), accumulate, _ptr(ids), n_ids, H, d,
+                                                           T, nb, Tp, p_attn, seed_attn, 0, 0, kv_flag, kv_pitch, 3, _ptr(off),
+                                                           n_groups, _stream()), "csn_block_attn_bwd_dq_f32")
             del datt
             if plan.q_ranges is None:
                 d_m = project_wgrad(g, x_all)
@@ -714,7 +737,7 @@
 def _lnb_head(link: MixLink, dfeats: torch.Tensor, scale: torch.Tensor, group: int):
     if link is None or link.pre is None:
         return None
-    xhat, rstd, w_fc, p_fc, seed_fc, n, mode, need_dx, w_fc_t = link.pre
+    xhat, rstd, w_fc, p_fc, seed_fc, n, mode, need_dx, w_fc_t, (opl, block) = link.pre
     E, C, NP = xhat.shape
     D = w_fc.shape[1]
     L = _lib.lib()
@@ -728,12 +751,15 @@
         rowsum = torch.empty((n // group, C), device=dev, dtype=torch.float32)
         dz = torch.empty((E, C, NP), device=dev, dtype=torch.float32)
         dz_res = torch.empty((E, C, NP), device=dev, dtype=torch.float32) if (need_dx and p_fc > 0) else None
-        datt = torch.empty((E, D, NP), device=dev, dtype=torch.float32)
+        if dz_res is not None:
+            opl = 0
+        datt = torch.empty((E, opl), device=dev, dtype=torch.bfloat16) if opl else torch.empty((E, D, NP), device=dev, dtype=torch.float32)
         if w_fc_t is None:
             w_fc_t = w_fc.t().contiguous()
-        _lib.check(L.csn_outproj_lnb_f32(_ptr(dfeats), _ptr(xhat), _ptr(rstd), C * NP, _ptr(w_fc_t), _ptr(dz), _ptr(dz_res),
-                                         _ptr(datt), 0, n, C, D, NP, NP, p_fc, seed_fc, None, n, _ptr(scale), group, _ptr(rowdot),
-                                         _ptr(rowsum), _ptr(red_ws), ws_n, _stream()), "csn_outproj_lnb_f32")
+        with operand_planes(block if opl else 0):
+            _lib.check(L.csn_outproj_lnb_f32(_ptr(dfeats), _ptr(xhat), _ptr(rstd), C * NP, _ptr(w_fc_t), _ptr(dz), _ptr(dz_res),
+                                             _ptr(datt), 0, n, C, D, NP, NP, p_fc, seed_fc, None, n, _ptr(scale), group,
+                                             _ptr(rowdot), _ptr(rowsum), _ptr(red_ws), ws_n, _stream()), "csn_outproj_lnb_f32")
     link.head_done = (dz, dz_res, datt, w_fc_t)
     return rowdot, rowsum
 
diff --git a/csn_amd/tuning.py b/csn_amd/tuning.py
--- a/csn_amd/tuning.py
+++ b/csn_amd/tuning.py
@@ -25,6 +25,7 @@
     dv_from_scores: bool = True
     folded_projections: bool = True
     kv_same: bool = True
+    operand_planes: bool = True
     named: frozenset = frozenset()
     score_flow: Dict[object, int] = field(default_factory=lambda: {
         1: KEEP_SCORES,
diff --git a/include/csn_hip.h b/include/csn_hip.h
--- a/include/csn_hip.h
+++ b/include/csn_hip.h
@@ -384,6 +384,10 @@
                             int c_in, int c_out, const int* fwd_table, const int* bwd_table, const float* w, float* dx,
                             long long ld_dx, float* dw, float* dbias, void* ws, long long ws_bytes, void* stream);
 
+CSN_API long long csn_operand_planes_elements(int n_evals, int d_model, int d_inner, int ld, int n_points, int block);
+CSN_API int csn_set_thread_operand_planes(int block);
+CSN_API int csn_get_thread_operand_planes(void);
+
 #define CSN_DEV_BIG_TILES 0
 #define CSN_DEV_WIDE_GEMM 1
 #define CSN_DEV_WIDE_FORMS 2
@@ -391,6 +395,7 @@
 #define CSN_DEV_LNB_GROUP 5
 #define CSN_DEV_SCONV_NB 7
 #define CSN_DEV_KV_SAME 8
+#define CSN_DEV_OPERAND_PLANES 9
 CSN_API int csn_dev_set(int key, int value);
 CSN_API int csn_dev_get(int key);
 
```

After: 18.17 million points/s (median of 5 runs). About the same (+0.2%).
